# VinAIResearch/COMBAT

Measured on AMD Instinct MI355X. Metric: images/sec per alternated generator+surrogate step, CIFAR-10 bs=128, 1/2/4/8 GPU, higher is better.
Workload: dtype bf16; 1 GPU; train_generator.py --dataset cifar10 --pc 0.5 --noise_rate 0.08: alternated PreActResNet18 surrogate + UNet generator step (Phase C + Phase G, both Nesterov-SGD updates), bs=128 per GPU, on-device augmentation on; per_gpu_batch=128, global_batch=128, parallelism=dp1 (RCCL all-reduce of netC grads in Phase C, netG grads in Phase G), losses_finite=True, deterministic=True

## Files before the change

combat_amd/_lib.py:

```python
from __future__ import annotations

import ctypes as C
import os

HERE = os.path.dirname(os.path.abspath(__file__))
LIB_PATH = os.environ.get("COMBAT_HIP_LIB") or os.path.join(HERE, "libcombat_hip.so")

c_i32, c_i64, c_f32, c_vp = C.c_int32, C.c_int64, C.c_float, C.c_void_p


class ConvArgs(C.Structure):

    _fields_ = [
        ("N", c_i32), ("H", c_i32), ("W", c_i32), ("C", c_i32),
        ("P", c_i32), ("Q", c_i32), ("K", c_i32),
        ("R", c_i32), ("S", c_i32), ("stride", c_i32), ("pad", c_i32),
        ("mode", c_i32),
        ("src", c_vp), ("wpack", c_vp), ("kpad", c_i32), ("rows_pad", c_i32), ("dst", c_vp),
        ("pro_scale", c_vp), ("pro_shift", c_vp), ("pro_group_stride", c_i32), ("pro_act", c_i32),
        ("pro_slope", c_f32),
        ("bias", c_vp), ("add_pre", c_vp), ("mask_x", c_vp), ("mask_scale", c_vp), ("mask_shift", c_vp),
        ("mask_activated", c_i32), ("mask_group_stride", c_i32), ("mask_slope", c_f32), ("mask_mul_scale", c_i32),
        ("add_post", c_vp), ("tanh_out", c_i32),
        ("stats_kind", c_i32), ("stats", c_vp), ("xh_mean", c_vp), ("xh_rstd", c_vp),
        ("act_dst", c_vp), ("act_scale", c_vp), ("act_shift", c_vp), ("act_slope", c_f32),
        ("workspace", c_vp), ("workspace_bytes", c_i64),
        ("tile", c_i32),
        ("src2", c_vp), ("wpack2", c_vp), ("kpad2", c_i32), ("rows_pad2", c_i32),
        ("pro_act_dst", c_vp),
    ]


class WgradArgs(C.Structure):

    _fields_ = [
        ("N", c_i32), ("H", c_i32), ("W", c_i32), ("C", c_i32),
        ("P", c_i32), ("Q", c_i32), ("K", c_i32),
        ("R", c_i32), ("S", c_i32), ("stride", c_i32), ("pad", c_i32),
        ("src", c_vp), ("dy", c_vp), ("dw", c_vp), ("k_real", c_i32), ("c_real", c_i32),
        ("pro_scale", c_vp), ("pro_shift", c_vp), ("pro_group_stride", c_i32), ("pro_act", c_i32),
        ("pro_slope", c_f32), ("split", c_i32),
        ("workspace", c_vp), ("workspace_bytes", c_i64),
        ("defer_reduce", c_i32), ("reserved", c_i32),
        ("reduce_first", c_vp),
    ]


class PackDesc(C.Structure):

    _fields_ = [("w", c_vp), ("wf", c_vp), ("wd", c_vp),
                ("K", c_i32), ("taps", c_i32), ("c_real", c_i32), ("C", c_i32), ("dup_hilo", c_i32),
                ("rows_pad_f", c_i32), ("kpad_f", c_i32), ("rows_pad_d", c_i32), ("kpad_d", c_i32), ("reserved", c_i32),
                ("row_scale", c_vp)]


class BnDesc(C.Structure):

    _fields_ = [("gamma", c_vp), ("beta", c_vp), ("running_mean", c_vp), ("running_var", c_vp),
                ("scale", c_vp), ("shift", c_vp), ("C", c_i32), ("reserved", c_i32)]


SIGNATURES = {
    "combat_version": (C.c_char_p, []),
    "combat_abi_version": (C.c_int, []),
    "combat_set_deterministic": (None, [C.c_int]),
    "combat_get_deterministic": (C.c_int, []),
    "combat_conv_gemm": (C.c_int, [C.POINTER(ConvArgs), c_vp]),
    "combat_conv_gemm_pair": (C.c_int, [C.POINTER(ConvArgs), C.POINTER(ConvArgs), c_vp]),
    "combat_conv_workspace_bytes": (c_i64, [C.POINTER(ConvArgs)]),
    "combat_conv_pick_tile": (C.c_int, [C.POINTER(ConvArgs)]),
    "combat_conv_stats_granule": (C.c_int, [C.c_int]),
    "combat_conv_stats_layout": (C.c_int, [C.POINTER(ConvArgs), C.POINTER(c_i32), C.POINTER(c_i32)]),
    "combat_conv_wgrad": (C.c_int, [C.POINTER(WgradArgs), c_vp]),
    "combat_conv_wgrad_workspace_bytes": (c_i64, [C.POINTER(WgradArgs)]),
    "combat_conv_wgrad_reduce": (C.c_int, [C.POINTER(WgradArgs), c_vp]),
    "combat_pack_weights": (C.c_int, [c_vp, c_i32, c_i32, c_i32, c_i32, c_i32, c_vp, c_i32, c_i32, c_vp, c_i32,
                                      c_i32, c_vp]),
    "combat_norm_finalize": (C.c_int, [c_vp, c_i32, c_i32, c_i32, c_f32, c_f32, c_vp, c_vp, c_vp, c_vp, c_vp, c_vp,
                                       c_vp, c_vp, c_f32, c_vp, c_vp, c_i64, c_vp]),
    "combat_norm_scratch_bytes": (c_i64, [c_i32, c_i32]),
    "combat_bn_eval_fold": (C.c_int, [c_vp, c_vp, c_vp, c_vp, c_f32, c_i32, c_vp, c_vp, c_vp]),
    "combat_pack_weights_batch": (C.c_int, [c_vp, c_i32, c_vp]),
    "combat_bn_eval_fold_batch": (C.c_int, [c_vp, c_i32, c_f32, c_vp]),
    "combat_group_stats": (C.c_int, [c_vp, c_i32, c_i32, c_i32, c_vp, c_vp]),
    "combat_norm_bwd_finalize": (C.c_int, [c_vp, c_i32, c_i32, c_i32, c_f32, c_vp, c_vp, c_vp, c_vp, c_vp, c_vp,
                                           c_vp, c_vp, c_vp, c_i64, c_vp]),
    "combat_norm_bwd_apply": (C.c_int, [c_vp, c_vp, c_vp, c_vp, c_i64, c_i32, c_i32, c_i32, c_vp, c_vp, c_vp, c_vp]),
    "combat_norm_act_fused": (C.c_int, [c_vp, c_vp, c_i32, c_i32, c_i64, c_i32, c_f32, c_f32, c_vp, c_vp, c_vp, c_vp, c_vp,
                                        c_vp, c_vp, c_vp, c_f32, c_vp, c_vp, c_i64, c_vp, c_vp]),
    "combat_norm_add_act_fused": (C.c_int, [c_vp, c_vp, c_i32, c_i32, c_i64, c_i32, c_f32, c_f32, c_vp, c_vp, c_vp, c_vp, c_vp,
                                            c_vp, c_vp, c_vp, c_f32, c_vp, c_vp, c_i64, c_vp, c_vp, c_vp, c_vp, c_vp]),
    "combat_norm_bwd_fused": (C.c_int, [c_vp, c_vp, c_vp, c_vp, c_i32, c_i32, c_i64, c_i32, c_vp, c_vp, c_vp, c_vp, c_vp,
                                        c_vp, c_i64, c_vp, c_vp]),
    "combat_group_stats_bwd": (C.c_int, [c_vp, c_vp, c_i32, c_i32, c_i32, c_i32, c_vp, c_vp, c_vp, c_vp]),
    "combat_unet_up_fused": (C.c_int, [c_vp, c_vp, c_i32, c_vp, c_vp, c_vp, c_i32, c_i32, c_i32, c_i32, c_f32, c_vp, c_vp,
                                       c_vp, c_vp, c_vp, c_vp]),
    "combat_unet_up_bwd_fused": (C.c_int, [c_vp, c_vp, c_vp, c_vp, c_vp, c_i32, c_i32, c_i32, c_i32, c_vp, c_vp, c_vp]),
    "combat_unet_up_fwd": (C.c_int, [c_vp, c_vp, c_vp, c_vp, c_vp, c_vp, c_i32, c_i32, c_i32, c_i32, c_vp, c_vp]),
    "combat_unet_up_bwd": (C.c_int, [c_vp, c_vp, c_i32, c_i32, c_i32, c_i32, c_vp, c_vp]),
    "combat_trigger_fwd": (C.c_int, [c_vp, c_vp, c_vp, c_vp, c_f32, c_i32, c_i32, c_vp, c_vp, c_vp, c_vp, c_vp]),
    "combat_trigger_bwd": (C.c_int, [c_vp, c_vp, c_vp, c_vp, c_f32, c_i32, c_i32, c_vp, c_vp, c_vp, c_f32, c_i32, c_vp, c_vp]),
    "combat_trigger_tv_fwd": (C.c_int, [c_vp, c_vp, c_vp, c_vp, c_f32, c_i32, c_i32, c_vp, c_vp, c_vp, c_vp]),
    "combat_trigger_tv_bwd": (C.c_int, [c_vp, c_vp, c_vp, c_vp, c_f32, c_i32, c_i32, c_vp, c_vp, c_vp, c_f32, c_f32, c_i32, c_vp, c_vp]),
    "combat_trigger_pair_fwd": (C.c_int, [c_vp, c_vp, c_vp, c_vp, c_f32, c_i32, c_i32, c_vp, c_vp, c_vp, c_vp]),
    "combat_trigger_pair_bwd": (C.c_int, [c_vp, c_vp, c_vp, c_vp, c_f32, c_i32, c_i32, c_vp, c_vp, c_vp, c_f32, c_vp, c_i32,
                                          c_vp, c_vp]),
    "combat_trigger_groups_fwd": (C.c_int, [c_vp, c_vp, c_vp, c_vp, c_f32, c_i32, c_i32, c_i32, c_vp, c_vp, c_vp]),
    "combat_trigger_groups_bwd": (C.c_int, [c_vp, c_vp, c_vp, c_vp, c_f32, c_i32, c_i32, c_i32, c_vp, c_vp, c_vp, c_f32, c_i32,
                                            c_vp, c_vp]),
    "combat_cond_fwd": (C.c_int, [c_vp, c_vp, c_i32, c_i32, c_i32, c_i32, c_vp, c_vp]),
    "combat_cond_wgrad": (C.c_int, [c_vp, c_vp, c_i32, c_i32, c_i32, c_i32, c_vp, c_vp, c_vp, c_vp]),
    "combat_augment_fwd": (C.c_int, [c_vp, c_vp, c_vp, c_i32, c_i32, c_vp, c_vp, c_vp]),
    "combat_augment_bwd": (C.c_int, [c_vp, c_i32, c_vp, c_i32, c_i32, c_vp, c_i32, c_vp]),
    "combat_head_fwd": (C.c_int, [c_vp, c_i32, c_i32, c_i32, c_vp, c_vp, c_i32, c_vp, c_f32, c_vp, c_vp, c_vp, c_vp,
                                  c_vp, c_vp, c_vp]),
    "combat_head_bwd": (C.c_int, [c_vp, c_i32, c_i32, c_i32, c_vp, c_i32, c_vp, c_vp, c_f32, c_vp, c_vp, c_vp, c_vp,
                                  c_vp]),
    "combat_head_fwd_bwd": (C.c_int, [c_vp, c_i32, c_i32, c_i32, c_vp, c_vp, c_i32, c_vp, c_f32, c_vp, c_vp, c_vp, c_vp,
                                      c_vp, c_vp, c_vp, c_vp, c_vp]),
    "combat_head_bwd_weights": (C.c_int, [c_vp, c_vp, c_i32, c_i32, c_i32, c_i32, c_vp, c_vp, c_vp]),
    "combat_prune_sweep": (C.c_int, [c_vp, c_i32, c_vp, c_vp, c_vp, c_i32, c_i32, c_i32, c_vp, c_vp, c_vp, c_vp, c_vp]),
    "combat_feature_colsum": (C.c_int, [c_vp, c_i32, c_i32, c_vp, c_vp]),
    "combat_strip_superimpose": (C.c_int, [c_vp, c_i32, c_vp, c_i32, c_vp, c_i32, c_i32, c_i32, c_vp, c_vp]),
    "combat_strip_entropy": (C.c_int, [c_vp, c_i32, c_i32, c_i32, c_vp, c_vp]),
    "combat_nc_blend": (C.c_int, [c_vp, c_i32, c_vp, c_i32, c_vp, c_i32, c_i32, c_i32, c_i32, c_vp, c_vp, c_f32, c_vp, c_vp,
                                  c_vp]),
    "combat_nc_update": (C.c_int, [c_vp, c_vp, c_i32, c_vp, c_i32, c_vp, c_i32, c_i32, c_i32, c_i32, c_vp, c_i32, c_i32,
                                   c_vp, c_vp, c_vp, c_vp, c_f32, c_vp, c_f32, c_f32, c_f32, c_f32, c_vp, c_vp, c_vp, c_i32,
                                   c_vp, c_vp]),
    "combat_gradcam_seed": (C.c_int, [c_vp, c_vp, c_i32, c_i32, c_i32, c_i32, c_vp, c_vp, c_vp, c_vp]),
    "combat_gradcam_map": (C.c_int, [c_vp, c_vp, c_i32, c_i32, c_i32, c_i32, c_vp, c_vp, c_vp, c_vp]),
    "combat_comm_unique_id": (C.c_int, [c_vp]),
    "combat_comm_init_rank": (C.c_int, [C.POINTER(c_vp), c_i32, c_vp, c_i32]),
    "combat_comm_destroy": (C.c_int, [c_vp]),
    "combat_allreduce": (C.c_int, [c_vp, c_i64, c_i32, c_vp, c_vp]),
    "combat_sgd_nesterov": (C.c_int, [c_vp, c_vp, c_i32, c_i64, c_f32, c_f32, c_f32, c_f32, c_i32, c_vp]),
    "combat_image_to_c8": (C.c_int, [c_vp, c_i32, c_i32, c_vp, c_vp]),
    "combat_nhwc_to_nchw_f32": (C.c_int, [c_vp, c_i32, c_i32, c_i32, c_i32, c_i32, c_vp, c_vp]),
    "combat_nchw_to_nhwc_bf16": (C.c_int, [c_vp, c_i32, c_i32, c_i32, c_i32, c_i32, c_vp, c_vp]),
    "combat_memset_zero": (C.c_int, [c_vp, c_i64, c_vp]),
    "combat_copy3": (C.c_int, [c_vp, c_vp, c_i64, c_vp, c_vp, c_i64, c_vp, c_vp, c_i64, c_vp]),
    "combat_relu_mask": (C.c_int, [c_vp, c_vp, c_i64, c_vp, c_vp]),
    "combat_colsum": (C.c_int, [c_vp, c_i64, c_i32, c_i32, c_vp, c_vp]),
    "combat_log_terms": (C.c_int, [c_vp, c_vp, c_vp, c_i32, c_i32, c_vp, c_vp, c_vp, c_vp]),
    "combat_log_terms_tv": (C.c_int, [c_vp, c_vp, c_vp, c_vp, c_i32, c_i32, c_vp, c_vp, c_vp, c_vp]),
    "combat_maxpool2": (C.c_int, [c_vp, c_i32, c_i32, c_i32, c_i32, c_vp, c_vp]),
    "combat_elu_affine": (C.c_int, [c_vp, c_i64, c_i32, c_vp, c_vp, c_vp, c_vp]),
    "combat_affine_act": (C.c_int, [c_vp, c_i64, c_i32, c_vp, c_vp, c_i64, c_f32, c_vp, c_vp]),
    "combat_dct_u8": (C.c_int, [c_vp, c_vp, c_i32, c_i32, c_vp, c_vp]),
    "combat_linear_nhwc": (C.c_int, [c_vp, c_i32, c_i32, c_i32, c_i32, c_vp, c_vp, c_i32, c_vp, c_vp]),
    "combat_grid_head_fwd": (C.c_int, [c_vp, c_vp, c_vp, c_i32, c_i32, c_vp, c_vp]),
    "combat_wanet_grid": (C.c_int, [c_vp, c_vp, c_i32, c_i32, c_f32, c_vp, c_vp, c_vp]),
    "combat_warp_fwd": (C.c_int, [c_vp, c_vp, c_vp, c_i32, c_i32, c_i32, c_vp, c_vp]),
    "combat_warp_bwd": (C.c_int, [c_vp, c_vp, c_vp, c_vp, c_i32, c_i32, c_i32, c_i32, c_vp, c_vp]),
    "combat_warp_bwd_input": (C.c_int, [c_vp, c_vp, c_i32, c_i32, c_i32, c_vp, c_vp]),
    "combat_wanet_field_bwd": (C.c_int, [c_vp, c_i32, c_vp, c_vp, c_i32, c_i32, c_f32, c_f32, c_vp, c_vp, c_vp, c_i32, c_vp,
                                         c_vp, c_vp, c_vp, c_vp]),
    "combat_plan_create": (c_vp, []),
    "combat_plan_destroy": (None, [c_vp]),
    "combat_plan_record": (C.c_int, [c_vp, c_i32]),
    "combat_plan_record_cancel": (C.c_int, []),
    "combat_plan_set_after": (C.c_int, [c_vp, c_i32]),
    "combat_plan_size": (c_i32, [c_vp]),
    "combat_plan_run": (C.c_int, [c_vp, c_i32, c_i32, c_vp, C.POINTER(c_vp), c_i32]),
    "combat_plan_join": (C.c_int, [c_vp, c_vp, C.POINTER(c_vp), c_i32]),
    "combat_plan_failed_call": (c_i32, [c_vp]),
}

TILE_128x128, TILE_128x64, TILE_64x64, TILE_128x16, TILE_64x128 = 1, 2, 3, 4, 5
TILE_H256x64, TILE_H128x128, TILE_H128x64, TILE_H64x64, TILE_D128x64, TILE_D128x32 = 6, 7, 8, 9, 10, 11
TILE_G128x64, TILE_G128x32 = 12, 13
TILE_D256x64, TILE_C8, TILE_D256W64, TILE_S128x64, TILE_K8 = 14, 15, 16, 17, 18
STATS_PER_WORKGROUP = 4


class CombatHipError(RuntimeError):
    pass


def load(path: str = LIB_PATH) -> C.CDLL:
    if not os.path.exists(path):
        raise ImportError(
            "combat_amd: %s not found -- the HIP library is required (no CPU fallback exists); "
            "build it with `python -m combat_amd.build`" % path)
    lib = C.CDLL(path)
    for name, (res, args) in SIGNATURES.items():
        try:
            fn = getattr(lib, name)
        except AttributeError as e:
            raise ImportError("combat_amd: %s does not export %s" % (path, name)) from e
        fn.restype = res
        fn.argtypes = args
    return lib


lib = load()


def check(status: int, what: str, detail: str = "") -> None:
    if status == 0:
        return
    kind = {-1: "invalid shape/argument", -2: "HIP launch failed"}.get(status, "status %d" % status)
    raise CombatHipError("%s: %s %s" % (what, kind, detail))
```

combat_amd/csrc/capi.cpp:

```cpp
#include "combat_hip.h"

#include <hip/hip_runtime.h>

#include <atomic>
#include <cstdlib>
#include <mutex>
#include <unordered_map>

#define COMBAT_ABI_VERSION 20

extern "C" const char *combat_version(void) { return "combat_hip gfx950 abi17"; }
extern "C" int combat_abi_version(void) { return COMBAT_ABI_VERSION; }

static std::atomic<int> g_deterministic{-1};
bool combat_deterministic() {
    int v = g_deterministic.load(std::memory_order_relaxed);
    if (v < 0) {
        const char *e = getenv("COMBAT_DETERMINISTIC");
        v = e && e[0] == '1';
        g_deterministic.store(v, std::memory_order_relaxed);
    }
    return v != 0;
}
extern "C" void combat_set_deterministic(int on) { g_deterministic.store(on ? 1 : 0, std::memory_order_relaxed); }
extern "C" int combat_get_deterministic(void) { return combat_deterministic() ? 1 : 0; }

float *combat_stream_scratch(void *stream, size_t bytes) {
    constexpr size_t kBytes = 2u << 20;
    if (bytes > kBytes) return nullptr;
    static std::mutex mu;
    static std::unordered_map<void *, float *> regions;
    std::lock_guard<std::mutex> lock(mu);
    int dev = 0;
    if (hipGetDevice(&dev) != hipSuccess) return nullptr;
    void *key = reinterpret_cast<void *>(reinterpret_cast<uintptr_t>(stream) ^ (static_cast<uintptr_t>(dev + 1) << 56));
    auto it = regions.find(key);
    if (it != regions.end()) return it->second;
    void *ptr = nullptr;
    if (hipMalloc(&ptr, kBytes) != hipSuccess) return nullptr;
    regions.emplace(key, static_cast<float *>(ptr));
    return static_cast<float *>(ptr);
}
```

combat_amd/csrc/conv_wgrad.hip:

```cpp
#include "conv_common.hpp"
#include "plan.hpp"

namespace {

struct WgradParams {
    combat_wgrad_args a;
    int M, PQ, ntaps, tiles_k, tiles_c, split, pix_per_split;
    float *ws;
};

template <int BMC, int BNC>
struct WCfg {
    static constexpr int WGK = (BNC == 16) ? 4 : (BMC == 16 ? 1 : 2);
    static constexpr int WGC = 4 / WGK;
    static constexpr int WK = BMC / WGK;
    static constexpr int WC = BNC / WGC;
    static constexpr int FK = WK / 16;
    static constexpr int FC = WC / 16;
    static constexpr int SK = (BMC + 16) * 2;
    static constexpr int SC = (BNC + 16) * 2;
    static constexpr int CHK = BMC / 8;
    static constexpr int CHC = BNC / 8;
    static constexpr int ITK = (64 * CHK + 255) / 256;
    static constexpr int ITC = (64 * CHC + 255) / 256;
// ... 276 lines not shown
            {
                const unsigned char *b = kl + prow * SK + (wid * 16 + pp * 4) * 2;
                const s16x4_t lo = lds_tr16(b), hi = lds_tr16(b + 4 * SK);
                const s16x8_t v = {lo[0], lo[1], lo[2], lo[3], hi[0], hi[1], hi[2], hi[3]};
                fk[ks] = __builtin_bit_cast(bf16x8_t, v);
            }
#pragma unroll
            for (int j = 0; j < FC; ++j) {
                const unsigned char *b = cl + prow * SC + (j * 16 + pp * 4) * 2;
                const s16x4_t lo = lds_tr16(b), hi = lds_tr16(b + 4 * SC);
                const s16x8_t v = {lo[0], lo[1], lo[2], lo[3], hi[0], hi[1], hi[2], hi[3]};
                fc[ks][j] = __builtin_bit_cast(bf16x8_t, v);
            }
        }
        __builtin_amdgcn_sched_barrier(0);
#pragma unroll
        for (int ks = 0; ks < 2; ++ks)
#pragma unroll
            for (int j = 0; j < FC; ++j) acc[j] = __builtin_amdgcn_mfma_f32_16x16x32_bf16(fk[ks], fc[ks][j], acc[j], 0, 0, 0);
        __builtin_amdgcn_sched_barrier(0);
    };
    load_tile(0);
    store_tile(0);
    __syncthreads();
    for (int kt = 0; kt < nkt; ++kt) {
        const bool more = kt + 1 < nkt;
        if (more) load_tile(kt + 1);
        compute(kt & 1);
        if (more) store_tile((kt + 1) & 1);
        __syncthreads();
    }
    float *ep = reinterpret_cast<float *>(smem);
    {
        const int fr = lane & 15, fq = lane >> 4;
#pragma unroll
        for (int j = 0; j < FC; ++j) {
            const int col = j * 16 + fr, row = wid * 16 + fq * 4;
#pragma unroll
            for (int e = 0; e < 4; ++e) ep[(row + e) * EPS + col] = acc[j][e];
        }
    }
    __syncthreads();
    const int creal = a.c_real;
    if (p.ws) {
        float *slab = p.ws + (size_t)blockIdx.x * (BMC * 9 * creal);
        for (int idx = tid; idx < BMC * 9 * creal; idx += 256) {
            const int row = idx / (9 * creal), rem = idx - row * 9 * creal;
            const int tap = rem / creal, c = rem - tap * creal;
            float v = ep[row * EPS + tap * 8 + c];
            if (creal < 8 && c + creal < 8) v += ep[row * EPS + tap * 8 + c + creal];
            slab[idx] = v;
        }
        return;
    }
    for (int idx = tid; idx < BMC * 72; idx += 256) {
        const int row = idx / 72, col = idx - row * 72;
        const int n = k0 + row, tap = col >> 3;
        int c = col & 7;
        if (n >= a.k_real) continue;
        if (creal < 8) {
            if (c >= 2 * creal) continue;
            if (c >= creal) c -= creal;
        }
        atomicAdd(a.dw + ((size_t)n * 9 + tap) * creal + c, ep[row * EPS + col]);
    }
}

__global__ __launch_bounds__(256) void conv_wgrad_c8_reduce_kernel(const float *__restrict__ ws, float *__restrict__ dw,
                                                                   int tiles_k, int split, int per_tile, int k_real,
                                                                   int row_elems, float *__restrict__ part) {
    const int e = blockIdx.x * 256 + threadIdx.x, tile_k = blockIdx.y;
    if (e >= per_tile) return;
    const int n = tile_k * 64 + e / row_elems;
    if (n >= k_real) return;
    float s0 = 0.f, s1 = 0.f, s2 = 0.f, s3 = 0.f;
    const int G = gridDim.z;
    int sp = blockIdx.z;
    for (; sp + 3 * G < split; sp += 4 * G) {
        s0 += ws[((size_t)sp * tiles_k + tile_k) * per_tile + e];
        s1 += ws[((size_t)(sp + G) * tiles_k + tile_k) * per_tile + e];
        s2 += ws[((size_t)(sp + 2 * G) * tiles_k + tile_k) * per_tile + e];
        s3 += ws[((size_t)(sp + 3 * G) * tiles_k + tile_k) * per_tile + e];
    }
    for (; sp < split; sp += G) s0 += ws[((size_t)sp * tiles_k + tile_k) * per_tile + e];
    const float s = (s0 + s1) + (s2 + s3);
    if (part) part[((size_t)blockIdx.z * tiles_k + tile_k) * per_tile + e] = s;
    else atomicAdd(dw + (size_t)tile_k * per_tile + e, s);
}

int launch_c8(WgradParams p, hipStream_t st) {
    constexpr int SMEM = 2 * 64 * ((64 + 16) * 2 + (80 + 16) * 2);
    static_assert(SMEM >= 64 * 84 * 4, "epilogue image");
    static bool attr_set = false;
    if (!attr_set) {
        if (hipFuncSetAttribute(reinterpret_cast<const void *>(conv_wgrad_c8_kernel), hipFuncAttributeMaxDynamicSharedMemorySize, SMEM) != hipSuccess)
            return COMBAT_ELAUNCH;
        attr_set = true;
    }
    p.tiles_k = p.a.K / 64;
    p.tiles_c = 1;
    int split = p.a.split;
    const int ktiles = (p.M + 63) / 64;
    if (split <= 0) {
        split = (256 + p.tiles_k - 1) / p.tiles_k;
        const int max_split = (ktiles + 3) / 4;
        if (split > max_split) split = max_split;
        if (split < 1) split = 1;
    }
    if (split > ktiles) split = ktiles;
    p.pix_per_split = ((ktiles + split - 1) / split) * 64;
    p.split = (p.M + p.pix_per_split - 1) / p.pix_per_split;
    const int per_tile = 64 * 9 * p.a.c_real;
    const long need = (long)p.tiles_k * p.split * per_tile * 4;
    p.ws = (p.split > 1 && p.a.workspace && p.a.workspace_bytes >= need) ? reinterpret_cast<float *>(p.a.workspace) : nullptr;
    if (combat_deterministic() && p.split > 1 && !p.ws) return COMBAT_EINVAL;
    COMBAT_LAUNCH(conv_wgrad_c8_kernel, dim3((unsigned)(p.tiles_k * p.split)), dim3(256), SMEM, st, p);
    CB_LAUNCH_CHECK();
    if (p.ws) {
        const int groups = p.split >= 32 ? 16 : 1;
        float *part = nullptr;
        if (combat_deterministic() && groups > 1) {
            const long extra = (long)groups * p.tiles_k * per_tile * 4;
            if (p.a.workspace_bytes >= need + extra) part = p.ws + need / 4;
        }
        const int g1 = combat_deterministic() && !part ? 1 : groups;
        COMBAT_LAUNCH(conv_wgrad_c8_reduce_kernel, dim3((per_tile + 255) / 256, p.tiles_k, g1), dim3(256), 0, st, (const float *)p.ws,
                           p.a.dw, p.tiles_k, p.split, per_tile, p.a.k_real, 9 * p.a.c_real, part);
        CB_LAUNCH_CHECK();
        if (part) {
            COMBAT_LAUNCH(conv_wgrad_c8_reduce_kernel, dim3((per_tile + 255) / 256, p.tiles_k, 1), dim3(256), 0, st, (const float *)part,
                               p.a.dw, p.tiles_k, groups, per_tile, p.a.k_real, 9 * p.a.c_real, (float *)nullptr);
            CB_LAUNCH_CHECK();
        }
    }
    return COMBAT_OK;
}

__global__ __launch_bounds__(256) void wgrad_slab_reduce_kernel(const float *__restrict__ ws, float *__restrict__ dw, int split,
                                                                int ntaps, int tiles_k, int tiles_c, int bmc, int bnc, int k_real,
                                                                int c_real, int C) {
    const long e = (long)blockIdx.x * 256 + threadIdx.x;
    if (e >= (long)k_real * ntaps * c_real) return;
    const int c = (int)(e % c_real), tap = (int)((e / c_real) % ntaps), n = (int)(e / ((long)c_real * ntaps));
    const int tile_k = n / bmc, row = n - tile_k * bmc;
    const size_t tile_elems = (size_t)bmc * bnc, sstride = (size_t)ntaps * tiles_k * tiles_c * tile_elems;
    float total = 0.f;
    for (int half = 0; half < 2; ++half) {
        const int cs = c + half * c_real;
        if (half && (c_real >= C || cs >= C || cs >= 2 * c_real)) break;
        const int tile_c = cs / bnc, col = cs - tile_c * bnc;
        const float *src = ws + (((size_t)tap * tiles_k + tile_k) * tiles_c + tile_c) * tile_elems + (size_t)row * bnc + col;
        float s0 = 0.f, s1 = 0.f, s2 = 0.f, s3 = 0.f;
        int sp = 0;
        for (; sp + 4 <= split; sp += 4) {
            s0 += src[(size_t)sp * sstride];
            s1 += src[(size_t)(sp + 1) * sstride];
            s2 += src[(size_t)(sp + 2) * sstride];
            s3 += src[(size_t)(sp + 3) * sstride];
        }
        for (; sp < split; ++sp) s0 += src[(size_t)sp * sstride];
        total += (s0 + s1) + (s2 + s3);
    }
    dw[e] += total;
}

template <int BMC, int BNC>
int64_t generic_slab_bytes(const combat_wgrad_args &a, int split) {
    const long tiles_k = (a.K + BMC - 1) / BMC, tiles_c = (a.C + BNC - 1) / BNC;
    return (int64_t)split * a.R * a.S * tiles_k * tiles_c * BMC * BNC * 4;
}

template <int BMC, int BNC>
int launch(WgradParams p, hipStream_t st) {
    using T = WCfg<BMC, BNC>;
    static bool attr_set = false;
    auto kern = conv_wgrad_kernel<BMC, BNC>;
    if (!attr_set) {
        if (hipFuncSetAttribute(reinterpret_cast<const void *>(kern), hipFuncAttributeMaxDynamicSharedMemorySize,
                                T::SMEM) != hipSuccess)
            return COMBAT_ELAUNCH;
        attr_set = true;
    }
    p.tiles_k = (p.a.K + BMC - 1) / BMC;
    p.tiles_c = (p.a.C + BNC - 1) / BNC;
    int split = p.a.split;
    const int ktiles = (p.M + 63) / 64;
    if (split <= 0) {
        const int base = p.tiles_k * p.tiles_c * p.ntaps;
        split = ((BMC == 16 ? 2304 : 256) + base - 1) / base;
        const int max_split = (ktiles + 3) / 4;
        if (split > max_split) split = max_split;
        if (split < 1) split = 1;
    }
    if (split > ktiles) split = ktiles;
    p.pix_per_split = ((ktiles + split - 1) / split) * 64;
    p.split = (p.M + p.pix_per_split - 1) / p.pix_per_split;
    const long blocks = (long)p.tiles_k * p.tiles_c * p.ntaps * p.split;
    p.ws = nullptr;
    if (combat_deterministic() && p.split > 1) {
        const int64_t need = generic_slab_bytes<BMC, BNC>(p.a, p.split);
        if (!p.a.workspace || p.a.workspace_bytes < need) return COMBAT_EINVAL;
        p.ws = reinterpret_cast<float *>(p.a.workspace);
    }
    COMBAT_LAUNCH(kern, dim3((unsigned)blocks), dim3(256), T::SMEM, st, p);
    CB_LAUNCH_CHECK();
    if (p.ws) {
        const long elems = (long)p.a.k_real * p.ntaps * p.a.c_real;
        COMBAT_LAUNCH(wgrad_slab_reduce_kernel, dim3((unsigned)((elems + 255) / 256)), dim3(256), 0, st, (const float *)p.ws, p.a.dw,
                      p.split, p.ntaps, p.tiles_k, p.tiles_c, BMC, BNC, p.a.k_real, p.a.c_real, p.a.C);
        CB_LAUNCH_CHECK();
    }
    return COMBAT_OK;
}

template <int BMC, int BNC>
int generic_split(const combat_wgrad_args &a) {
    const long M = (long)a.N * a.P * a.Q;
    const int ktiles = (int)((M + 63) / 64), ntaps = a.R * a.S;
    const int tiles_k = (a.K + BMC - 1) / BMC, tiles_c = (a.C + BNC - 1) / BNC;
    int split = a.split > 0 ? a.split : 0;
    if (split <= 0) {
        const int base = tiles_k * tiles_c * ntaps;
        split = ((BMC == 16 ? 2304 : 256) + base - 1) / base;
        const int max_split = (ktiles + 3) / 4;
        if (split > max_split) split = max_split;
        if (split < 1) split = 1;
    }
    if (split > ktiles) split = ktiles;
    const int pix_per_split = ((ktiles + split - 1) / split) * 64;
    return (int)((M + pix_per_split - 1) / pix_per_split);
}

bool c8_applies(const combat_wgrad_args *a) {
    return a->split >= 0 && a->C == 8 && a->R == 3 && (a->K & 63) == 0 && !a->pro_scale && !a->pro_act;
}

int64_t c8_workspace(const combat_wgrad_args &a) {
    const long M = (long)a.N * a.P * a.Q;
    const int ktiles = (int)((M + 63) / 64), tiles_k = a.K / 64;
    int split = a.split;
    if (split <= 0) {
        split = (256 + tiles_k - 1) / tiles_k;
        const int max_split = (ktiles + 3) / 4;
        if (split > max_split) split = max_split;
        if (split < 1) split = 1;
    }
    if (split > ktiles) split = ktiles;
    const int pix_per_split = ((ktiles + split - 1) / split) * 64;
    const long nsplit = (M + pix_per_split - 1) / pix_per_split;
    if (nsplit <= 1) return 0;
    const int64_t per_tile = 64 * 9 * a.c_real * 4;
    return tiles_k * nsplit * per_tile + (nsplit >= 32 ? 16 * tiles_k * per_tile : 0);
}

int64_t generic_workspace(const combat_wgrad_args &a) {
    if (a.C <= 16) return generic_slab_bytes<64, 16>(a, generic_split<64, 16>(a));
    if (a.K <= 16) return generic_slab_bytes<16, 64>(a, generic_split<16, 64>(a));
    if (a.C % 128 == 0 && a.K % 128 == 0) return generic_slab_bytes<128, 128>(a, generic_split<128, 128>(a));
    return generic_slab_bytes<64, 64>(a, generic_split<64, 64>(a));
}

}

extern "C" int64_t combat_conv_wgrad_workspace_bytes(const combat_wgrad_args *a) {
    if (!a) return 0;
    const int64_t dma = a->split >= 0 ? (int64_t)conv_wgrad3x3_dma_workspace(a) : 0;
    if (dma > 0 || !combat_deterministic()) return dma;
    return c8_applies(a) ? c8_workspace(*a) : generic_workspace(*a);
}

static int validate_wgrad_args(const combat_wgrad_args *a) {
    if (!a || !a->src || !a->dy || !a->dw) return COMBAT_EINVAL;
    if (a->N <= 0 || a->H <= 0 || a->W <= 0 || a->P <= 0 || a->Q <= 0) return COMBAT_EINVAL;
    if (a->C < 8 || (a->C & 7) || a->K < 8 || (a->K & 7)) return COMBAT_EINVAL;
    if (a->R != a->S || (a->R != 1 && a->R != 3)) return COMBAT_EINVAL;
    if (a->stride != 1 && a->stride != 2) return COMBAT_EINVAL;
    if (a->c_real <= 0 || a->c_real > a->C || a->k_real <= 0 || a->k_real > a->K) return COMBAT_EINVAL;
    if ((a->pro_scale == nullptr) != (a->pro_shift == nullptr)) return COMBAT_EINVAL;
    if ((long)a->N * a->P * a->Q > 0x7fffffffL / 8) return COMBAT_EINVAL;
    return COMBAT_OK;
}

extern "C" int combat_conv_wgrad_reduce(const combat_wgrad_args *a, void *stream) {
    COMBAT_PLAN_HOOK(combat_conv_wgrad_reduce, a);
    if (validate_wgrad_args(a) != COMBAT_OK) return COMBAT_EINVAL;
    if (a->split < 0 || !a->defer_reduce) return COMBAT_OK;
    return conv_wgrad3x3_dma_reduce(a, as_stream(stream));
}

extern "C" int combat_conv_wgrad(const combat_wgrad_args *a, void *stream) {
    COMBAT_PLAN_HOOK(combat_conv_wgrad, a);
    if (validate_wgrad_args(a) != COMBAT_OK) return COMBAT_EINVAL;
    WgradParams p;
    p.a = *a;
    p.ws = nullptr;
    p.PQ = a->P * a->Q;
    p.M = (int)((long)a->N * p.PQ);
    p.ntaps = a->R * a->S;
    hipStream_t st = as_stream(stream);
    if (a->split >= 0) {
        int rc = conv_wgrad3x3_dma_try(a, st);
        if (rc <= 0) return rc;
    }
    if (a->reduce_first) {
        const int rc = combat_conv_wgrad_reduce(a->reduce_first, stream);
        if (rc != COMBAT_OK) return rc;
    }
    if (a->split >= 0 && !combat_deterministic()) {
        const int rc = conv_wgrad3x3_try(a, st);
        if (rc <= 0) return rc;
    }
    if (a->split < 0) p.a.split = 0;
    if (c8_applies(a)) return launch_c8(p, st);
    if (a->C <= 16) return launch<64, 16>(p, st);
    if (a->K <= 16) return launch<16, 64>(p, st);
    if (a->C % 128 == 0 && a->K % 128 == 0) return launch<128, 128>(p, st);
    return launch<64, 64>(p, st);
}
```

combat_amd/csrc/conv_wgrad3x3_dma.hip:

```cpp
#include "conv_common.hpp"
#include <stdlib.h>

namespace {

typedef __attribute__((address_space(3))) void lds_void_t;
constexpr unsigned kOob = 0x40000000u;

struct W3dParams {
    combat_wgrad_args a;
    int TW, TH, TI, HWP, HH, HROWS, hpw, tw_shift, th_shift;
    int tiles_x, tiles_y, ntiles, tiles_k, tiles_c, split, per;
    unsigned x_bytes, dy_bytes;
    float *ws;
    const float *red_ws;
    float *red_dw;
    int red_base, red_tiles_c, red_split, red_k_real, red_c_real, red_pad;
    unsigned long long *stamps;
};

#ifdef COMBAT_STAMPS
static unsigned long long *g_stamps_wgrad_host = nullptr;
extern "C" int combat_debug_set_stamps_wgrad(void *p) { g_stamps_wgrad_host = (unsigned long long *)p; return 0; }
#define WCLK() __builtin_readcyclecounter()
#else
#define WCLK() 0ull
#endif

typedef __attribute__((address_space(3))) unsigned char lds_u8;
__device__ __forceinline__ s16x4_t tr16d(const lds_u8 *p) {
    return __builtin_amdgcn_ds_read_tr16_b64_v4i16((__attribute__((address_space(3))) s16x4_t *)(const_cast<lds_u8 *>(p)));
}

__device__ __forceinline__ bf16x8_t join8(const s16x4_t lo, const s16x4_t hi) {
    typedef __attribute__((ext_vector_type(8))) short s16x8_t;
    const s16x8_t v = {lo[0], lo[1], lo[2], lo[3], hi[0], hi[1], hi[2], hi[3]};
    return __builtin_bit_cast(bf16x8_t, v);
}

__device__ __forceinline__ int xkey(int TW, int line, int hx) {
    return ((hx >> 1) & 1) | ((TW == 4 ? (line >> 1) & 1 : ((hx >> 3) + line) & 1) << 1);
}
__device__ __forceinline__ int dkey(int pk) { return ((pk >> 1) & 1) | (((pk >> 3) & 1) << 1); }

template <int N>
__device__ __forceinline__ void wait_vm_lgkm0_barrier() {
    asm volatile("s_waitcnt vmcnt(%0) lgkmcnt(0)" ::"n"(N) : "memory");
    __builtin_amdgcn_s_barrier();
    asm volatile("" ::: "memory");
}

template <int NT>
__device__ __forceinline__ void reduce_slabs(const float *__restrict__ ws, float *__restrict__ dw, int base, int tiles_c, int split,
                                             int k_real, int c_real, unsigned char *scratch, int block, int nblocks) {
    constexpr int U = 4;
    const int tid = threadIdx.x;
    const long e4 = (long)base * 9 * 1024;
    const long per = (e4 + nblocks - 1) / nblocks;
    const long q0 = (long)block * per, q1 = q0 + per < e4 ? q0 + per : e4;
    int SL = 1;
    while (SL * 2 <= split && SL < 32 && (long)(NT / (SL * 2)) * U >= per) SL *= 2;
    const int QP = NT / SL, sl = tid / QP, ql = tid - sl * QP;
    const int nsl = (split - sl + SL - 1) / SL;
    f32x4_t *scr = reinterpret_cast<f32x4_t *>(scratch);
    const size_t sstride = (size_t)base * 9 * 4096;
    for (long qb = q0; qb < q1; qb += (long)QP * U) {
        f32x4_t acc[U];
        long qq[U];
#pragma unroll
        for (int u = 0; u < U; ++u) {
            acc[u] = f32x4_t{0.f, 0.f, 0.f, 0.f};
            qq[u] = qb + (long)u * QP + ql;
        }
        for (int i = 0; i < nsl; i += 4) {
            f32x4_t v[U][4];
#pragma unroll
            for (int u = 0; u < U; ++u)
#pragma unroll
                for (int j = 0; j < 4; ++j) {
                    const bool ok = qq[u] < q1 && i + j < nsl;
                    const float *src = ws + (ok ? qq[u] : q0) * 4 + (size_t)(ok ? sl + (i + j) * SL : 0) * sstride;
                    const f32x4_t x = *reinterpret_cast<const f32x4_t *>(src);
                    v[u][j] = ok ? x : f32x4_t{0.f, 0.f, 0.f, 0.f};
                }
#pragma unroll
            for (int u = 0; u < U; ++u) acc[u] += (v[u][0] + v[u][1]) + (v[u][2] + v[u][3]);
        }
        if (SL > 1) {
#pragma unroll
            for (int u = 0; u < U; ++u) scr[tid * U + u] = acc[u];
            __syncthreads();
            if (sl == 0)
                for (int l = 1; l < SL; ++l)
#pragma unroll
                    for (int u = 0; u < U; ++u) acc[u] += scr[(l * QP + ql) * U + u];
        }
        if (sl == 0) {
#pragma unroll
            for (int u = 0; u < U; ++u) {
                const long q = qq[u];
                if (q >= q1) continue;
                const int f4 = (int)(q & 1023), tap = (int)((q >> 10) % 9), tile = (int)(q / (9 * 1024));
                const int i = f4 >> 9, wave = (f4 >> 6) & 7, lane = f4 & 63;
                const int row = (i * 2 + (wave & 1)) * 16 + (lane >> 4) * 4, col = (wave >> 1) * 16 + (lane & 15);
                const int tile_c = tile % tiles_c, tile_k = tile / tiles_c;
                const int n = tile_k * 64 + row, c = tile_c * 64 + col;
                if (c < c_real) {
#pragma unroll
                    for (int e = 0; e < 4; ++e)
                        if (n + e < k_real) dw[((size_t)(n + e) * 9 + tap) * c_real + c] += acc[u][e];
                }
            }
        }
        if (SL > 1) __syncthreads();
    }
}

template <int HPW, int NS, bool RED>
__device__ __forceinline__ void wgrad3x3_dma_body(const W3dParams &p) {
    extern __shared__ __attribute__((aligned(16))) unsigned char smem[];
    const combat_wgrad_args &a = p.a;
    const int tid = threadIdx.x, lane = tid & 63;
    const int wid = __builtin_amdgcn_readfirstlane(tid >> 6);
    const int wave_k = wid & 1, wave_c = wid >> 1;
    if (RED && p.red_ws) {
        reduce_slabs<512>(p.red_ws, p.red_dw, p.red_base, p.red_tiles_c, p.red_split, p.red_k_real, p.red_c_real, smem, blockIdx.x, gridDim.x);
        __syncthreads();
    }
    int bid = blockIdx.x;
    const int tile_c = bid % p.tiles_c; bid /= p.tiles_c;
    const int tile_k = bid % p.tiles_k;
    const int sp = bid / p.tiles_k;
    const int k0 = tile_k * 64, c0 = tile_c * 64;
    const int t_begin = sp * p.per;
    int t_end = t_begin + p.per;
    if (t_end > p.ntiles) t_end = p.ntiles;
    if (t_begin >= t_end) return;

    const int C = a.C, K = a.K, H = a.H, W = a.W;
    constexpr int XBYTES = HPW * 8192, DYBYTES = 64 * 128, DYBASE = NS * XBYTES;
    constexpr int NDMA = 1 + HPW;
    auto rsrc_words = [&](const void *ptr, unsigned bytes) __attribute__((always_inline)) {
        const unsigned long base = (unsigned long)ptr;
        u32x4_t w;
        w[0] = __builtin_amdgcn_readfirstlane((unsigned)base);
        w[1] = __builtin_amdgcn_readfirstlane((unsigned)(base >> 32) & 0xffffu);
        w[2] = __builtin_amdgcn_readfirstlane(bytes);
        w[3] = 0x00020000u;
        return w;
    };
    const u32x4_t xrs = rsrc_words(a.src, p.x_bytes), dyrs = rsrc_words(a.dy, p.dy_bytes);
    const unsigned lds0 = __builtin_amdgcn_readfirstlane((unsigned)(unsigned long)(lds_void_t *)smem) + wid * 1024;
#ifdef COMBAT_WGRAD_BUILTIN_DMA
    const __amdgpu_buffer_rsrc_t xrsrc = __builtin_amdgcn_make_buffer_rsrc(const_cast<void *>(a.src), 0, p.x_bytes, 0x00020000);
    const __amdgpu_buffer_rsrc_t dyrsrc = __builtin_amdgcn_make_buffer_rsrc(const_cast<void *>(a.dy), 0, p.dy_bytes, 0x00020000);
#define COMBAT_W3_DMA(rs_builtin, rs_words, lds_off, voff) \
    __builtin_amdgcn_raw_ptr_buffer_load_lds(rs_builtin, (lds_void_t *)(smem + (lds_off) + wid * 1024), 16, voff, 0, 0, 0)
#else
#define COMBAT_W3_DMA(rs_builtin, rs_words, lds_off, voff) \
    asm volatile("s_mov_b32 m0, %0\n\ts_nop 0\n\tbuffer_load_dwordx4 %1, %2, 0 offen lds" ::"s"(lds0_l + (unsigned)(lds_off)), "v"(voff), "s"(rs_words##_l) : "memory", "m0")
#endif

    int hdec[HPW], hrel[HPW];
#pragma unroll
    for (int j = 0; j < HPW; ++j) {
        const int row = (wid + 8 * j) * 8 + (lane >> 3), slot = lane & 7;
        const int hx = row % p.HWP, line = row / p.HWP;
        const int hy = line % p.HH, ti = line / p.HH;
        const int chunk = (((slot >> 1) ^ xkey(p.TW, line, hx)) << 1) | (slot & 1);
        hdec[j] = row < p.HROWS ? (hx | (hy << 8) | (ti << 16)) : -1;
        hrel[j] = (((ti * H + hy - 1) * W + hx - 1) * C + c0 + chunk * 8) * 2;
        asm volatile("" : "+v"(hdec[j]), "+v"(hrel[j]));
    }
    int dti[1], drel[1];
#pragma unroll
    for (int j = 0; j < 1; ++j) {
        const int pk = wid * 8 + (lane >> 3), slot = lane & 7;
        const int tx = pk & (p.TW - 1), ty = (pk >> p.tw_shift) & (p.TH - 1), ti = pk >> (p.tw_shift + p.th_shift);
        const int chunk = (((slot >> 1) ^ dkey(pk)) << 1) | (slot & 1);
        dti[j] = ti;
        drel[j] = (((ti * H + ty) * W + tx) * K + k0 + chunk * 8) * 2;
        asm volatile("" : "+v"(dti[j]), "+v"(drel[j]));
    }
    int nt_x, nt_y, nt_g;
    {
        const int t = t_begin;
        nt_x = t % p.tiles_x;
        nt_y = (t / p.tiles_x) % p.tiles_y;
        nt_g = t / (p.tiles_x * p.tiles_y);
    }
    int is_img0 = 0, is_oy0 = 0, is_ox0 = 0, is_xorg = 0, is_dorg = 0;
    auto issue_prep = [&]() __attribute__((always_inline)) {
        is_img0 = nt_g * p.TI;
        is_oy0 = nt_y * p.TH;
        is_ox0 = nt_x * p.TW;
        const int origin = (is_img0 * H + is_oy0) * W + is_ox0;
        is_xorg = origin * C * 2;
        is_dorg = origin * K * 2;
        if (++nt_x == p.tiles_x) {
            nt_x = 0;
            if (++nt_y == p.tiles_y) {
                nt_y = 0;
                ++nt_g;
            }
        }
    };
    auto issue_piece = [&](auto j_tag, auto slot_tag) __attribute__((always_inline)) {
        constexpr int j = decltype(j_tag)::value;
        constexpr int slot_i = decltype(slot_tag)::value;
        const u32x4_t xrs_l = xrs, dyrs_l = dyrs;
        const unsigned lds0_l = lds0;
        (void)xrs_l; (void)dyrs_l; (void)lds0_l;
        if constexpr (j == 0) {
            const unsigned off = is_img0 + dti[0] < a.N ? (unsigned)(is_dorg + drel[0]) : kOob;
            COMBAT_W3_DMA(dyrsrc, dyrs, DYBASE + slot_i * DYBYTES, off);
        } else if constexpr (j <= HPW) {
            const int d = hdec[j - 1];
            const bool ok = d >= 0 && is_img0 + (d >> 16) < a.N && (unsigned)(is_oy0 + ((d >> 8) & 255) - 1) < (unsigned)H &&
                            (unsigned)(is_ox0 + (d & 255) - 1) < (unsigned)W;
            const unsigned off = ok ? (unsigned)(is_xorg + hrel[j - 1]) : kOob;
            COMBAT_W3_DMA(xrsrc, xrs, slot_i * XBYTES + 8 * (j - 1) * 1024, off);
        }
    };
    auto issue = [&](auto slot_tag) __attribute__((always_inline)) {
        using std::integral_constant;
        issue_prep();
        issue_piece(integral_constant<int, 0>{}, slot_tag);
        issue_piece(integral_constant<int, 1>{}, slot_tag);
        issue_piece(integral_constant<int, 2>{}, slot_tag);
        issue_piece(integral_constant<int, 3>{}, slot_tag);
        issue_piece(integral_constant<int, 4>{}, slot_tag);
    };

    const int q = (lane & 15) >> 2, pp = lane & 3, fq = lane >> 4;
    constexpr int SPS = 65536 / XBYTES, NSETS = (NS + SPS - 1) / SPS;
    const lds_u8 *const smem_l = (const lds_u8 *)smem;
    const lds_u8 *dyp[2][2][2], *xp[NSETS][2][2][9];
    int dya[2][2], xa[2][2][9];
#pragma unroll
    for (int ks = 0; ks < 2; ++ks)
#pragma unroll
        for (int hi = 0; hi < 2; ++hi) {
            const int pk = ks * 32 + fq * 8 + q + 4 * hi;
            dya[ks][hi] = pk * 128 + ((wave_k ^ dkey(pk)) & 3) * 32 + pp * 8;
            const int tx = pk & (p.TW - 1), ty = (pk >> p.tw_shift) & (p.TH - 1), ti = pk >> (p.tw_shift + p.th_shift);
#pragma unroll
            for (int tap = 0; tap < 9; ++tap) {
                const int r = (tap * 11) >> 5, s = tap - 3 * r;
                const int line = ti * p.HH + ty + r, hx = tx + s;
                xa[ks][hi][tap] = (line * p.HWP + hx) * 128 + ((wave_c ^ xkey(p.TW, line, hx)) & 3) * 32 + pp * 8;
#pragma unroll
                for (int set = 0; set < NSETS; ++set) {
                    xp[set][ks][hi][tap] = smem_l + set * SPS * XBYTES + xa[ks][hi][tap];
                    asm volatile("" : "+v"(xp[set][ks][hi][tap]));
                }
            }
#pragma unroll
            for (int i = 0; i < 2; ++i) {
                dyp[ks][hi][i] = smem_l + DYBASE + (dya[ks][hi] ^ (i * 64));
                asm volatile("" : "+v"(dyp[ks][hi][i]));
            }
        }

    f32x4_t acc[9][2];
#pragma unroll
    for (int t = 0; t < 9; ++t)
#pragma unroll
        for (int i = 0; i < 2; ++i) acc[t][i] = f32x4_t{0.f, 0.f, 0.f, 0.f};

    auto x_frags = [&](bf16x8_t (&fx)[2], auto slot_tag, auto tap_tag) __attribute__((always_inline)) {
        constexpr int tap = decltype(tap_tag)::value, slot = decltype(slot_tag)::value;
        constexpr int set = slot / SPS, imm = (slot % SPS) * XBYTES;
#pragma unroll
        for (int ks = 0; ks < 2; ++ks) fx[ks] = join8(tr16d(xp[set][ks][0][tap] + imm), tr16d(xp[set][ks][1][tap] + imm));
#ifdef COMBAT_NO_INTERLEAVE
        __builtin_amdgcn_sched_barrier(0);
#endif
    };
    auto mfma_tap = [&](auto tap_tag, const bf16x8_t (&fk)[2][2], const bf16x8_t (&fx)[2]) __attribute__((always_inline)) {
        constexpr int tap = decltype(tap_tag)::value;
#pragma unroll
        for (int ks = 0; ks < 2; ++ks)
#pragma unroll
            for (int i = 0; i < 2; ++i)
                acc[tap][i] = __builtin_amdgcn_mfma_f32_16x16x32_bf16(fk[ks][i], fx[ks], acc[tap][i], 0, 0, 0);
#ifndef COMBAT_NO_INTERLEAVE
        if (tap < 8) {
#pragma unroll
            for (int r = 0; r < 4; ++r) {
                __builtin_amdgcn_sched_group_barrier(0x008, 1, 0);
                __builtin_amdgcn_sched_group_barrier(0x100, 1, 0);
            }
        }
#endif
        __builtin_amdgcn_sched_barrier(0);
    };
    auto compute = [&](auto slot_tag, auto nslot_tag, bool ahead) __attribute__((always_inline)) {
        constexpr int slot = decltype(slot_tag)::value, imm = slot * DYBYTES;
        bf16x8_t fk[2][2];
#pragma unroll
        for (int ks = 0; ks < 2; ++ks)
#pragma unroll
            for (int i = 0; i < 2; ++i)
                fk[ks][i] = join8(tr16d(dyp[ks][0][i] + imm), tr16d(dyp[ks][1][i] + imm));
        using std::integral_constant;
        (void)nslot_tag;
        (void)ahead;
        bf16x8_t fx0[2], fx1[2];
        x_frags(fx0, slot_tag, integral_constant<int, 0>{});
        __builtin_amdgcn_sched_barrier(0);
#define COMBAT_W3_TAP(t, cur, nxt)                                                   \
        if (t < 8) x_frags(nxt, slot_tag, integral_constant<int, (t < 8 ? t + 1 : 8)>{});  \
        mfma_tap(integral_constant<int, t>{}, fk, cur);
        COMBAT_W3_TAP(0, fx0, fx1) COMBAT_W3_TAP(1, fx1, fx0) COMBAT_W3_TAP(2, fx0, fx1) COMBAT_W3_TAP(3, fx1, fx0)
        COMBAT_W3_TAP(4, fx0, fx1) COMBAT_W3_TAP(5, fx1, fx0) COMBAT_W3_TAP(6, fx0, fx1) COMBAT_W3_TAP(7, fx1, fx0)
        COMBAT_W3_TAP(8, fx0, fx1)
#undef COMBAT_W3_TAP
    };
    static_assert(HPW <= 4, "issue() spells out 1 + HPW <= 5 pieces");

    const int npatch = t_end - t_begin;
    using std::integral_constant;
    unsigned long long ph[4] = {0, 0, 0, 0};
    unsigned long long c_loop0 = 0;
    {
    issue(integral_constant<int, 0>{});
    if (NS > 2 && npatch > 1) issue(integral_constant<int, 1 % NS>{});
    if (NS > 2 && npatch > 1) wait_vm_lgkm0_barrier<NDMA>(); else wait_vm_lgkm0_barrier<0>();
    c_loop0 = WCLK();
    auto body = [&](auto slot_tag, int i) __attribute__((always_inline)) {
        constexpr int slot = decltype(slot_tag)::value, nslot = (slot + NS - 1) % NS;
        const bool ahead = i + NS - 1 < npatch;
        const unsigned long long c0 = WCLK();
        if (ahead) issue(integral_constant<int, nslot>{});
        __builtin_amdgcn_sched_barrier(0);
        const unsigned long long c1 = WCLK();
        compute(integral_constant<int, slot>{}, integral_constant<int, nslot>{}, ahead);
        const unsigned long long c2 = WCLK();
        if (ahead) wait_vm_lgkm0_barrier<(NS - 2) * NDMA>(); else wait_vm_lgkm0_barrier<0>();
#ifdef COMBAT_STAMPS
        const unsigned long long c3 = WCLK();
        ph[0] += c1 - c0; ph[1] += c2 - c1; ph[2] += c3 - c2; ph[3] += 1;
#else
        (void)c0; (void)c1; (void)c2;
#endif
    };
    for (int i = 0; i < npatch; i += NS) {
        body(integral_constant<int, 0>{}, i);
        if (NS > 1 && i + 1 < npatch) body(integral_constant<int, 1 % NS>{}, i + 1);
        if (NS > 2 && i + 2 < npatch) body(integral_constant<int, 2 % NS>{}, i + 2);
    }
    }
    static_assert(NS == 2 || NS == 3, "the patch loop is unrolled for rings of two or three stages");
#ifdef COMBAT_STAMPS
    const unsigned long long c_loop1 = WCLK();
#endif

    if (p.ws) {
        float *slab = p.ws + (size_t)blockIdx.x * 9 * 4096;
#pragma unroll
        for (int tap = 0; tap < 9; ++tap)
#pragma unroll
            for (int i = 0; i < 2; ++i)
                *reinterpret_cast<f32x4_t *>(slab + tap * 4096 + ((i * 8 + wid) * 64 + lane) * 4) = acc[tap][i];
    } else {
        float *ep = reinterpret_cast<float *>(smem);
        constexpr int EPS = 68;
        const int fr = lane & 15;
#pragma unroll 1
        for (int tap = 0; tap < 9; ++tap) {
#pragma unroll
            for (int i = 0; i < 2; ++i) {
                const int col = wave_c * 16 + fr;
                const int row = (i * 2 + wave_k) * 16 + fq * 4;
                f32x4_t v;
                switch (tap) {
                    case 0: v = acc[0][i]; break;
                    case 1: v = acc[1][i]; break;
                    case 2: v = acc[2][i]; break;
                    case 3: v = acc[3][i]; break;
                    case 4: v = acc[4][i]; break;
                    case 5: v = acc[5][i]; break;
                    case 6: v = acc[6][i]; break;
                    case 7: v = acc[7][i]; break;
                    default: v = acc[8][i]; break;
                }
#pragma unroll
                for (int e = 0; e < 4; ++e) ep[(row + e) * EPS + col] = v[e];
            }
            __syncthreads();
            for (int idx = tid; idx < 64 * 64; idx += 512) {
                const int row = idx >> 6, col = idx & 63;
                const int n = k0 + row, c = c0 + col;
                if (n < a.k_real && c < a.c_real) atomicAdd(a.dw + ((size_t)n * 9 + tap) * a.c_real + c, ep[row * EPS + col]);
            }
            __syncthreads();
        }
    }
#ifdef COMBAT_STAMPS
    if (lane == 0 && p.stamps) {
        unsigned long long *o = p.stamps + (blockIdx.x * 8 + wid) * 8;
        o[0] = ph[0]; o[1] = ph[1]; o[2] = ph[2]; o[3] = ph[3];
        o[4] = c_loop1 - c_loop0; o[5] = WCLK() - c_loop1; o[6] = c_loop0;
    }
#endif
}

__global__ __launch_bounds__(256) void wgrad3x3_reduce_kernel(const float *__restrict__ ws, float *__restrict__ dw,
                                                              int base, int tiles_c, int split, int k_real, int c_real) {
    const long e4 = (long)blockIdx.x * 256 + threadIdx.x;
    if (e4 >= (long)base * 9 * 1024) return;
    const int f4 = (int)(e4 & 1023), tap = (int)((e4 >> 10) % 9), tile = (int)(e4 / (9 * 1024));
    const int per = (split + gridDim.y - 1) / gridDim.y;
    const int s0 = blockIdx.y * per, s1 = s0 + per < split ? s0 + per : split;
    f32x4_t acc = {0.f, 0.f, 0.f, 0.f};
    const float *src = ws + ((size_t)tile * 9 + tap) * 4096 + f4 * 4;
    const size_t sstride = (size_t)base * 9 * 4096;
    int s = s0;
    for (; s + 4 <= s1; s += 4) {
        const f32x4_t v0 = *reinterpret_cast<const f32x4_t *>(src + (size_t)s * sstride);
        const f32x4_t v1 = *reinterpret_cast<const f32x4_t *>(src + (size_t)(s + 1) * sstride);
        const f32x4_t v2 = *reinterpret_cast<const f32x4_t *>(src + (size_t)(s + 2) * sstride);
        const f32x4_t v3 = *reinterpret_cast<const f32x4_t *>(src + (size_t)(s + 3) * sstride);
        acc += (v0 + v1) + (v2 + v3);
    }
    for (; s < s1; ++s) acc += *reinterpret_cast<const f32x4_t *>(src + (size_t)s * sstride);
    const int i = f4 >> 9, wave = (f4 >> 6) & 7, lane = f4 & 63;
    const int row = (i * 2 + (wave & 1)) * 16 + (lane >> 4) * 4, col = (wave >> 1) * 16 + (lane & 15);
    const int tile_c = tile % tiles_c, tile_k = tile / tiles_c;
    const int n = tile_k * 64 + row, c = tile_c * 64 + col;
    if (c < c_real && s0 < s1) {
#pragma unroll
        for (int e = 0; e < 4; ++e) {
            if (n + e >= k_real) break;
            float *o = dw + ((size_t)(n + e) * 9 + tap) * c_real + c;
            if (gridDim.y == 1) *o += acc[e];
            else atomicAdd(o, acc[e]);
        }
    }
}

__global__ __launch_bounds__(256) void wgrad3x3_reduce_det_kernel(const float *__restrict__ ws, float *__restrict__ dw, int base,
                                                                  int tiles_c, int split, int k_real, int c_real) {
    __shared__ __attribute__((aligned(16))) unsigned char scratch[256 * 64];
    reduce_slabs<256>(ws, dw, base, tiles_c, split, k_real, c_real, scratch, blockIdx.x, gridDim.x);
}

template <int HPW, int NS, bool RED>
__global__ __launch_bounds__(512, 1) void conv_wgrad3x3_dma_kernel(const W3dParams p) { wgrad3x3_dma_body<HPW, NS, RED>(p); }

template <int HPW, int NS, bool RED>
int launch_w3d_red(const W3dParams &p, int blocks, hipStream_t st) {
    constexpr int stage = 8192 + HPW * 8192;
    constexpr int ep = 64 * 68 * 4;
    constexpr int smem = NS * stage > ep ? NS * stage : ep;
    auto kern = conv_wgrad3x3_dma_kernel<HPW, NS, RED>;
    static bool attr = false;
    if (!attr) {
        if (hipFuncSetAttribute(reinterpret_cast<const void *>(kern), hipFuncAttributeMaxDynamicSharedMemorySize, smem) != hipSuccess)
            return COMBAT_ELAUNCH;
        attr = true;
    }
    COMBAT_LAUNCH(kern, dim3(blocks), dim3(512), smem, st, p);
    CB_LAUNCH_CHECK();
    return COMBAT_OK;
}

template <int HPW, int NS>
int launch_w3d(const W3dParams &p, int blocks, hipStream_t st) {
    return p.red_ws ? launch_w3d_red<HPW, NS, true>(p, blocks, st) : launch_w3d_red<HPW, NS, false>(p, blocks, st);
}

bool w3d_geometry(const combat_wgrad_args *a, W3dParams &p, int &smem) {
    if (!(a->R == 3 && a->S == 3 && a->stride == 1 && a->pad == 1 && a->P == a->H && a->Q == a->W)) return false;
    if (a->pro_scale || a->pro_act) return false;
    if (a->C < 64 || (a->C & 63) || a->K < 64 || (a->K & 63) || a->c_real != a->C) return false;
    const int W = a->W, H = a->H;
    const int TW = W < 16 ? W : 16;
    const int TH = H < 64 / TW ? H : 64 / TW;
    const int TI = 64 / (TW * TH);
    if (TW < 2 || TI < 1 || TW * TH * TI != 64) return false;
    p.a = *a;
    p.TW = TW; p.TH = TH; p.TI = TI;
    p.HWP = TW + 2; p.HH = TH + 2; p.HROWS = TI * p.HH * p.HWP;
    p.hpw = (p.HROWS + 63) / 64;
    p.tw_shift = ilog2_exact(TW); p.th_shift = ilog2_exact(TH);
    if (p.tw_shift < 0 || p.th_shift < 0 || W % TW || H % TH) return false;
    const long xb = (long)a->N * H * W * a->C * 2, db = (long)a->N * H * W * a->K * 2;
    if (xb >= (long)kOob || db >= (long)kOob) return false;
    p.x_bytes = (unsigned)xb; p.dy_bytes = (unsigned)db;
    p.tiles_x = W / TW; p.tiles_y = H / TH;
    p.ntiles = p.tiles_x * p.tiles_y * ((a->N + TI - 1) / TI);
    p.tiles_k = a->K / 64; p.tiles_c = a->C / 64;
    smem = 0;
    return p.hpw >= 2 && p.hpw <= 4;
}

int pick_split(const combat_wgrad_args *a, const W3dParams &p, bool with_ws) {
    const int base = p.tiles_k * p.tiles_c;
    int split = a->split;
    if (split <= 0) {
        static const int ws_wgs = getenv("COMBAT_WGRAD_WGS") ? atoi(getenv("COMBAT_WGRAD_WGS")) : 128;
        const int by_cus = ((with_ws ? ws_wgs : 256) + base - 1) / base;
        const int by_atomics = 164 / base > 0 ? 164 / base : 1;
        split = with_ws || by_cus < by_atomics ? by_cus : by_atomics;
        const int by_work = (p.ntiles + 3) / 4;
        if (split > by_work) split = by_work;
        if (split < 1) split = 1;
    }
    if (split > p.ntiles) split = p.ntiles;
    const int per = (p.ntiles + split - 1) / split;
    return (p.ntiles + per - 1) / per;
}

}

long conv_wgrad3x3_dma_workspace(const combat_wgrad_args *a) {
    W3dParams p;
    int smem;
    if (!w3d_geometry(a, p, smem)) return 0;
    const int split = pick_split(a, p, true);
    return split > 1 ? (long)split * p.tiles_k * p.tiles_c * 9 * 4096 * 4 : 0;
}

namespace {
bool w3d_plan(const combat_wgrad_args *a, W3dParams &p) {
    int smem;
    if (!w3d_geometry(a, p, smem)) return false;
    const int base = p.tiles_k * p.tiles_c;
    int split = pick_split(a, p, true);
    const bool use_ws = split > 1 && a->workspace && a->workspace_bytes >= (long)split * base * 9 * 4096 * 4;
    if (!use_ws) split = pick_split(a, p, false);
    p.ws = use_ws ? reinterpret_cast<float *>(a->workspace) : nullptr;
    p.per = (p.ntiles + split - 1) / split;
    p.split = (p.ntiles + p.per - 1) / p.per;
    return true;
}

int launch_reduce(const combat_wgrad_args *a, const W3dParams &p, hipStream_t st) {
    const int base = p.tiles_k * p.tiles_c;
    static const bool env_det = getenv("COMBAT_WGRAD_DET_REDUCE") != nullptr;
    const bool det = combat_deterministic();
    const bool atomics = !env_det && (!det || base >= 4);
    if (atomics) {
        const long e4 = (long)base * 9 * 1024;
        int groups = (int)(512 / ((e4 + 255) / 256));
        if (groups < 1 || det) groups = 1;
        if (groups > p.split) groups = p.split;
        COMBAT_LAUNCH(wgrad3x3_reduce_kernel, dim3((unsigned)((e4 + 255) / 256), groups), dim3(256), 0, st, p.ws, a->dw, base,
                           p.tiles_c, p.split, a->k_real, a->c_real);
    } else {
        COMBAT_LAUNCH(wgrad3x3_reduce_det_kernel, dim3(256), dim3(256), 0, st, (const float *)p.ws, a->dw, base, p.tiles_c, p.split,
                           a->k_real, a->c_real);
    }
    CB_LAUNCH_CHECK();
    return COMBAT_OK;
}

bool fill_reduce_first(const combat_wgrad_args *prev, W3dParams &p) {
    p.red_ws = nullptr;
    p.red_dw = nullptr;
    p.red_base = p.red_tiles_c = p.red_split = p.red_k_real = p.red_c_real = p.red_pad = 0;
    if (!prev) return true;
    W3dParams q;
    if (!w3d_plan(prev, q)) return true;
    if (!q.ws) return true;
    p.red_ws = q.ws;
    p.red_dw = prev->dw;
    p.red_base = q.tiles_k * q.tiles_c;
    p.red_tiles_c = q.tiles_c;
    p.red_split = q.split;
    p.red_k_real = prev->k_real;
    p.red_c_real = prev->c_real;
    return true;
}
}

int conv_wgrad3x3_dma_try(const combat_wgrad_args *a, hipStream_t st) {
    W3dParams p;
    if (!w3d_plan(a, p)) return 1;
    if (combat_deterministic() && !p.ws && p.split > 1) return COMBAT_EINVAL;
    if (!fill_reduce_first(a->reduce_first, p)) return COMBAT_EINVAL;
#ifdef COMBAT_STAMPS
    p.stamps = g_stamps_wgrad_host;
#else
    p.stamps = nullptr;
#endif
    const int blocks = p.tiles_k * p.tiles_c * p.split;
    int rc;
    if (p.hpw == 2) rc = launch_w3d<2, 3>(p, blocks, st);
    else if (p.hpw == 3) rc = launch_w3d<3, 2>(p, blocks, st);
    else rc = launch_w3d<4, 2>(p, blocks, st);
    if (rc != COMBAT_OK || !p.ws || a->defer_reduce) return rc;
    return launch_reduce(a, p, st);
}

int conv_wgrad3x3_dma_reduce(const combat_wgrad_args *a, hipStream_t st) {
    W3dParams p;
    if (!w3d_plan(a, p) || !p.ws) return COMBAT_OK;
    return launch_reduce(a, p, st);
}
```

combat_amd/engine.py:

```python
from __future__ import annotations

import ctypes
import os
from typing import Dict, List, Optional, Tuple

import torch

from . import ops
from ._lib import STATS_PER_WORKGROUP, TILE_D128x32, TILE_D128x64, TILE_S128x64, CombatHipError, ConvArgs, lib
from .nets import UNET_LAYERS
from .ops import Affine, PackedConv, bf16

BATCH_STATS_ROWS = 0 if os.environ.get("COMBAT_STATS_PER_WAVE") == "1" else STATS_PER_WORKGROUP

f32 = torch.float32


def _p(t):
    return None if t is None else t.data_ptr()


class Plan:

    serial = False
# ... 113 lines not shown
            return self._run_py(prof, on_mark)
        prog = self._program()
        if on_mark is None:
            prog = self._prog_nomark
        stream = torch.cuda.current_stream()
        st = stream.cuda_stream
        n_aux = self.aux_queues if (self.aux and not Plan.serial) else 0
        auxp = _aux_pointers(stream, n_aux) if n_aux else None
        cp = self._cplan
        for it in prog:
            kind = it[0]
            if kind == "c":
                rc = lib.combat_plan_run(cp, it[1], it[2], st, auxp, n_aux)
                if rc:
                    what = self._cnames[lib.combat_plan_failed_call(cp)]
                    kindname = {-1: "invalid shape/argument", -2: "HIP launch failed"}.get(rc, "status %d" % rc)
                    raise CombatHipError("%s/%s: %s" % (self.name, what, kindname))
            elif kind == "py":
                rc = it[1](*it[2], st)
                if rc:
                    raise CombatHipError("%s/%s: status %d" % (self.name, it[3], rc))
            else:
                if n_aux:
                    ops.check(lib.combat_plan_join(cp, st, auxp, n_aux), "combat_plan_join")
                on_mark(it[1])
        if n_aux:
            ops.check(lib.combat_plan_join(cp, st, auxp, n_aux), "combat_plan_join")

    def __del__(self):
        try:
            if self._cplan:
                lib.combat_plan_destroy(self._cplan)
        except Exception:
            pass

    def _run_py(self, prof: Optional[list] = None, on_mark=None) -> None:
        stream = torch.cuda.current_stream()
        st = stream.cuda_stream
        auxs = []
        if self.aux and not Plan.serial:
            auxs = [_aux_stream(stream, k) for k in range(self.aux_queues)]
        used = set()
        awaited = set(self.after.values()) if auxs else set()
        done: Dict[int, torch.cuda.Event] = {}
        for ci, (cfunc, args, what) in enumerate(self.calls):
            if auxs and ci in self.after and self.after[ci] in done:
                (auxs[self.aux[ci]] if ci in self.aux else stream).wait_event(done[self.after[ci]])
            if prof is not None and cfunc is lib.combat_conv_gemm_pair:
                rc = 0
                for sub, arg in zip(what.split("+"), args):
                    e0, e1 = torch.cuda.Event(enable_timing=True), torch.cuda.Event(enable_timing=True)
                    e0.record(stream)
                    rc = rc or lib.combat_conv_gemm(arg, st)
                    e1.record(stream)
                    prof.append((self.name + "/" + sub, arg._obj, e0, e1))
            elif prof is not None and (cfunc is lib.combat_conv_gemm or cfunc is lib.combat_conv_wgrad or
                                       cfunc is lib.combat_conv_wgrad_reduce):
                e0, e1 = torch.cuda.Event(enable_timing=True), torch.cuda.Event(enable_timing=True)
                e0.record(stream)
                rc = cfunc(*args, st)
                e1.record(stream)
                prof.append((self.name + "/" + what, args[0]._obj, e0, e1))
            elif auxs and ci in self.aux:
                q = self.aux[ci]
                ev = torch.cuda.Event()
                ev.record(stream)
                auxs[q].wait_event(ev)
                rc = cfunc(*args, auxs[q].cuda_stream)
                used.add(q)
            else:
                rc = cfunc(*args, st)
            if rc:
                kind = {-1: "invalid shape/argument", -2: "HIP launch failed"}.get(rc, "status %d" % rc)
                raise CombatHipError("%s/%s: %s" % (self.name, what, kind))
            if ci in awaited:
                done[ci] = torch.cuda.Event()
                done[ci].record(auxs[self.aux[ci]] if ci in self.aux else stream)
            if on_mark is not None and ci in self.marks:
                for q in used:
                    ev = torch.cuda.Event()
                    ev.record(auxs[q])
                    stream.wait_event(ev)
                on_mark(self.marks[ci])
        for q in used:
            ev = torch.cuda.Event()
            ev.record(auxs[q])
            stream.wait_event(ev)

    def __len__(self):
        return len(self.calls)


_AUX_STREAMS: Dict = {}
_AUX_POINTERS: Dict = {}


class PlanSeq:

    def __init__(self, name: str, plans):
        self.name, self.plans = name, list(plans)

    @property
    def calls(self):
        return [c for p in self.plans for c in p.calls]

    def run(self, prof: Optional[list] = None, on_mark=None) -> None:
        for p in self.plans:
            p.run(prof, on_mark=on_mark)

    def __len__(self):
        return sum(len(p) for p in self.plans)


def _aux_pointers(parent: torch.cuda.Stream, n: int):
    key = (parent.device, parent.cuda_stream, n)
    arr = _AUX_POINTERS.get(key)
    if arr is None:
        arr = (ctypes.c_void_p * n)(*[_aux_stream(parent, k).cuda_stream for k in range(n)])
        _AUX_POINTERS[key] = arr
    return arr


_HIP = None


def low_priority_stream(dev) -> torch.cuda.Stream:
    global _HIP
    if _HIP is None:
        _HIP = ctypes.CDLL("libamdhip64.so")
    least, greatest = ctypes.c_int(), ctypes.c_int()
    assert _HIP.hipDeviceGetStreamPriorityRange(ctypes.byref(least), ctypes.byref(greatest)) == 0
    h = ctypes.c_void_p()
    with torch.cuda.device(dev):
        assert _HIP.hipStreamCreateWithPriority(ctypes.byref(h), 1, least.value) == 0
    print("low-priority stream: range least %d greatest %d" % (least.value, greatest.value), flush=True)
    return torch.cuda.ExternalStream(h.value, device=dev)


def _aux_stream(parent: torch.cuda.Stream, k: int = 0) -> torch.cuda.Stream:
    key = (parent.device, parent.cuda_stream, k)
    s = _AUX_STREAMS.get(key)
    if s is None:
        if os.environ.get("COMBAT_LOW_PRIO_SIDE", "0") == "1":
            s = low_priority_stream(parent.device)
        else:
            s = torch.cuda.Stream(device=parent.device)
        _AUX_STREAMS[key] = s
    return s


class Slot:

    def __init__(self, device, n: int, hw: int):
        self.device, self.N, self.hw = device, n, hw
        self.bufs: Dict[str, torch.Tensor] = {}
        self.norm: Dict[str, "NormState"] = {}
        self.plans: Dict[str, Plan] = {}

    def half_view(self, lo: int, n: int, share: Tuple[str, ...]) -> "Slot":
        s = Slot(self.device, n, self.hw)
        for k in share:
            if k in self.bufs:
                s.bufs[k] = self.bufs[k][lo:lo + n]
        s.feat_hw = getattr(self, "feat_hw", None)
        return s

    def buf(self, name: str, shape, dtype=bf16, zero: bool = False) -> torch.Tensor:
        t = self.bufs.get(name)
        if t is None:
            t = (torch.zeros if zero else torch.empty)(tuple(shape), dtype=dtype, device=self.device)
            self.bufs[name] = t
        assert tuple(t.shape) == tuple(shape) and t.dtype == dtype, (name, t.shape, shape)
        return t


class NormState:

    def __init__(self, slot: Slot, key: str, groups: int, c: int):
        mk = lambda s: slot.buf("%s.%s" % (key, s), (groups, c), f32)
        self.groups, self.C = groups, c
        self.mean, self.rstd, self.scale, self.shift = mk("mean"), mk("rstd"), mk("scale"), mk("shift")
        self.pending = self.bpending = None
        self._slot, self._key = slot, key


class FlatParams:

    ALIGN = 64

    def __init__(self, module: torch.nn.Module):
        params = list(module.named_parameters())
        dev = params[0][1].device
        self.offsets: Dict[str, Tuple[int, int, tuple]] = {}
        off = 0
        for name, p in params:
            self.offsets[name] = (off, p.numel(), tuple(p.shape))
            off += (p.numel() + self.ALIGN - 1) // self.ALIGN * self.ALIGN
        self.total = off
        self.flat = torch.zeros(off, dtype=f32, device=dev)
        self.grad = torch.zeros(off, dtype=f32, device=dev)
        self.mom = torch.zeros(off, dtype=f32, device=dev)
        with torch.no_grad():
            for name, p in params:
                o, n, shape = self.offsets[name]
                dst = self.flat[o:o + n]
                if p.dim() == 4:
                    k, c, r, s = shape
                    dst.copy_(p.detach().permute(0, 2, 3, 1).reshape(-1))
                    p.data = dst.view(k, r, s, c).permute(0, 3, 1, 2)
                else:
                    dst.copy_(p.detach().reshape(-1))
                    p.data = dst.view(shape)
        self.sgd_ptrs = torch.tensor([[self.flat.data_ptr(), self.grad.data_ptr(), self.mom.data_ptr()]],
                                     dtype=torch.int64, device=dev)
        self.sgd_sizes = torch.tensor([self.total], dtype=torch.int64, device=dev)

    def _slice(self, base: torch.Tensor, name: str) -> torch.Tensor:
        o, n, _ = self.offsets[name]
        return base[o:o + n]

    def grad_phys(self, name: str) -> torch.Tensor:
        o, n, shape = self.offsets[name]
        g = self.grad[o:o + n]
        if len(shape) == 4:
            k, c, r, s = shape
            return g.view(k, r * s, c)
        return g.view(shape)

    def logical(self, base: torch.Tensor, name: str) -> torch.Tensor:
        o, n, shape = self.offsets[name]
        g = base[o:o + n]
        if len(shape) == 4:
            k, c, r, s = shape
            return g.view(k, r, s, c).permute(0, 3, 1, 2)
        return g.view(shape)

    zero_ev = None

    def zero_grad_behind(self) -> None:
        if Plan.serial:
            return
        main = torch.cuda.current_stream()
        aux = _aux_stream(main)
        ev = torch.cuda.Event()
        ev.record(main)
        aux.wait_event(ev)
        ops.check(lib.combat_memset_zero(self.grad.data_ptr(), self.total * 4, aux.cuda_stream), "zero_grad")
        self.zero_ev = torch.cuda.Event()
        self.zero_ev.record(aux)

    def sgd_step(self, lr: float, momentum: float = 0.9, weight_decay: float = 5e-4, grad_scale: float = 1.0):
        ops.sgd_nesterov(self.sgd_ptrs, self.sgd_sizes, 1, self.total, lr, momentum, weight_decay, grad_scale, False)




def _zero_grad_call(fp, st):
    ev = fp.zero_ev
    if ev is not None:
        fp.zero_ev = None
        torch.cuda.current_stream().wait_event(ev)
        return 0
    return lib.combat_memset_zero(fp.grad.data_ptr(), fp.total * 4, st)


_SHORT_WORKGROUPS = False


class short_workgroups:

    def __enter__(self):
        global _SHORT_WORKGROUPS
        self.prev, _SHORT_WORKGROUPS = _SHORT_WORKGROUPS, True

    def __exit__(self, *exc):
        global _SHORT_WORKGROUPS
        _SHORT_WORKGROUPS = self.prev


def _tile_preference(a) -> None:
    if _SHORT_WORKGROUPS and a.tile == 0 and lib.combat_conv_pick_tile(ctypes.byref(a)) == TILE_S128x64:
        a.tile = TILE_D128x64


FUSE_SHORTCUT = os.environ.get("COMBAT_NO_FUSED_SHORTCUT", "0") != "1"
REDUCE_BEHIND = os.environ.get("COMBAT_REDUCE_BEHIND", "0") == "1"
FUSED_PROLOGUE = os.environ.get("COMBAT_FUSED_PROLOGUE", "0") == "1"


def fuse_shortcut(dy, dx, pc: PackedConv, dy_sc, pc_sc: PackedConv):
    if FUSE_SHORTCUT and not Plan.serial_shortcuts and ops.shortcut_fusable(dy, dx, pc, pc_sc) and tuple(dy_sc.shape) == tuple(dy.shape):
        return (dy_sc, pc_sc)
    return None


def rec_conv(plan: Plan, what: str, src, dst, pc: PackedConv, mode: int, **kw):
    a = ops.conv_args(src, dst, pc, mode, workspace=plan.workspace(src.device), **kw)
    _tile_preference(a)
    plan.hold(a)
    plan.add(what, lib.combat_conv_gemm, ctypes.byref(a))
    return a


def rec_wgrad(plan: Plan, what: str, src, dy, pc: PackedConv, dw, pro: Optional[Affine] = None, aux: bool = True):
    a = ops.WgradArgs()
    a.N, a.H, a.W, a.C = src.shape
    _, a.P, a.Q, a.K = dy.shape
    a.R = a.S = pc.R
    a.stride, a.pad = pc.stride, pc.pad
    a.src, a.dy, a.dw, a.k_real, a.c_real = src.data_ptr(), dy.data_ptr(), dw.data_ptr(), pc.K, pc.c_real
    if pro is not None:
        a.pro_scale, a.pro_shift = _p(pro.scale), _p(pro.shift)
        a.pro_group_stride, a.pro_act, a.pro_slope = pro.group_stride, int(pro.act), pro.slope
    a.split = 0
    queue = plan.next_aux_queue() if aux else -1
    ws = _wgrad_workspace(src.device, queue)
    a.workspace, a.workspace_bytes = ws.data_ptr(), ws.numel()
    need = int(lib.combat_conv_wgrad_workspace_bytes(ctypes.byref(a)))
    prev = plan.chain.get(queue) if aux else None
    if aux and REDUCE_BEHIND and not Plan.defer_reduces and need > 0:
        if prev is not None:
            a.reduce_first = ctypes.addressof(prev[1])
            plan.pending_reduces = [q for q in plan.pending_reduces if q[1] is not prev[1]]
            plan.hold(prev[1])
            plan.chain.pop(queue)
        k = plan.chain_count.get(queue, 0)
        plan.chain_count[queue] = k + 1
        ws = _wgrad_slab_region(src.device, queue, k % 2, need)
        a.workspace, a.workspace_bytes, a.defer_reduce = ws.data_ptr(), ws.numel(), 1
        plan.chain[queue] = (what, a)
    elif aux and need > 0 and Plan.defer_reduces:
        ws = torch.empty(need, dtype=torch.uint8, device=src.device)
        a.workspace, a.workspace_bytes, a.defer_reduce = ws.data_ptr(), need, 1
    plan.hold(a, src, dy, dw, pro, ws)
    plan.add(what, lib.combat_conv_wgrad, ctypes.byref(a), aux=aux)
    plan.wgrads.append((len(plan.calls) - 1, a))
    if a.defer_reduce:
        plan.pending_reduces.append((what + ".reduce", a, len(plan.calls) - 1))


def set_deterministic(on: bool) -> None:
    lib.combat_set_deterministic(1 if on else 0)


def deterministic() -> bool:
    return bool(lib.combat_get_deterministic())


_WGRAD_SLABS: Dict = {}


def _wgrad_slab_region(device, queue: int, which: int, need: int) -> torch.Tensor:
    key = (device, int(queue), int(which))
    t = _WGRAD_SLABS.get(key)
    if t is None or t.numel() < need:
        t = torch.empty(max(need, 24 << 20), dtype=torch.uint8, device=device)
        _WGRAD_SLABS[key] = t
    return t


def balance_wgrads(plan: Plan, device) -> None:
    tail = int(os.environ.get("COMBAT_WGRAD_MAIN_TAIL", WGRAD_MAIN_TAIL))
    if tail <= 0 or Plan.serial:
        return
    aux_calls = [(ci, a) for ci, a in plan.wgrads if ci in plan.aux]
    ws = _wgrad_workspace(device, -1)
    plan._prog = None
    for ci, a in aux_calls[-tail:]:
        plan.aux.pop(ci, None)
        a.workspace, a.workspace_bytes = ws.data_ptr(), ws.numel()
        plan.hold(ws)


WGRAD_MAIN_TAIL = 0


_WGRAD_WS: Dict = {}


def _wgrad_workspace(device, queue: int = 0) -> torch.Tensor:
    key = (device, int(queue))
    ws = _WGRAD_WS.get(key)
    if ws is None:
        ws = torch.empty(48 << 20, dtype=torch.uint8, device=device)
        _WGRAD_WS[key] = ws
    return ws


def rec_act(plan: Plan, what: str, src, dst, aff: Affine):
    c = src.shape[-1]
    rows = src.numel() // c
    group_rows = (src.shape[1] * src.shape[2]) if aff.group_stride else 0
    assert aff.act and aff.group_stride in (0, c)
    plan.hold(src, dst, aff)
    plan.add(what, lib.combat_affine_act, src.data_ptr(), rows, c, _p(aff.scale), _p(aff.shift), group_rows,
             float(aff.slope), dst.data_ptr())


def _pow2_part(pq: int, cap: int = 32) -> int:
    g = 1
    while g * 2 <= cap and pq % (g * 2) == 0:
        g *= 2
    return g


class NetEngine:

    _flush_at_marks = False

    @property
    def flush_at_marks(self) -> bool:
        return self._flush_at_marks

    @flush_at_marks.setter
    def flush_at_marks(self, value: bool) -> None:
        value = bool(value)
        if value != self._flush_at_marks:
            for slot in getattr(self, "slots", {}).values():
                for k in [k for k in slot.plans if k.startswith("bwd")]:
                    del slot.plans[k]
        self._flush_at_marks = value

    def __init__(self, module: torch.nn.Module):
        self.module = module
        self.device = next(module.parameters()).device
        if self.device.type != "cuda":
            raise CombatHipError("combat_amd engines run on the GPU only (module is on %s); there is no CPU path"
                                 % self.device)
        self.fp = FlatParams(module)
        self.convs: List[PackedConv] = []
        self.slots: Dict[Tuple, Slot] = {}
        self._scratch = torch.empty(ops.norm_scratch_bytes(1, 512) // 4, dtype=f32, device=self.device)
        self.weights_dirty = True

    def mark_weights_dirty(self) -> None:
        self.weights_dirty = True

    def slot(self, name: str, n: int, hw: int) -> Slot:
        key = (name, n, hw)
        s = self.slots.get(key)
        if s is None:
            s = Slot(self.device, n, hw)
            self.slots[key] = s
        return s

    def _pc(self, weight, stride, pad, cin_pad, dup=False, need_dgrad=True, row_scale=None) -> PackedConv:
        pc = PackedConv(weight, stride, pad, cin_pad, dup_hilo=dup, need_dgrad=need_dgrad, row_scale=row_scale)
        self.convs.append(pc)
        return pc

    def refresh(self) -> None:
        if not self.weights_dirty:
            return
        self._pack_all()
        self._refresh_extra()
        self.weights_dirty = False

    def _pack_all(self) -> None:
        ptrs = tuple(pc.weight.data_ptr() for pc in self.convs)
        if getattr(self, "_pack_ptrs", None) != ptrs:
            masters = [pc.master() for pc in self.convs]
            if any(m.data_ptr() != q for m, q in zip(masters, ptrs)):
                self._pack_ptrs = None
                for pc in self.convs:
                    pc.pack()
                return
            from ._lib import PackDesc
            tab = (PackDesc * len(self.convs))()
            for d, pc, m in zip(tab, self.convs, masters):
                pc.fill_desc(d, m)
            self._pack_tab = torch.frombuffer(bytearray(bytes(tab)), dtype=torch.uint8).to(self.device)
            self._pack_ptrs = ptrs
        ops.check(lib.combat_pack_weights_batch(self._pack_tab.data_ptr(), len(self.convs),
                                                torch.cuda.current_stream().cuda_stream), "combat_pack_weights_batch")

    def _refresh_extra(self) -> None:
        pass

    FUSED_DIRECT_PX = 1024

    def _conv_norm(self, plan: Plan, slot: Slot, key: str, src, dst, pc: PackedConv, *, groups: int,
                   gamma=None, beta=None, running=None, act_dst=None, slope: float = 0.0, defer: bool = False,
                   **conv_kw) -> NormState:
        n, p, q, c = dst.shape
        pq, m = p * q, n * p * q
        a = ops.conv_args(src, dst, pc, 0, workspace=plan.workspace(src.device), **conv_kw)
        a.stats_kind = 1 | (BATCH_STATS_ROWS if groups == 1 else 0)
        _tile_preference(a)
        rows, rpi = ops.conv_stats_layout(a)
        fused = (groups == 1) or (rpi > 0)
        st = slot.norm.get(key)
        if st is None:
            st = NormState(slot, key, groups, c)
            slot.norm[key] = st
        part = None
        if fused:
            part = slot.buf(key + ".part", (rows, 2, c), f32)
            a.stats = part.data_ptr()
            rpg = rows if groups == 1 else rpi
        else:
            a.stats_kind = 0
        plan.hold(a, part)
        plan.add(key + ".conv", lib.combat_conv_gemm, ctypes.byref(a))
        one_launch = act_dst is not None or defer
        if not fused and not (one_launch and pq <= self.FUSED_DIRECT_PX):
            g = _pow2_part(pq)
            parts = m // g
            part = slot.buf(key + ".part", (parts, 2, c), f32)
            plan.add(key + ".stats", lib.combat_group_stats, dst.data_ptr(), parts, g, c, part.data_ptr())
            rpg = pq // g
        rm = rv = nbt = None
        if running is not None:
            rm, rv, nbt = running
        plan.hold(gamma, beta, rm, rv, nbt)
        if one_launch:
            st.pending = dict(x=dst, part=part, rpg=rpg if part is not None else 0, pxg=m // groups, key=key,
                              gamma=gamma, beta=beta, rm=rm, rv=rv, nbt=nbt)
            if act_dst is not None:
                self._norm_act(plan, st, act_dst, slope)
            return st
        plan.add(key + ".finalize", lib.combat_norm_finalize, part.data_ptr(), groups, rpg, c, float(m // groups),
                 1e-5, _p(gamma), _p(beta), st.mean.data_ptr(), st.rstd.data_ptr(), st.scale.data_ptr(),
                 st.shift.data_ptr(), _p(rm), _p(rv), 0.1, _p(nbt), self._scratch.data_ptr(),
                 self._scratch.numel() * 4)
        return st

    def _lds_prologue_ok(self, src, pc: PackedConv) -> bool:
        if not FUSED_PROLOGUE or pc.R != 3 or pc.stride != 1:
            return False
        n, h, w, _ = src.shape
        probe = getattr(self, "_pro_probe", None)
        if probe is None:
            t = torch.zeros(512, dtype=f32, device=self.device)
            probe = self._pro_probe = Affine(t, t, 0, True, 0.0)
        a = ConvArgs()
        a.N, a.H, a.W, a.C = src.shape
        a.P, a.Q, a.K = h, w, pc.Kc
        a.R = a.S = 3
        a.stride, a.pad, a.mode = 1, pc.pad, 0
        a.src, a.dst, a.pro_act_dst = src.data_ptr(), src.data_ptr(), src.data_ptr()
        a.wpack, a.kpad, a.rows_pad = pc.wf.data_ptr(), pc.kpad_f, pc.rows_f
        a.pro_scale, a.pro_shift, a.pro_act = probe.scale.data_ptr(), probe.shift.data_ptr(), 1
        return lib.combat_conv_pick_tile(ctypes.byref(a)) in (TILE_D128x64, TILE_D128x32)

    def _norm_act(self, plan: Plan, st: NormState, act_dst, slope: float):
        q = st.pending
        st.pending = None
        x = q["x"]
        plan.hold(x, act_dst, q["part"])
        plan.add(q["key"] + ".finact", lib.combat_norm_act_fused, x.data_ptr(), _p(q["part"]), st.groups, q["rpg"],
                 q["pxg"], st.C, 1e-5, float(slope), _p(q["gamma"]), _p(q["beta"]), st.mean.data_ptr(),
                 st.rstd.data_ptr(), st.scale.data_ptr(), st.shift.data_ptr(), _p(q["rm"]), _p(q["rv"]), 0.1,
                 _p(q["nbt"]), self._scratch.data_ptr(), self._scratch.numel() * 4, act_dst.data_ptr())

    def _dgrad_norm(self, plan: Plan, slot: Slot, key: str, dy, dz, pc: PackedConv, x_pre, st: NormState, *,
                    group_stride: int, slope: float, gamma=None, dgamma=None, dbeta=None, add_pre=None, shortcut=None):
        n, p, q, c = dz.shape
        pq, m = p * q, n * p * q
        groups = st.groups
        mask = Affine(st.scale, st.shift, group_stride, True, slope)
        a = ops.conv_args(dy, dz, pc, 1, add_pre=add_pre, mask_x=x_pre, mask=mask, workspace=plan.workspace(dy.device),
                          shortcut=shortcut)
        a.stats_kind = 2 | (BATCH_STATS_ROWS if groups == 1 else 0)
        a.xh_mean, a.xh_rstd = st.mean.data_ptr(), st.rstd.data_ptr()
        _tile_preference(a)
        rows, rpi = ops.conv_stats_layout(a)
        fused = (groups == 1) or (rpi > 0)
        part, rpg = None, 0
        if fused:
            part = slot.buf(key + ".bpart", (rows, 2, c), f32)
            a.stats = part.data_ptr()
            rpg = rows if groups == 1 else rpi
        else:
            a.stats_kind, a.xh_mean, a.xh_rstd = 0, None, None
        plan.hold(a, part)
        plan.add(key + ".dgrad", lib.combat_conv_gemm, ctypes.byref(a))
        if not fused and pq > self.FUSED_DIRECT_PX:
            part, rpg = self._stats_bwd(plan, slot, key, dz, x_pre, st)
        st.bpending = dict(part=part, rpg=rpg, gamma=gamma, dgamma=dgamma, dbeta=dbeta)

    def _stats_bwd(self, plan: Plan, slot: Slot, key: str, dz, x_pre, st: NormState):
        n, p, q, c = dz.shape
        pq, m = p * q, n * p * q
        g = _pow2_part(pq if st.groups > 1 else m)
        parts = m // g
        part = slot.buf(key + ".bpart", (parts, 2, c), f32)
        ppi = (pq // g) if st.groups > 1 else 0
        plan.add(key + ".bstats", lib.combat_group_stats_bwd, dz.data_ptr(), x_pre.data_ptr(), parts, g, c, ppi,
                 st.mean.data_ptr(), st.rstd.data_ptr(), part.data_ptr())
        return part, (pq // g if st.groups > 1 else parts)

    def _bwd_apply(self, plan: Plan, slot: Slot, key: str, dz, x_pre, dx, st: NormState, add=None):
        n, p, q, c = dz.shape
        pq, m = p * q, n * p * q
        pend = getattr(st, "bpending", None) or dict(part=None, rpg=0, gamma=None, dgamma=None, dbeta=None)
        st.bpending = None
        part, rpg = pend["part"], pend["rpg"]
        pxg = m // st.groups
        if part is None and (st.groups == 1 or pq > self.FUSED_DIRECT_PX):
            part, rpg = self._stats_bwd(plan, slot, key, dz, x_pre, st)
        plan.hold(dz, x_pre, dx, add, part, pend["gamma"], pend["dgamma"], pend["dbeta"])
        plan.add(key + ".bfused", lib.combat_norm_bwd_fused, dz.data_ptr(), x_pre.data_ptr(), _p(add), _p(part),
                 st.groups, rpg, pxg, c, _p(pend["gamma"]), st.mean.data_ptr(), st.rstd.data_ptr(),
                 _p(pend["dgamma"]), _p(pend["dbeta"]), self._scratch.data_ptr(), self._scratch.numel() * 4,
                 dx.data_ptr())




class _BN:
    def __init__(self, eng: "NetEngine", mod: torch.nn.BatchNorm2d, prefix: str):
        self.prefix, self.C = prefix, mod.num_features
        self.gamma, self.beta = mod.weight.data, mod.bias.data
        self.rm, self.rv, self.nbt = mod.running_mean, mod.running_var, mod.num_batches_tracked
        self.escale = torch.empty(self.C, dtype=f32, device=eng.device)
        self.eshift = torch.empty(self.C, dtype=f32, device=eng.device)

    def fold(self):
        ops.bn_eval_fold(self.gamma, self.beta, self.rm, self.rv, self.escale, self.eshift)

    def eval_affine(self) -> Affine:
        return Affine(self.escale, self.eshift, 0, True, 0.0)


class _Blk:
    pass


class PreActEngine(NetEngine):

    def __init__(self, module):
        super().__init__(module)
        m = module
        self.classes = m.linear.out_features
        self.stem = self._pc(m.conv1.weight.data, 1, 1, 8, dup=True)
        self.blocks: List[_Blk] = []
        self.bns: List[_BN] = []
        for li in range(1, 5):
            for bi, blk in enumerate(getattr(m, "layer%d" % li)):
                e = _Blk()
                e.prefix = "layer%d.%d." % (li, bi)
                e.stride, e.cin, e.planes = blk.stride, blk.conv1.in_channels, blk.conv1.out_channels
                e.bn1, e.bn2 = _BN(self, blk.bn1, e.prefix + "bn1"), _BN(self, blk.bn2, e.prefix + "bn2")
                e.conv1 = self._pc(blk.conv1.weight.data, blk.stride, 1, e.cin)
                e.conv2 = self._pc(blk.conv2.weight.data, 1, 1, e.planes)
                e.sc = self._pc(blk.shortcut[0].weight.data, blk.stride, 0, e.cin) if hasattr(blk, "shortcut") else None
                self.blocks.append(e)
                self.bns += [e.bn1, e.bn2]
        self.lin_w, self.lin_b = m.linear.weight.data, m.linear.bias.data

    def _refresh_extra(self):
        self.fold_bn()

    def fold_bn(self):
        ptrs = tuple(t.data_ptr() for bn in self.bns for t in (bn.gamma, bn.beta, bn.rm, bn.rv))
        if getattr(self, "_bn_ptrs", None) != ptrs:
            from ._lib import BnDesc
            tab = (BnDesc * len(self.bns))()
            for d, bn in zip(tab, self.bns):
                d.gamma, d.beta, d.running_mean, d.running_var = (t.data_ptr() for t in (bn.gamma, bn.beta, bn.rm, bn.rv))
                d.scale, d.shift, d.C = bn.escale.data_ptr(), bn.eshift.data_ptr(), bn.C
            self._bn_tab = torch.frombuffer(bytearray(bytes(tab)), dtype=torch.uint8).to(self.device)
            self._bn_ptrs = ptrs
        ops.check(lib.combat_bn_eval_fold_batch(self._bn_tab.data_ptr(), len(self.bns), 1e-5,
                                                torch.cuda.current_stream().cuda_stream), "combat_bn_eval_fold_batch")

    def head_bufs(self, slot: Slot):
        n = slot.N
        return dict(
            logits=slot.buf("logits", (n, self.classes), f32), dlogits=slot.buf("dlogits", (n, self.classes), f32),
            pooled=slot.buf("pooled", (n, self.lin_w.shape[1]), f32), loss=slot.buf("loss", (1,), f32, zero=True),
            correct=slot.buf("correct", (2,), torch.int32, zero=True),
            targets=slot.buf("targets", (n,), torch.int64, zero=True),
            targets2=slot.buf("targets2", (n,), torch.int64, zero=True))

    def input(self, slot: Slot) -> torch.Tensor:
        return slot.buf("x", (slot.N, slot.hw, slot.hw, 8))

    FWD_SHARED = ("stem", "logits", "dlogits", "pooled", "targets", "targets2") + tuple(
        "b%d.%s" % (b, s) for b in range(8) for s in ("y1", "out", "sc", "a1", "act")) + ("stem.act",)

    def forward_plan(self, slot: Slot, train: bool, loss_weight: float = 1.0, with_targets2: bool = False,
                     split_head: bool = False, head_bwd: bool = False, two_loss: bool = False, keep_raw_blocks=()) -> Plan:
        keep_raw_blocks = tuple(sorted(set(int(b) for b in keep_raw_blocks)))
        if keep_raw_blocks:
            if type(self) is not PreActEngine or train or two_loss:
                raise ValueError("keep_raw_blocks: only an eval pass of the pre-activation classifier keeps extra raw outputs")
            if keep_raw_blocks[0] < 0 or keep_raw_blocks[-1] >= len(self.blocks):
                raise ValueError("keep_raw_blocks: blocks %s outside 0..%d" % (keep_raw_blocks, len(self.blocks) - 1))
        if two_loss:
            assert not train and not split_head and not with_targets2 and not head_bwd
            key = "fwd.eval.%g.tl" % loss_weight
            if key not in slot.plans:
                halves = self.two_loss_halves(slot)
                slot.plans[key] = PlanSeq("%s.%s" % (type(self).__name__, key),
                                          [self.forward_plan(s, False, loss_weight) for s in halves])
                slot.feat_hw = halves[0].feat_hw
            return slot.plans[key]
        key = "fwd.%s.%g.%d.%d%s" % ("train" if train else "eval", loss_weight, with_targets2, split_head, ".hb" if head_bwd else "")
        if keep_raw_blocks:
            key += ".kr" + ",".join(str(b) for b in keep_raw_blocks)
        if key in slot.plans:
            return slot.plans[key]
        P = Plan("preact." + key)
        n, hw = slot.N, slot.hw
        x = self.input(slot)
        if keep_raw_blocks:
            cur, chw = self._forward_eval_body(P, slot, x, keep_raw_blocks)
        elif not train:
            cur, chw = self._forward_eval_body(P, slot, x)
        else:
            cur, chw = self._forward_train_body(P, slot, x)
        h = self.head_bufs(slot)
        P.hold(h)
        if head_bwd:
            assert not split_head and type(self) is PreActEngine
            d_feat = slot.buf("g.feat", cur.shape)
            P.hold(d_feat)
            P.add("head+bwd", lib.combat_head_fwd_bwd, cur.data_ptr(), n, chw, cur.shape[-1], self.lin_w.data_ptr(),
                  self.lin_b.data_ptr(), self.classes, h["targets"].data_ptr(), loss_weight, h["pooled"].data_ptr(),
                  h["logits"].data_ptr(), h["loss"].data_ptr(), h["correct"].data_ptr(),
                  h["targets2"].data_ptr() if with_targets2 else None,
                  h["correct"][1:].data_ptr() if with_targets2 else None, h["dlogits"].data_ptr(), d_feat.data_ptr())
        elif not split_head:
            P.add("head", lib.combat_head_fwd, cur.data_ptr(), n, chw, cur.shape[-1], self.lin_w.data_ptr(),
                  self.lin_b.data_ptr(), self.classes, h["targets"].data_ptr(), loss_weight, h["pooled"].data_ptr(),
                  h["logits"].data_ptr(), h["loss"].data_ptr(), h["correct"].data_ptr(),
                  h["targets2"].data_ptr() if with_targets2 else None,
                  h["correct"][1:].data_ptr() if with_targets2 else None)
        else:
            assert not train and n % 2 == 0
            m = n // 2
            loss0 = slot.buf("loss0", (1,), f32, zero=True)
            correct0 = slot.buf("correct0", (2,), torch.int32, zero=True)
            views = [cur[:m], cur[m:], h["targets"][:m], h["targets"][m:], h["pooled"][:m], h["pooled"][m:],
                     h["logits"][:m], h["logits"][m:], h["targets2"][m:]]
            P.hold(views, loss0, correct0)
            P.add("head.metric", lib.combat_head_fwd, views[0].data_ptr(), m, chw, cur.shape[-1], self.lin_w.data_ptr(),
                  self.lin_b.data_ptr(), self.classes, views[2].data_ptr(), 1.0, views[4].data_ptr(),
                  views[6].data_ptr(), loss0.data_ptr(), correct0.data_ptr(), None, None)
            P.add("head.loss", lib.combat_head_fwd, views[1].data_ptr(), m, chw, cur.shape[-1], self.lin_w.data_ptr(),
                  self.lin_b.data_ptr(), self.classes, views[3].data_ptr(), loss_weight, views[5].data_ptr(),
                  views[7].data_ptr(), h["loss"].data_ptr(), h["correct"].data_ptr(),
                  views[8].data_ptr() if with_targets2 else None,
                  h["correct"][1:].data_ptr() if with_targets2 else None)
        slot.plans[key] = P
        slot.feat_hw = chw
        return P

    def _forward_train_body(self, P: Plan, slot: Slot, x):
        n, hw = slot.N, slot.hw
        cur = slot.buf("stem", (n, hw, hw, 64))

        def fuse(blk, src):
            return blk.sc is None and blk.stride == 1 and self._lds_prologue_ok(src, blk.conv1)

        first = self.blocks[0].bn1
        a0 = slot.buf("b0.a0", cur.shape)
        st = self._conv_norm(P, slot, first.prefix, x, cur, self.stem, groups=1, gamma=first.gamma, beta=first.beta,
                             running=(first.rm, first.rv, first.nbt), act_dst=None if fuse(self.blocks[0], cur) else a0)
        chw = hw
        for b, blk in enumerate(self.blocks):
            ohw = chw // blk.stride
            i_sc = len(P.calls)
            if blk.sc is not None:
                resid = slot.buf("b%d.sc" % b, (n, ohw, ohw, blk.planes))
                rec_conv(P, "b%d.sc" % b, a0, resid, blk.sc, 0)
            else:
                resid = cur
            y1 = slot.buf("b%d.y1" % b, (n, ohw, ohw, blk.planes))
            out = slot.buf("b%d.out" % b, (n, ohw, ohw, blk.planes))
            nxt = self.blocks[b + 1].bn1 if b + 1 < len(self.blocks) else None
            a1 = slot.buf("b%d.a1t" % b, y1.shape)
            fuse2 = self._lds_prologue_ok(y1, blk.conv2)
            bn2 = dict(groups=1, gamma=blk.bn2.gamma, beta=blk.bn2.beta, running=(blk.bn2.rm, blk.bn2.rv, blk.bn2.nbt),
                       act_dst=None if fuse2 else a1)
            if fuse(blk, cur):
                st2 = self._conv_norm(P, slot, blk.bn2.prefix, cur, y1, blk.conv1, **bn2,
                                      pro=Affine(st.scale, st.shift, 0, True, 0.0), pro_act_dst=a0)
            else:
                st2 = self._conv_norm(P, slot, blk.bn2.prefix, a0, y1, blk.conv1, **bn2)
            if blk.sc is not None:
                P.merge_convs(i_sc)
            c2 = dict(add_post=resid)
            src2 = a1
            if fuse2:
                c2.update(pro=Affine(st2.scale, st2.shift, 0, True, 0.0), pro_act_dst=a1)
                src2 = y1
            if nxt is not None:
                a0 = slot.buf("b%d.a0" % (b + 1), out.shape)
                st = self._conv_norm(P, slot, nxt.prefix, src2, out, blk.conv2, groups=1, gamma=nxt.gamma, beta=nxt.beta,
                                     running=(nxt.rm, nxt.rv, nxt.nbt),
                                     act_dst=None if fuse(self.blocks[b + 1], out) else a0, **c2)
            else:
                rec_conv(P, "b%d.c2" % b, src2, out, blk.conv2, 0, **c2)
            cur, chw = out, ohw
        return cur, chw

    def _forward_eval_body(self, P: Plan, slot: Slot, x, keep_raw_blocks=()):
        n, hw = slot.N, slot.hw
        blocks = self.blocks
        raw = slot.buf("stem", (n, hw, hw, 64)) if blocks[0].sc is None else None
        act = slot.buf("stem.act", (n, hw, hw, 64))
        rec_conv(P, "stem", x, raw, self.stem, 0, act_dst=act, act=blocks[0].bn1.eval_affine())
        chw = hw
        for b, blk in enumerate(blocks):
            ohw = chw // blk.stride
            shape = (n, ohw, ohw, blk.planes)
            if blk.sc is not None:
                resid = slot.buf("b%d.sc" % b, shape)
                rec_conv(P, "b%d.sc" % b, act, resid, blk.sc, 0)
            else:
                resid = raw
            a1 = slot.buf("b%d.a1" % b, shape)
            rec_conv(P, "b%d.c1" % b, act, None, blk.conv1, 0, act_dst=a1, act=blk.bn2.eval_affine())
            if blk.sc is not None:
                P.merge_convs(len(P.calls) - 2)
            nxt = blocks[b + 1] if b + 1 < len(blocks) else None
            keep_raw = nxt is None or nxt.sc is None or b in keep_raw_blocks
            out = slot.buf("b%d.out" % b, shape) if keep_raw else None
            if nxt is not None:
                nact = slot.buf("b%d.act" % b, shape)
                rec_conv(P, "b%d.c2" % b, a1, out, blk.conv2, 0, add_post=resid, act_dst=nact, act=nxt.bn1.eval_affine())
            else:
                nact = None
                rec_conv(P, "b%d.c2" % b, a1, out, blk.conv2, 0, add_post=resid)
            raw, act, chw = out, nact, ohw
        return raw, chw

    def _block_io(self, slot: Slot, b: int):
        xin = slot.bufs["stem"] if b == 0 else slot.bufs["b%d.out" % (b - 1)]
        return xin, slot.bufs["b%d.y1" % b], slot.bufs["b%d.out" % b]

    def backward_train_plan(self, slot: Slot, loss_weight: float = 1.0, head_done: bool = False) -> Plan:
        key = "bwd.train.%g%s" % (loss_weight, ".hd" if head_done else "")
        if key in slot.plans:
            return slot.plans[key]
        P = Plan("preact." + key)
        P.flush_at_marks = self.flush_at_marks
        fp, n = self.fp, slot.N
        h = self.head_bufs(slot)
        P.add("zero_grad", _zero_grad_call, fp)
        feat = slot.bufs["b%d.out" % (len(self.blocks) - 1)]
        d_out = slot.buf("g.feat", feat.shape)
        if not head_done:
            P.add("head_bwd", lib.combat_head_bwd, h["pooled"].data_ptr(), n, slot.feat_hw, feat.shape[-1],
                  self.lin_w.data_ptr(), self.classes, h["logits"].data_ptr(), h["targets"].data_ptr(), loss_weight,
                  h["dlogits"].data_ptr(), d_out.data_ptr(), fp.grad_phys("linear.weight").data_ptr(),
                  fp.grad_phys("linear.bias").data_ptr())
        head_w_pending = head_done
        for b in reversed(range(len(self.blocks))):
            blk = self.blocks[b]
            xin, y1, _ = self._block_io(slot, b)
            st1, st2 = slot.norm[blk.bn1.prefix], slot.norm[blk.bn2.prefix]
            a0, a1 = slot.bufs["b%d.a0" % b], slot.bufs["b%d.a1t" % b]
            pre = blk.prefix
            if not head_w_pending:
                rec_wgrad(P, "b%d.c2.wgrad" % b, a1, d_out, blk.conv2, fp.grad_phys(pre + "conv2.weight"))
            dz2 = slot.buf("g.b%d.dz2" % b, y1.shape)
            self._dgrad_norm(P, slot, "g." + blk.bn2.prefix, d_out, dz2, blk.conv2, y1, st2, group_stride=0,
                             slope=0.0, gamma=blk.bn2.gamma, dgamma=fp.grad_phys(pre + "bn2.weight"),
                             dbeta=fp.grad_phys(pre + "bn2.bias"))
            if head_w_pending:
                head_w_pending = False
                P.hold(h)
                P.add("head_bwd.w", lib.combat_head_bwd_weights, h["dlogits"].data_ptr(), h["pooled"].data_ptr(), n, slot.feat_hw,
                      feat.shape[-1], self.classes, fp.grad_phys("linear.weight").data_ptr(), fp.grad_phys("linear.bias").data_ptr(),
                      aux=True)
                rec_wgrad(P, "b%d.c2.wgrad" % b, a1, d_out, blk.conv2, fp.grad_phys(pre + "conv2.weight"))
            dy1 = slot.buf("g.b%d.dy1" % b, y1.shape)
            self._bwd_apply(P, slot, "g." + blk.bn2.prefix, dz2, y1, dy1, st2)
            tsc, fused = None, None
            dz1 = slot.buf("g.b%d.dz1" % b, xin.shape)
            if blk.sc is not None:
                rec_wgrad(P, "b%d.sc.wgrad" % b, a0, d_out, blk.sc, fp.grad_phys(pre + "shortcut.0.weight"))
                fused = fuse_shortcut(dy1, dz1, blk.conv1, d_out, blk.sc)
                if fused is None:
                    tsc = slot.buf("g.b%d.tsc" % b, xin.shape)
                    rec_conv(P, "b%d.sc.dgrad" % b, d_out, tsc, blk.sc, 1)
            rec_wgrad(P, "b%d.c1.wgrad" % b, a0, dy1, blk.conv1, fp.grad_phys(pre + "conv1.weight"))
            self._dgrad_norm(P, slot, "g." + blk.bn1.prefix, dy1, dz1, blk.conv1, xin, st1, group_stride=0,
                             slope=0.0, gamma=blk.bn1.gamma, dgamma=fp.grad_phys(pre + "bn1.weight"),
                             dbeta=fp.grad_phys(pre + "bn1.bias"), add_pre=tsc, shortcut=fused)
            dxin = slot.buf("g.b%d.dx" % b, xin.shape)
            self._bwd_apply(P, slot, "g." + blk.bn1.prefix, dz1, xin, dxin, st1,
                            add=None if blk.sc is not None else d_out)
            d_out = dxin
            if b in (6, 4, 2):
                P.mark(fp.offsets[pre + "bn1.weight"][0])
        rec_wgrad(P, "stem.wgrad", self.input(slot), d_out, self.stem, fp.grad_phys("conv1.weight"), aux=False)
        P.mark(0)
        balance_wgrads(P, self.device)
        slot.plans[key] = P
        return P

    def two_loss_halves(self, slot: Slot):
        halves = getattr(slot, "two_loss_halves", None)
        if halves is None:
            assert slot.N % 2 == 0
            m = slot.N // 2
            h, x = self.head_bufs(slot), self.input(slot)
            gimg = slot.buf("g.img", (slot.N, slot.hw, slot.hw, 8))
            cells = ((h["loss"], h["correct"]),
                     (slot.buf("loss1", (1,), f32, zero=True), slot.buf("correct1", (2,), torch.int32, zero=True)))
            halves = []
            for k in range(2):
                s = Slot(slot.device, m, slot.hw)
                for name in ("logits", "dlogits", "pooled", "targets", "targets2"):
                    s.bufs[name] = h[name][k * m:(k + 1) * m]
                s.bufs["x"], s.bufs["g.img"] = x[k * m:(k + 1) * m], gimg[k * m:(k + 1) * m]
                s.bufs["loss"], s.bufs["correct"] = cells[k]
                halves.append(s)
            slot.two_loss_halves = halves
        return halves

    def _two_loss_backward(self, slot: Slot, half_weights) -> PlanSeq:
        key = "bwd.eval.tl%g,%g" % tuple(half_weights)
        if key not in slot.plans:
            slot.plans[key] = PlanSeq("%s.%s" % (type(self).__name__, key),
                                      [self.backward_eval_plan(s, float(w)) for s, w in zip(self.two_loss_halves(slot),
                                                                                            half_weights)])
        return slot.plans[key]

    def backward_eval_plan(self, slot: Slot, loss_weight: float, head_done: bool = False, half_weights=None,
                           stop_before: Optional[int] = None) -> Plan:
        if half_weights is not None:
            assert not head_done and stop_before is None
            return self._two_loss_backward(slot, half_weights)
        key = "bwd.eval.%g%s" % (loss_weight, ".hd" if head_done else "")
        if stop_before is not None:
            if not 0 <= int(stop_before) < len(self.blocks):
                raise ValueError("stop_before: block %s outside 0..%d" % (stop_before, len(self.blocks) - 1))
            stop_before = int(stop_before)
            key += ".sb%d" % stop_before
        if key in slot.plans:
            return slot.plans[key]
        P = Plan("preact." + key)
        n = slot.N
        h = self.head_bufs(slot)
        feat = slot.bufs["b%d.out" % (len(self.blocks) - 1)]
        d_out = slot.buf("g.feat", feat.shape)
        if not head_done:
            P.add("head_bwd", lib.combat_head_bwd, None, n, slot.feat_hw, feat.shape[-1], self.lin_w.data_ptr(),
                  self.classes, h["logits"].data_ptr(), h["targets"].data_ptr(), loss_weight, h["dlogits"].data_ptr(),
                  d_out.data_ptr(), None, None)
        for b in reversed(range(len(self.blocks))):
            blk = self.blocks[b]
            xact = slot.bufs["stem.act"] if b == 0 else slot.bufs["b%d.act" % (b - 1)]
            a1 = slot.bufs["b%d.a1" % b]
            dy1 = slot.buf("g.b%d.dy1" % b, a1.shape)
            rec_conv(P, "b%d.c2.dgrad" % b, d_out, dy1, blk.conv2, 1, mask_x=a1, mask=blk.bn2.eval_affine(),
                     mask_mul_scale=True, mask_activated=True)
            tsc, fused = None, None
            dxin = slot.buf("g.b%d.dx" % b, xact.shape)
            if blk.sc is not None:
                fused = fuse_shortcut(dy1, dxin, blk.conv1, d_out, blk.sc)
                if fused is None:
                    tsc = slot.buf("g.b%d.tsc" % b, xact.shape)
                    rec_conv(P, "b%d.sc.dgrad" % b, d_out, tsc, blk.sc, 1)
            rec_conv(P, "b%d.c1.dgrad" % b, dy1, dxin, blk.conv1, 1, shortcut=fused, add_pre=tsc, mask_x=xact,
                     mask=blk.bn1.eval_affine(), mask_mul_scale=True, mask_activated=True,
                     add_post=None if blk.sc is not None else d_out)
            d_out = dxin
            if b == stop_before:
                slot.plans[key] = P
                return P
        gimg = slot.buf("g.img", (n, slot.hw, slot.hw, 8))
        rec_conv(P, "stem.dgrad", d_out, gimg, self.stem, 1)
        slot.plans[key] = P
        return P


class ResNetEngine(PreActEngine):

    def __init__(self, module):
        NetEngine.__init__(self, module)
        m = module
        self.classes = m.linear.out_features
        self.stem = self._pc(m.conv1.weight.data, 1, 1, 8, dup=True)
        self.bn0 = _BN(self, m.bn1, "bn1")
        self.blocks: List[_Blk] = []
        self.bns: List[_BN] = [self.bn0]
        for li in range(1, 5):
            for bi, blk in enumerate(getattr(m, "layer%d" % li)):
                e = _Blk()
                e.prefix = "layer%d.%d." % (li, bi)
                e.stride, e.cin, e.planes = blk.stride, blk.conv1.in_channels, blk.conv1.out_channels
                e.bn1, e.bn2 = _BN(self, blk.bn1, e.prefix + "bn1"), _BN(self, blk.bn2, e.prefix + "bn2")
                e.conv1 = self._pc(blk.conv1.weight.data, blk.stride, 1, e.cin)
                e.conv2 = self._pc(blk.conv2.weight.data, 1, 1, e.planes)
                e.conv2e = self._pc(blk.conv2.weight.data, 1, 1, e.planes, row_scale=e.bn2.escale)
                e.sc = e.sce = e.bns = None
                if len(blk.shortcut):
                    e.bns = _BN(self, blk.shortcut[1], e.prefix + "shortcut.1")
                    e.sc = self._pc(blk.shortcut[0].weight.data, blk.stride, 0, e.cin)
                    e.sce = self._pc(blk.shortcut[0].weight.data, blk.stride, 0, e.cin, row_scale=e.bns.escale)
                    self.bns.append(e.bns)
                self.blocks.append(e)
                self.bns += [e.bn1, e.bn2]
        self.lin_w, self.lin_b = m.linear.weight.data, m.linear.bias.data
        self.ones = torch.ones(512, dtype=f32, device=self.device)
        self.zeros = torch.zeros(512, dtype=f32, device=self.device)

    def refresh(self) -> None:
        if not self.weights_dirty:
            return
        self.fold_bn()
        self._pack_all()
        self.weights_dirty = False

    FWD_SHARED = ("stem.a", "logits", "dlogits", "pooled", "targets", "targets2") + tuple(
        "b%d.%s" % (b, s) for b in range(8) for s in ("a1", "out", "scv"))

    def _block_in(self, slot: Slot, b: int):
        return slot.bufs["stem.a"] if b == 0 else slot.bufs["b%d.out" % (b - 1)]

    def _forward_eval_body(self, P: Plan, slot: Slot, x):
        n, hw = slot.N, slot.hw
        cur = slot.buf("stem.a", (n, hw, hw, 64))
        rec_conv(P, "stem", x, None, self.stem, 0, act_dst=cur, act=self.bn0.eval_affine())
        relu = Affine(self.ones, self.zeros, 0, True, 0.0)
        chw = hw
        for b, blk in enumerate(self.blocks):
            ohw = chw // blk.stride
            shape = (n, ohw, ohw, blk.planes)
            a1 = slot.buf("b%d.a1" % b, shape)
            rec_conv(P, "b%d.c1" % b, cur, None, blk.conv1, 0, act_dst=a1, act=blk.bn1.eval_affine())
            if blk.sc is not None:
                resid = slot.buf("b%d.scv" % b, shape)
                rec_conv(P, "b%d.sc" % b, cur, resid, blk.sce, 0, bias=blk.bns.eshift)
                P.merge_convs(len(P.calls) - 2)
            else:
                resid = cur
            out = slot.buf("b%d.out" % b, shape)
            rec_conv(P, "b%d.c2" % b, a1, None, blk.conv2e, 0, bias=blk.bn2.eshift, add_post=resid, act_dst=out, act=relu)
            cur, chw = out, ohw
        return cur, chw

    def _norm_add_act(self, plan: Plan, st: NormState, act_dst, add, add_scale, add_shift):
        q = st.pending
        st.pending = None
        x = q["x"]
        plan.hold(x, act_dst, q["part"], add, add_scale, add_shift)
        plan.add(q["key"] + ".finaddact", lib.combat_norm_add_act_fused, x.data_ptr(), _p(q["part"]), st.groups, q["rpg"],
                 q["pxg"], st.C, 1e-5, 0.0, _p(q["gamma"]), _p(q["beta"]), st.mean.data_ptr(), st.rstd.data_ptr(),
                 st.scale.data_ptr(), st.shift.data_ptr(), _p(q["rm"]), _p(q["rv"]), 0.1, _p(q["nbt"]),
                 self._scratch.data_ptr(), self._scratch.numel() * 4, add.data_ptr(), _p(add_scale), _p(add_shift),
                 act_dst.data_ptr())

    def _forward_train_body(self, P: Plan, slot: Slot, x):
        n, hw = slot.N, slot.hw
        bnk = lambda bn: dict(gamma=bn.gamma, beta=bn.beta, running=(bn.rm, bn.rv, bn.nbt))
        y0 = slot.buf("stem", (n, hw, hw, 64))
        cur = slot.buf("stem.a", y0.shape)
        self._conv_norm(P, slot, self.bn0.prefix, x, y0, self.stem, groups=1, act_dst=cur, **bnk(self.bn0))
        chw = hw
        for b, blk in enumerate(self.blocks):
            ohw = chw // blk.stride
            shape = (n, ohw, ohw, blk.planes)
            y1, a1 = slot.buf("b%d.y1" % b, shape), slot.buf("b%d.a1" % b, shape)
            self._conv_norm(P, slot, blk.bn1.prefix, cur, y1, blk.conv1, groups=1, act_dst=a1, **bnk(blk.bn1))
            y2 = slot.buf("b%d.y2" % b, shape)
            st2 = self._conv_norm(P, slot, blk.bn2.prefix, a1, y2, blk.conv2, groups=1, defer=True, **bnk(blk.bn2))
            out = slot.buf("b%d.out" % b, shape)
            if blk.sc is not None:
                ys = slot.buf("b%d.ys" % b, shape)
                sts = self._conv_norm(P, slot, blk.bns.prefix, cur, ys, blk.sc, groups=1, **bnk(blk.bns))
                self._norm_add_act(P, st2, out, ys, sts.scale, sts.shift)
            else:
                self._norm_add_act(P, st2, out, cur, None, None)
            cur, chw = out, ohw
        return cur, chw

    def _head_grad(self, P: Plan, slot: Slot, loss_weight: float, train: bool):
        fp, n = self.fp, slot.N
        h = self.head_bufs(slot)
        feat = slot.bufs["b%d.out" % (len(self.blocks) - 1)]
        d_feat = slot.buf("g.feat", feat.shape)
        P.add("head_bwd", lib.combat_head_bwd, h["pooled"].data_ptr() if train else None, n, slot.feat_hw, feat.shape[-1],
              self.lin_w.data_ptr(), self.classes, h["logits"].data_ptr(), h["targets"].data_ptr(), loss_weight,
              h["dlogits"].data_ptr(), d_feat.data_ptr(), fp.grad_phys("linear.weight").data_ptr() if train else None,
              fp.grad_phys("linear.bias").data_ptr() if train else None)
        d_out = slot.buf("g.feat.m", feat.shape)
        P.add("head_bwd.relu", lib.combat_relu_mask, d_feat.data_ptr(), feat.data_ptr(), feat.numel(), d_out.data_ptr())
        return d_out

    def backward_train_plan(self, slot: Slot, loss_weight: float = 1.0) -> Plan:
        key = "bwd.train.%g" % loss_weight
        if key in slot.plans:
            return slot.plans[key]
        P = Plan("resnet." + key)
        P.flush_at_marks = self.flush_at_marks
        fp = self.fp
        G = lambda name, like: slot.buf("g." + name, like.shape)
        P.add("zero_grad", _zero_grad_call, fp)
        d_out = self._head_grad(P, slot, loss_weight, True)

        def bn_bwd(bn, key_, dz, x_pre, name):
            st = slot.norm[bn.prefix]
            st.bpending = dict(part=None, rpg=0, gamma=bn.gamma, dgamma=fp.grad_phys(bn.prefix + ".weight"),
                               dbeta=fp.grad_phys(bn.prefix + ".bias"))
            dx = G(name, x_pre)
            self._bwd_apply(P, slot, key_, dz, x_pre, dx, st)
            return dx

        for b in reversed(range(len(self.blocks))):
            blk, pre = self.blocks[b], self.blocks[b].prefix
            cur_in = self._block_in(slot, b)
            y1, a1, y2 = slot.bufs["b%d.y1" % b], slot.bufs["b%d.a1" % b], slot.bufs["b%d.y2" % b]
            dy2 = bn_bwd(blk.bn2, "g." + blk.bn2.prefix, d_out, y2, "b%d.dy2" % b)
            tsc, dys = None, None
            if blk.sc is not None:
                dys = bn_bwd(blk.bns, "g." + blk.bns.prefix, d_out, slot.bufs["b%d.ys" % b], "b%d.dys" % b)
                rec_wgrad(P, "b%d.sc.wgrad" % b, cur_in, dys, blk.sc, fp.grad_phys(pre + "shortcut.0.weight"))
            rec_wgrad(P, "b%d.c2.wgrad" % b, a1, dy2, blk.conv2, fp.grad_phys(pre + "conv2.weight"))
            st1 = slot.norm[blk.bn1.prefix]
            dz1 = G("b%d.dz1" % b, y1)
            self._dgrad_norm(P, slot, "g." + blk.bn1.prefix, dy2, dz1, blk.conv2, y1, st1, group_stride=0, slope=0.0,
                             gamma=blk.bn1.gamma, dgamma=fp.grad_phys(pre + "bn1.weight"),
                             dbeta=fp.grad_phys(pre + "bn1.bias"))
            dy1 = G("b%d.dy1" % b, y1)
            self._bwd_apply(P, slot, "g." + blk.bn1.prefix, dz1, y1, dy1, st1)
            rec_wgrad(P, "b%d.c1.wgrad" % b, cur_in, dy1, blk.conv1, fp.grad_phys(pre + "conv1.weight"))
            dxin = G("b%d.dx" % b, cur_in) if b > 0 else None
            fused = None
            if blk.sc is not None:
                fused = fuse_shortcut(dy1, dxin, blk.conv1, dys, blk.sc) if b > 0 else None
                if fused is None:
                    tsc = G("b%d.tsc" % b, cur_in)
                    rec_conv(P, "b%d.sc.dgrad" % b, dys, tsc, blk.sc, 1)
            other = (None if fused is not None else tsc) if blk.sc is not None else d_out
            if b > 0:
                rec_conv(P, "b%d.c1.dgrad" % b, dy1, dxin, blk.conv1, 1, shortcut=fused, add_pre=other, mask_x=cur_in,
                         mask_activated=True)
                d_out = dxin
                if b in (6, 4, 2):
                    P.mark(fp.offsets[pre + "conv1.weight"][0])
            else:
                y0, st0 = slot.bufs["stem"], slot.norm[self.bn0.prefix]
                dz0 = G("stem.dz", y0)
                self._dgrad_norm(P, slot, "g." + self.bn0.prefix, dy1, dz0, blk.conv1, y0, st0, group_stride=0, slope=0.0,
                                 gamma=self.bn0.gamma, dgamma=fp.grad_phys("bn1.weight"), dbeta=fp.grad_phys("bn1.bias"),
                                 add_pre=other)
                dy0 = G("stem.dy", y0)
                self._bwd_apply(P, slot, "g." + self.bn0.prefix, dz0, y0, dy0, st0)
                rec_wgrad(P, "stem.wgrad", self.input(slot), dy0, self.stem, fp.grad_phys("conv1.weight"), aux=False)
        P.mark(0)
        slot.plans[key] = P
        return P

    def backward_eval_plan(self, slot: Slot, loss_weight: float, half_weights=None) -> Plan:
        if half_weights is not None:
            return self._two_loss_backward(slot, half_weights)
        key = "bwd.eval.%g" % loss_weight
        if key in slot.plans:
            return slot.plans[key]
        P = Plan("resnet." + key)
        n = slot.N
        d_out = self._head_grad(P, slot, loss_weight, False)
        for b in reversed(range(len(self.blocks))):
            blk = self.blocks[b]
            cur_in, a1 = self._block_in(slot, b), slot.bufs["b%d.a1" % b]
            dy1 = slot.buf("g.b%d.dy1" % b, a1.shape)
            rec_conv(P, "b%d.c2.dgrad" % b, d_out, dy1, blk.conv2e, 1, mask_x=a1, mask=blk.bn1.eval_affine(),
                     mask_mul_scale=True, mask_activated=True)
            other, fused = d_out, None
            dxin = slot.buf("g.b%d.dx" % b, cur_in.shape)
            if blk.sc is not None:
                fused = fuse_shortcut(dy1, dxin, blk.conv1, d_out, blk.sce) if b > 0 else None
                other = None
                if fused is None:
                    other = slot.buf("g.b%d.tsc" % b, cur_in.shape)
                    rec_conv(P, "b%d.sc.dgrad" % b, d_out, other, blk.sce, 1)
            if b > 0:
                rec_conv(P, "b%d.c1.dgrad" % b, dy1, dxin, blk.conv1, 1, shortcut=fused, add_pre=other, mask_x=cur_in,
                         mask_activated=True)
            else:
                rec_conv(P, "b%d.c1.dgrad" % b, dy1, dxin, blk.conv1, 1, add_pre=other, mask_x=cur_in,
                         mask=self.bn0.eval_affine(), mask_mul_scale=True, mask_activated=True)
            d_out = dxin
        gimg = slot.buf("g.img", (n, slot.hw, slot.hw, 8))
        rec_conv(P, "stem.dgrad", d_out, gimg, self.stem, 1)
        slot.plans[key] = P
# ... 502 lines not shown
```

combat_amd/ops.py:

```python
from __future__ import annotations

import ctypes
from dataclasses import dataclass
from typing import Optional

import torch

from . import _lib
from ._lib import ConvArgs, WgradArgs, check, lib

bf16 = torch.bfloat16


def _p(t: Optional[torch.Tensor]):
    return None if t is None else t.data_ptr()


def _stream():
    return torch.cuda.current_stream().cuda_stream


def _round_up(v: int, m: int) -> int:
    return (v + m - 1) // m * m


def rows_pad(n: int) -> int:
    return 16 if n <= 16 else _round_up(n, 128)


@dataclass
class Affine:

    scale: Optional[torch.Tensor] = None
    shift: Optional[torch.Tensor] = None
    group_stride: int = 0
    act: bool = False
    slope: float = 0.0


class PackedConv:

    def __init__(self, weight: torch.Tensor, stride: int, pad: int, c_in_padded: int, dup_hilo: bool = False,
                 need_dgrad: bool = True, row_scale: Optional[torch.Tensor] = None):
        k, c_real, r, s = weight.shape
        self.row_scale = row_scale
        assert r == s
        self.weight = weight
        self.K, self.c_real, self.R, self.stride, self.pad = k, c_real, r, stride, pad
        self.C = c_in_padded
        self.Kc = _round_up(k, 8)
        self.dup_hilo = dup_hilo
        self.taps = r * s
        dev = weight.device
        self.rows_f, self.kpad_f = rows_pad(self.Kc), _round_up(self.taps * self.C, 64)
        self.wf = torch.empty(self.rows_f, self.kpad_f, dtype=bf16, device=dev)
        self.wd = None
        self.rows_d = self.kpad_d = 0
        if need_dgrad:
            self.rows_d, self.kpad_d = rows_pad(self.C), _round_up(self.taps * self.Kc, 64)
            self.wd = torch.empty(self.rows_d, self.kpad_d, dtype=bf16, device=dev)

    def master(self) -> torch.Tensor:
        w = self.weight.detach()
        return w.permute(0, 2, 3, 1).contiguous() if not w.permute(0, 2, 3, 1).is_contiguous() else w.permute(0, 2, 3, 1)

    def fill_desc(self, d, master: torch.Tensor) -> None:
        d.w, d.wf, d.wd = master.data_ptr(), self.wf.data_ptr(), (self.wd.data_ptr() if self.wd is not None else None)
        d.K, d.taps, d.c_real, d.C, d.dup_hilo = self.K, self.taps, self.c_real, self.C, int(self.dup_hilo)
        d.rows_pad_f, d.kpad_f = self.rows_f, self.kpad_f
        d.rows_pad_d, d.kpad_d = (self.rows_d, self.kpad_d) if self.wd is not None else (0, 0)
        d.row_scale = _p(self.row_scale)

    def pack(self) -> None:
        w = self.master()
        if self.row_scale is not None:
            from ._lib import PackDesc
            tab = (PackDesc * 1)()
            self.fill_desc(tab[0], w)
            dtab = torch.frombuffer(bytearray(bytes(tab)), dtype=torch.uint8).to(self.weight.device)
            check(lib.combat_pack_weights_batch(dtab.data_ptr(), 1, _stream()), "combat_pack_weights_batch")
            torch.cuda.current_stream().synchronize()
            return
        check(lib.combat_pack_weights(w.data_ptr(), self.K, self.taps, self.c_real, self.C, int(self.dup_hilo),
                                      self.wf.data_ptr(), self.rows_f, self.kpad_f, _p(self.wd), self.rows_d,
                                      self.kpad_d, _stream()),
              "combat_pack_weights", "K=%d C=%d taps=%d" % (self.K, self.C, self.taps))

    def out_hw(self, h: int, w: int):
        return ((h + 2 * self.pad - self.R) // self.stride + 1, (w + 2 * self.pad - self.R) // self.stride + 1)


def conv_args(src, dst, pc: PackedConv, mode: int, *, pro: Optional[Affine] = None, bias=None, add_pre=None,
              mask_x=None, mask: Optional[Affine] = None, mask_mul_scale=False, add_post=None, tanh_out=False,
              stats_kind=0, stats=None, xh_mean=None, xh_rstd=None, tile=0, act_dst=None,
              act: Optional[Affine] = None, mask_activated=False, workspace=None, shortcut=None,
              pro_act_dst=None) -> ConvArgs:
    a = ConvArgs()
    a.N, a.H, a.W, a.C = src.shape
    _, a.P, a.Q, a.K = (dst if dst is not None else act_dst).shape
    a.R = a.S = pc.R
    a.stride, a.pad, a.mode = pc.stride, pc.pad, mode
    a.src, a.dst = src.data_ptr(), _p(dst)
    if act_dst is not None:
        assert act is not None and act.group_stride == 0
        a.act_dst, a.act_scale, a.act_shift, a.act_slope = act_dst.data_ptr(), _p(act.scale), _p(act.shift), act.slope
    a.mask_activated = int(mask_activated)
    if mode == 0:
        a.wpack, a.kpad, a.rows_pad = pc.wf.data_ptr(), pc.kpad_f, pc.rows_f
    else:
        a.wpack, a.kpad, a.rows_pad = pc.wd.data_ptr(), pc.kpad_d, pc.rows_d
    if pro is not None:
        a.pro_scale, a.pro_shift = _p(pro.scale), _p(pro.shift)
        a.pro_group_stride, a.pro_act, a.pro_slope = pro.group_stride, int(pro.act), pro.slope
    if pro_act_dst is not None:
        assert pro is not None and tuple(pro_act_dst.shape) == tuple(src.shape)
        a.pro_act_dst = pro_act_dst.data_ptr()
    a.bias, a.add_pre, a.mask_x, a.add_post = _p(bias), _p(add_pre), _p(mask_x), _p(add_post)
    if mask is not None:
        a.mask_scale, a.mask_shift = _p(mask.scale), _p(mask.shift)
        a.mask_group_stride, a.mask_slope = mask.group_stride, mask.slope
    a.mask_mul_scale = int(mask_mul_scale)
    a.tanh_out = int(tanh_out)
    a.stats_kind, a.stats = stats_kind, _p(stats)
    a.xh_mean, a.xh_rstd = _p(xh_mean), _p(xh_rstd)
    a.tile = tile
    if shortcut is not None:
        src2, pc2 = shortcut
        assert mode == 1 and tuple(src2.shape) == tuple(src.shape)
        a.src2, a.wpack2, a.kpad2, a.rows_pad2 = src2.data_ptr(), pc2.wd.data_ptr(), pc2.kpad_d, pc2.rows_d
    if workspace is not None:
        need = int(lib.combat_conv_workspace_bytes(ctypes.byref(a)))
        if 0 < need <= workspace.numel() * workspace.element_size():
            a.workspace, a.workspace_bytes = workspace.data_ptr(), workspace.numel() * workspace.element_size()
    a._keepalive = (src, dst, pc, pro, bias, add_pre, mask_x, mask, add_post, stats, xh_mean, xh_rstd, act_dst, act,
                    workspace, shortcut, pro_act_dst)
    return a


def shortcut_fusable(dy, dx, pc: PackedConv, pc_sc: PackedConv) -> bool:
    if pc_sc.R != 1 or pc_sc.stride != 2 or pc_sc.wd is None:
        return False
    a = conv_args(dy, dx, pc, 1, shortcut=(dy, pc_sc))
    return lib.combat_conv_pick_tile(ctypes.byref(a)) > 0


def conv_tile_granule(a: ConvArgs):
    tile = lib.combat_conv_pick_tile(ctypes.byref(a))
    return tile, lib.combat_conv_stats_granule(tile)


def conv_stats_layout(a: ConvArgs):
    rows, rpi = ctypes.c_int32(0), ctypes.c_int32(0)
    check(lib.combat_conv_stats_layout(ctypes.byref(a), ctypes.byref(rows), ctypes.byref(rpi)),
          "combat_conv_stats_layout")
    return rows.value, rpi.value


def conv_launch(a: ConvArgs) -> None:
    check(lib.combat_conv_gemm(ctypes.byref(a), _stream()), "combat_conv_gemm",
          "mode=%d src=%dx%dx%dx%d dst=%dx%dx%d R=%d stride=%d" % (a.mode, a.N, a.H, a.W, a.C, a.P, a.Q, a.K, a.R,
                                                                   a.stride))


def conv_wgrad(src, dy, pc: PackedConv, dw, *, pro: Optional[Affine] = None, split=0, workspace=None) -> None:
    a = WgradArgs()
    a.N, a.H, a.W, a.C = src.shape
    _, a.P, a.Q, a.K = dy.shape
    a.R = a.S = pc.R
    a.stride, a.pad = pc.stride, pc.pad
    a.src, a.dy, a.dw, a.k_real, a.c_real = src.data_ptr(), dy.data_ptr(), dw.data_ptr(), pc.K, pc.c_real
    if pro is not None:
        a.pro_scale, a.pro_shift = _p(pro.scale), _p(pro.shift)
        a.pro_group_stride, a.pro_act, a.pro_slope = pro.group_stride, int(pro.act), pro.slope
    a.split = split
    if workspace is True:
        nbytes = int(lib.combat_conv_wgrad_workspace_bytes(ctypes.byref(a)))
        workspace = torch.empty(max(nbytes, 4), dtype=torch.uint8, device=src.device) if nbytes else None
    if workspace is not None:
        a.workspace, a.workspace_bytes = workspace.data_ptr(), workspace.numel() * workspace.element_size()
    check(lib.combat_conv_wgrad(ctypes.byref(a), _stream()), "combat_conv_wgrad",
          "src=%s dy=%s" % (tuple(src.shape), tuple(dy.shape)))


def norm_scratch_bytes(groups: int, c: int) -> int:
    return int(lib.combat_norm_scratch_bytes(groups, c))


def norm_finalize(partials, groups, rows_per_group, c, count, *, eps=1e-5, gamma=None, beta=None, mean=None,
                  rstd=None, scale=None, shift=None, running_mean=None, running_var=None, momentum=0.1, nbt=None,
                  scratch=None) -> None:
    check(lib.combat_norm_finalize(partials.data_ptr(), groups, rows_per_group, c, float(count), eps, _p(gamma),
                                   _p(beta), _p(mean), _p(rstd), _p(scale), _p(shift), _p(running_mean),
                                   _p(running_var), momentum, _p(nbt), _p(scratch),
                                   0 if scratch is None else scratch.numel() * scratch.element_size(), _stream()),
          "combat_norm_finalize", "groups=%d rows=%d C=%d" % (groups, rows_per_group, c))


def norm_bwd_finalize(partials, groups, rows_per_group, c, count, *, gamma, mean, rstd, ca, cb, cc, dgamma=None,
                      dbeta=None, scratch=None) -> None:
    check(lib.combat_norm_bwd_finalize(partials.data_ptr(), groups, rows_per_group, c, float(count), _p(gamma),
                                       mean.data_ptr(), rstd.data_ptr(), ca.data_ptr(), cb.data_ptr(), cc.data_ptr(),
                                       _p(dgamma), _p(dbeta), _p(scratch),
                                       0 if scratch is None else scratch.numel() * scratch.element_size(), _stream()),
          "combat_norm_bwd_finalize", "groups=%d rows=%d C=%d" % (groups, rows_per_group, c))


def bn_eval_fold(gamma, beta, rm, rv, scale, shift, eps=1e-5) -> None:
    check(lib.combat_bn_eval_fold(gamma.data_ptr(), beta.data_ptr(), rm.data_ptr(), rv.data_ptr(), eps,
                                  gamma.numel(), scale.data_ptr(), shift.data_ptr(), _stream()), "combat_bn_eval_fold")


def group_stats(x, parts, rows_per_part, partials) -> None:
    check(lib.combat_group_stats(x.data_ptr(), parts, rows_per_part, x.shape[-1], partials.data_ptr(), _stream()),
          "combat_group_stats", "parts=%d rows=%d C=%d" % (parts, rows_per_part, x.shape[-1]))


def group_stats_bwd(dz, x, parts, rows_per_part, parts_per_image, xh_mean, xh_rstd, partials) -> None:
    check(lib.combat_group_stats_bwd(dz.data_ptr(), x.data_ptr(), parts, rows_per_part, x.shape[-1], parts_per_image,
                                     xh_mean.data_ptr(), xh_rstd.data_ptr(), partials.data_ptr(), _stream()),
          "combat_group_stats_bwd", "parts=%d rows=%d C=%d" % (parts, rows_per_part, x.shape[-1]))


def norm_bwd_apply(dz, x, dx, ca, cb, cc, *, rows_per_group=0, add=None) -> None:
    c = x.shape[-1]
    rows = x.numel() // c
    check(lib.combat_norm_bwd_apply(dz.data_ptr(), x.data_ptr(), _p(add), dx.data_ptr(), rows, c, rows_per_group,
                                    int(rows_per_group > 0), ca.data_ptr(), cb.data_ptr(), cc.data_ptr(), _stream()),
          "combat_norm_bwd_apply", "rows=%d C=%d" % (rows, c))


def unet_up_fwd(y, sy, ty, out, skip=None, ss=None, ts=None) -> None:
    n, h, w, c = y.shape
    check(lib.combat_unet_up_fwd(y.data_ptr(), sy.data_ptr(), ty.data_ptr(), _p(skip), _p(ss), _p(ts), n, h, w, c,
                                 out.data_ptr(), _stream()), "combat_unet_up_fwd", str(tuple(y.shape)))


def unet_up_bwd(d_out, out, du) -> None:
    n, h, w, c = du.shape
    check(lib.combat_unet_up_bwd(d_out.data_ptr(), out.data_ptr(), n, h, w, c, du.data_ptr(), _stream()),
          "combat_unet_up_bwd", str(tuple(du.shape)))


def trigger_fwd(x, noise, p_mat, k1, noise_rate, out, out_c8=None, mse_partial=None, src_index=None) -> None:
    hw = x.shape[2]
    n = x.shape[0] if src_index is None else src_index.numel()
    check(lib.combat_trigger_fwd(x.data_ptr(), noise.data_ptr(), p_mat.data_ptr(), k1.data_ptr(), noise_rate, n, hw,
                                 _p(src_index), out.data_ptr(), _p(out_c8), _p(mse_partial), _stream()),
          "combat_trigger_fwd", str(tuple(x.shape)))


def trigger_bwd(x, noise, p_mat, k1, noise_rate, d_out, out, l2_scale, d_noise, pre_tanh=False, d_out2=None) -> None:
    n, _, hw, _ = x.shape
    check(lib.combat_trigger_bwd(x.data_ptr(), noise.data_ptr(), p_mat.data_ptr(), k1.data_ptr(), noise_rate, n, hw,
                                 _p(d_out), _p(d_out2), _p(out), l2_scale, int(pre_tanh), d_noise.data_ptr(), _stream()),
          "combat_trigger_bwd", str(tuple(x.shape)))


def trigger_tv_fwd(x, noise, p_mat, k1, noise_rate, out, tv_partial, mse_partial=None) -> None:
    n, _, hw, _ = x.shape
    check(lib.combat_trigger_tv_fwd(x.data_ptr(), noise.data_ptr(), p_mat.data_ptr(), k1.data_ptr(), noise_rate, n, hw,
                                    out.data_ptr(), _p(mse_partial), tv_partial.data_ptr(), _stream()),
          "combat_trigger_tv_fwd", str(tuple(x.shape)))


def trigger_tv_bwd(x, noise, p_mat, k1, noise_rate, d_out, out, l2_scale, tv_scale, d_noise, pre_tanh=False,
                   d_out2=None) -> None:
    n, _, hw, _ = x.shape
    check(lib.combat_trigger_tv_bwd(x.data_ptr(), noise.data_ptr(), p_mat.data_ptr(), k1.data_ptr(), noise_rate, n, hw,
                                    _p(d_out), _p(d_out2), _p(out), l2_scale, tv_scale, int(pre_tanh), d_noise.data_ptr(),
                                    _stream()),
          "combat_trigger_tv_bwd", str(tuple(x.shape)))


def trigger_pair_fwd(x, noise, p_mat, k1, noise_rate, out_bd, out_cross, mse_partial=None) -> None:
    n, _, hw, _ = x.shape
    check(lib.combat_trigger_pair_fwd(x.data_ptr(), noise.data_ptr(), p_mat.data_ptr(), k1.data_ptr(), noise_rate, n, hw,
                                      out_bd.data_ptr(), out_cross.data_ptr(), _p(mse_partial), _stream()),
          "combat_trigger_pair_fwd", str(tuple(x.shape)))


def trigger_pair_bwd(x, noise, p_mat, k1, noise_rate, d_bd, out_bd, l2_scale, d_cross, d_noise, pre_tanh=False,
                     d_bd2=None) -> None:
    n, _, hw, _ = x.shape
    check(lib.combat_trigger_pair_bwd(x.data_ptr(), noise.data_ptr(), p_mat.data_ptr(), k1.data_ptr(), noise_rate, n, hw,
                                      _p(d_bd), _p(d_bd2), _p(out_bd), l2_scale, _p(d_cross), int(pre_tanh),
                                      d_noise.data_ptr(), _stream()),
          "combat_trigger_pair_bwd", str(tuple(x.shape)))


def trigger_groups_fwd(x, noise, p_mat, k1, ps, noise_rate, out, mse_partial=None) -> None:
    n, _, hw, _ = x.shape
    if ps < 1 or k1.dtype != torch.float32 or k1.numel() < 3 * ((n + ps - 1) // max(ps, 1)) or not k1.is_contiguous():
        raise ValueError("trigger_groups_fwd: k1 must be contiguous fp32 [ceil(%d / ps)][3] with ps >= 1, got ps = %d, %s %s"
                         % (n, ps, k1.dtype, tuple(k1.shape)))
    check(lib.combat_trigger_groups_fwd(x.data_ptr(), noise.data_ptr(), p_mat.data_ptr(), k1.data_ptr(), noise_rate, n, hw,
                                        ps, out.data_ptr(), _p(mse_partial), _stream()),
          "combat_trigger_groups_fwd", "%s ps=%d" % (tuple(x.shape), ps))


def trigger_groups_bwd(x, noise, p_mat, k1, ps, noise_rate, d_out, out, l2_scale, d_noise, pre_tanh=False, d_out2=None) -> None:
    n, _, hw, _ = x.shape
    if ps < 1 or k1.dtype != torch.float32 or k1.numel() < 3 * ((n + ps - 1) // max(ps, 1)) or not k1.is_contiguous():
        raise ValueError("trigger_groups_bwd: k1 must be contiguous fp32 [ceil(%d / ps)][3] with ps >= 1, got ps = %d, %s %s"
                         % (n, ps, k1.dtype, tuple(k1.shape)))
    check(lib.combat_trigger_groups_bwd(x.data_ptr(), noise.data_ptr(), p_mat.data_ptr(), k1.data_ptr(), noise_rate, n, hw,
                                        ps, _p(d_out), _p(d_out2), _p(out), l2_scale, int(pre_tanh), d_noise.data_ptr(),
                                        _stream()),
          "combat_trigger_groups_bwd", "%s ps=%d" % (tuple(x.shape), ps))


def _cond_shapes(what, w, labels, nf, classes, n):
    if w.dtype != torch.float32 or tuple(w.shape) != (nf, 9, nf + classes) or not w.is_contiguous():
        raise ValueError("%s: the weight (or its gradient) must be contiguous fp32 [%d][9][%d], got %s %s"
                         % (what, nf, nf + classes, w.dtype, tuple(w.shape)))
    if labels.dtype != torch.int32 or labels.dim() != 1 or labels.numel() < n or not labels.is_contiguous():
        raise ValueError("%s: labels must be int32 [>= %d], got %s %s" % (what, n, labels.dtype, tuple(labels.shape)))


def cond_fwd(w, labels, classes, cond) -> None:
    n, s, s2, nf = cond.shape
    _cond_shapes("cond_fwd", w, labels, nf, classes, n)
    if cond.dtype != bf16 or s != s2 or not cond.is_contiguous():
        raise ValueError("cond_fwd: cond must be contiguous bf16 [n][s][s][nf], got %s %s" % (cond.dtype, tuple(cond.shape)))
    check(lib.combat_cond_fwd(w.data_ptr() + 4 * nf, labels.data_ptr(), n, s, nf, classes, cond.data_ptr(), _stream()),
          "combat_cond_fwd", "n=%d hw_map=%d nf=%d classes=%d" % (n, s, nf, classes))


def cond_wgrad(d, labels, classes, dw, scratch, dwf=None) -> None:
    n, s, s2, nf = d.shape
    _cond_shapes("cond_wgrad", dw, labels, nf, classes, n)
    if d.dtype != bf16 or s != s2 or not d.is_contiguous():
        raise ValueError("cond_wgrad: d must be contiguous bf16 [n][s][s][nf], got %s %s" % (d.dtype, tuple(d.shape)))
    if scratch.dtype != torch.float32 or scratch.numel() < n * 9 * nf or not scratch.is_contiguous():
        raise ValueError("cond_wgrad: scratch must be contiguous fp32 with at least %d elements" % (n * 9 * nf))
    if dwf is not None and (dwf.dtype != torch.float32 or dwf.numel() != nf * 9 * nf or not dwf.is_contiguous()):
        raise ValueError("cond_wgrad: dwf must be contiguous fp32 [%d][9][%d]" % (nf, nf))
    check(lib.combat_cond_wgrad(d.data_ptr(), labels.data_ptr(), n, s, nf, classes, _p(dwf), dw.data_ptr(), scratch.data_ptr(),
                                _stream()),
          "combat_cond_wgrad", "n=%d hw_map=%d nf=%d classes=%d" % (n, s, nf, classes))


def augment_fwd(x, n, hw, out_c8, params=None, index=None, out_f32=None) -> None:
    check(lib.combat_augment_fwd(x.data_ptr(), _p(index), _p(params), n, hw, out_c8.data_ptr(), _p(out_f32),
                                 _stream()), "combat_augment_fwd", "n=%d hw=%d" % (n, hw))


def augment_bwd(d_c8, n, hw, d_x, params=None, accumulate=False) -> None:
    check(lib.combat_augment_bwd(d_c8.data_ptr(), d_c8.shape[-1], _p(params), n, hw, d_x.data_ptr(),
                                 int(accumulate), _stream()),
          "combat_augment_bwd", "n=%d hw=%d" % (n, hw))


def head_fwd(feat, weight, bias, logits, *, targets=None, loss_weight=1.0, pooled=None, loss_sum=None, correct=None,
             targets2=None, correct2=None) -> None:
    n, hw, _, c = feat.shape
    check(lib.combat_head_fwd(feat.data_ptr(), n, hw, c, weight.data_ptr(), bias.data_ptr(), weight.shape[0],
                              _p(targets), loss_weight, _p(pooled), logits.data_ptr(), _p(loss_sum), _p(correct),
                              _p(targets2), _p(correct2), _stream()), "combat_head_fwd", str(tuple(feat.shape)))


def head_bwd(pooled, n, hw, c, weight, logits, targets, loss_weight, dlogits, d_feat=None, dw=None, db=None) -> None:
    check(lib.combat_head_bwd(_p(pooled), n, hw, c, weight.data_ptr(), weight.shape[0], logits.data_ptr(),
                              targets.data_ptr(), loss_weight, dlogits.data_ptr(), _p(d_feat), _p(dw), _p(db),
                              _stream()), "combat_head_bwd", "n=%d hw=%d C=%d" % (n, hw, c))


def prune_sweep(pooled, weight, bias, order, per, targets, correct, targets2=None, correct2=None) -> None:
    n, c = pooled.shape[0], order.numel()
    check(lib.combat_prune_sweep(pooled.data_ptr(), n, weight.data_ptr(), bias.data_ptr(), order.data_ptr(), c, per,
                                 weight.shape[0], _p(targets), _p(targets2), _p(correct), _p(correct2), _stream()),
          "combat_prune_sweep", "n=%d C=%d per=%d classes=%d" % (n, c, per, weight.shape[0]))


def feature_colsum(pooled, acc) -> None:
    n, fin = pooled.shape
    check(lib.combat_feature_colsum(pooled.data_ptr(), n, fin, acc.data_ptr(), _stream()), "combat_feature_colsum",
          "n=%d in=%d" % (n, fin))


def strip_superimpose(backgrounds, dataset, index, norm_cols, out_c8) -> None:
    b, hw = backgrounds.shape[0], backgrounds.shape[1]
    s = index.shape[1]
    if out_c8.shape[0] < b * s or tuple(out_c8.shape[1:]) != (hw, hw, 8) or tuple(dataset.shape[1:]) != (hw, hw, 3):
        raise ValueError("strip_superimpose: out_c8 %s / dataset %s do not hold %d x %d blends of %d x %d pixels"
                         % (tuple(out_c8.shape), tuple(dataset.shape), b, s, hw, hw))
    check(lib.combat_strip_superimpose(backgrounds.data_ptr(), b, dataset.data_ptr(), dataset.shape[0], index.data_ptr(),
                                       s, hw, norm_cols, out_c8.data_ptr(), _stream()),
          "combat_strip_superimpose", "B=%d S=%d hw=%d norm_cols=%d" % (b, s, hw, norm_cols))


def strip_entropy(logits, b, s, out) -> None:
    check(lib.combat_strip_entropy(logits.data_ptr(), b, s, logits.shape[1], out.data_ptr(), _stream()),
          "combat_strip_entropy", "B=%d S=%d classes=%d" % (b, s, logits.shape[1]))


def _nc_shapes(what, dataset, index, hw, mask_tanh, pattern_tanh, image_buf, n):
    if tuple(dataset.shape[1:]) != (hw, hw, 3) or dataset.dtype != torch.uint8 or index.dtype != torch.int32:
        raise ValueError("%s: dataset must be uint8 [n][%d][%d][3] and index int32, got %s %s / %s"
                         % (what, hw, hw, dataset.dtype, tuple(dataset.shape), index.dtype))
    if mask_tanh.numel() != hw * hw or pattern_tanh.numel() != 3 * hw * hw or mask_tanh.dtype != torch.float32 \
            or pattern_tanh.dtype != torch.float32:
        raise ValueError("%s: mask_tanh / pattern_tanh must be fp32 [%d][%d] / [3][%d][%d]" % (what, hw, hw, hw, hw))
    if image_buf.dim() != 4 or tuple(image_buf.shape[1:]) != (hw, hw, 8) or image_buf.dtype != bf16 or n > image_buf.shape[0]:
        raise ValueError("%s: the c8 buffer %s does not hold %d images of %d x %d pixels" % (what, tuple(image_buf.shape), n, hw, hw))


def nc_blend_args(dataset, index, cursor, bs, n, mask_tanh, pattern_tanh, epsilon, norm, out_c8):
    hw = out_c8.shape[1]
    _nc_shapes("nc_blend", dataset, index, hw, mask_tanh, pattern_tanh, out_c8, n)
    if norm.numel() != 6 or norm.dtype != torch.float32 or cursor.dtype != torch.int32:
        raise ValueError("nc_blend: norm must be fp32 [6] (mean, std) and cursor int32 [1]")
    return (dataset.data_ptr(), dataset.shape[0], index.data_ptr(), index.numel(), cursor.data_ptr(), bs, n, out_c8.shape[0], hw,
            mask_tanh.data_ptr(), pattern_tanh.data_ptr(), epsilon, norm.data_ptr(), out_c8.data_ptr())


def nc_blend(dataset, index, cursor, bs, n, mask_tanh, pattern_tanh, epsilon, norm, out_c8) -> None:
    args = nc_blend_args(dataset, index, cursor, bs, n, mask_tanh, pattern_tanh, epsilon, norm, out_c8)
    check(lib.combat_nc_blend(*args, _stream()), "combat_nc_blend", "n=%d N=%d hw=%d bs=%d" % (n, out_c8.shape[0], out_c8.shape[1], bs))


def nc_update_args(g_img, dataset, index, cursor, bs, n, logits, target_label, mask_tanh, pattern_tanh, exp_avg, exp_avg_sq,
                   epsilon, norm, lr, beta1, beta2, adam_eps, t, cost, stats, grad_out=None):
    hw = g_img.shape[1]
    _nc_shapes("nc_update", dataset, index, hw, mask_tanh, pattern_tanh, g_img, n)
    for name, v in (("exp_avg", exp_avg), ("exp_avg_sq", exp_avg_sq), ("grad_out", grad_out)):
        if v is not None and (v.numel() != 4 * hw * hw or v.dtype != torch.float32):
            raise ValueError("nc_update: %s must be fp32 [4][%d][%d]" % (name, hw, hw))
    if logits.dim() != 2 or logits.shape[0] < n or logits.dtype != torch.float32 or stats.dim() != 2 or stats.shape[1] != 4 \
            or stats.dtype != torch.float32:
        raise ValueError("nc_update: logits must be fp32 [>= n][classes] and stats fp32 [steps][4]")
    if norm.numel() != 6 or norm.dtype != torch.float32 or cursor.dtype != torch.int32 or t.dtype != torch.int32 \
            or cost.dtype != torch.float32:
        raise ValueError("nc_update: norm must be fp32 [6], cursor and t int32 [1], cost fp32 [1]")
    return (g_img.data_ptr(), dataset.data_ptr(), dataset.shape[0], index.data_ptr(), index.numel(), cursor.data_ptr(), bs, n,
            g_img.shape[0], hw, logits.data_ptr(), logits.shape[1], target_label, mask_tanh.data_ptr(), pattern_tanh.data_ptr(),
            exp_avg.data_ptr(), exp_avg_sq.data_ptr(), epsilon, norm.data_ptr(), lr, beta1, beta2, adam_eps, t.data_ptr(),
            cost.data_ptr(), stats.data_ptr(), stats.shape[0], _p(grad_out))


def nc_update(g_img, dataset, index, cursor, bs, n, logits, target_label, mask_tanh, pattern_tanh, exp_avg, exp_avg_sq,
              epsilon, norm, lr, beta1, beta2, adam_eps, t, cost, stats, grad_out=None) -> None:
    args = nc_update_args(g_img, dataset, index, cursor, bs, n, logits, target_label, mask_tanh, pattern_tanh, exp_avg,
                          exp_avg_sq, epsilon, norm, lr, beta1, beta2, adam_eps, t, cost, stats, grad_out)
    check(lib.combat_nc_update(*args, _stream()), "combat_nc_update",
          "n=%d N=%d hw=%d classes=%d target=%d" % (n, g_img.shape[0], g_img.shape[1], logits.shape[1], target_label))


def gradcam_seed(logits, index, n, weight, chosen, d_feat) -> None:
    N, classes = logits.shape
    c = weight.shape[1]
    if logits.dtype != torch.float32 or weight.dtype != torch.float32 or weight.shape[0] != classes or not weight.is_contiguous():
        raise ValueError("gradcam_seed: logits must be fp32 [N][classes] and weight fp32 [classes][C], got %s %s / %s %s"
                         % (logits.dtype, tuple(logits.shape), weight.dtype, tuple(weight.shape)))
    if chosen.dtype != torch.int32 or chosen.numel() < N or d_feat.dtype != bf16 or tuple(d_feat.shape) != (N, 4, 4, c):
        raise ValueError("gradcam_seed: chosen must be int32 [N = %d] and d_feat bf16 [%d][4][4][%d], got %s %s / %s %s"
                         % (N, N, c, chosen.dtype, tuple(chosen.shape), d_feat.dtype, tuple(d_feat.shape)))
    if index is not None and (index.dtype != torch.int32 or index.numel() < n):
        raise ValueError("gradcam_seed: index must be int32 [>= n = %d], got %s %s" % (n, index.dtype, tuple(index.shape)))
    check(lib.combat_gradcam_seed(logits.data_ptr(), _p(index), n, N, classes, c, weight.data_ptr(), chosen.data_ptr(),
                                  d_feat.data_ptr(), _stream()),
          "combat_gradcam_seed", "n=%d N=%d classes=%d C=%d" % (n, N, classes, c))


def gradcam_map(act, grad, n, cam, raw=None, weights=None) -> None:
    if act.dim() != 4 or act.shape != grad.shape or act.dtype != bf16 or grad.dtype != bf16 or act.shape[1] != act.shape[2] \
            or act.shape[0] < n or not act.is_contiguous() or not grad.is_contiguous():
        raise ValueError("gradcam_map: act and grad must be contiguous bf16 [>= n = %d][f][f][C] of one shape, got %s %s / %s %s"
                         % (n, act.dtype, tuple(act.shape), grad.dtype, tuple(grad.shape)))
    f, c = act.shape[1], act.shape[3]
    for name, v, size in (("cam", cam, n * 32 * 32), ("raw", raw, n * f * f), ("weights", weights, n * c)):
        if v is not None and (v.dtype != torch.float32 or v.numel() < size or not v.is_contiguous()):
            raise ValueError("gradcam_map: %s must be contiguous fp32 with at least %d elements, got %s %s"
                             % (name, size, v.dtype, tuple(v.shape)))
    check(lib.combat_gradcam_map(act.data_ptr(), grad.data_ptr(), n, f, c, 32, cam.data_ptr(), _p(raw), _p(weights), _stream()),
          "combat_gradcam_map", "n=%d f=%d C=%d" % (n, f, c))


def sgd_nesterov(ptrs, sizes, count, max_size, lr, momentum, weight_decay, grad_scale, first_step) -> None:
    check(lib.combat_sgd_nesterov(ptrs.data_ptr(), sizes.data_ptr(), count, max_size, lr, momentum, weight_decay,
                                  grad_scale, int(first_step), _stream()), "combat_sgd_nesterov", "count=%d" % count)


def image_to_c8(x, out_c8) -> None:
    n, _, hw, _ = x.shape
    check(lib.combat_image_to_c8(x.data_ptr(), n, hw, out_c8.data_ptr(), _stream()), "combat_image_to_c8")

# ... 39 lines not shown
```

include/combat_hip.h:

```cpp
#ifndef COMBAT_HIP_H
#define COMBAT_HIP_H

#include <stdint.h>

#ifdef __cplusplus
extern "C" {
#endif

#define COMBAT_OK 0
#define COMBAT_EINVAL (-1)
#define COMBAT_ELAUNCH (-2)

const char *combat_version(void);
int combat_abi_version(void);

void combat_set_deterministic(int on);
int combat_get_deterministic(void);

typedef struct combat_conv_args {
    int32_t N, H, W, C;
    int32_t P, Q, K;
    int32_t R, S, stride, pad;
    int32_t mode;
    const void *src;
    const void *wpack;
    int32_t kpad;
    int32_t rows_pad;
    void *dst;
    const float *pro_scale, *pro_shift;
    int32_t pro_group_stride;
    int32_t pro_act;
    float pro_slope;
    const float *bias;
    const void *add_pre;
    const void *mask_x;
    const float *mask_scale, *mask_shift;
    int32_t mask_activated;
    int32_t mask_group_stride;
    float mask_slope;
    int32_t mask_mul_scale;
    const void *add_post;
    int32_t tanh_out;
    int32_t stats_kind;
    float *stats;
    const float *xh_mean, *xh_rstd;
    void *act_dst;
    const float *act_scale, *act_shift;
    float act_slope;
    void *workspace;
    int64_t workspace_bytes;
    int32_t tile;
    const void *src2, *wpack2;
    int32_t kpad2, rows_pad2;
    void *pro_act_dst;
} combat_conv_args;

#define COMBAT_STATS_PER_WORKGROUP 4
#define COMBAT_TILE_128x128 1
#define COMBAT_TILE_128x64 2
#define COMBAT_TILE_64x64 3
#define COMBAT_TILE_128x16 4
#define COMBAT_TILE_64x128 5
#define COMBAT_TILE_H256x64 6
#define COMBAT_TILE_H128x128 7
#define COMBAT_TILE_H128x64 8
#define COMBAT_TILE_H64x64 9
#define COMBAT_TILE_D128x64 10
#define COMBAT_TILE_D128x32 11
#define COMBAT_TILE_G128x64 12
#define COMBAT_TILE_G128x32 13
#define COMBAT_TILE_D256x64 14
#define COMBAT_TILE_C8 15
#define COMBAT_TILE_S128x64 17
#define COMBAT_TILE_K8 18
#define COMBAT_TILE_D256W64 16

int combat_conv_gemm(const combat_conv_args *a, void *stream);
int combat_conv_gemm_pair(const combat_conv_args *a, const combat_conv_args *b, void *stream);
int64_t combat_conv_workspace_bytes(const combat_conv_args *a);
int combat_conv_pick_tile(const combat_conv_args *a);
int combat_conv_stats_granule(int tile);
int combat_conv_stats_layout(const combat_conv_args *a, int32_t *rows, int32_t *rows_per_image);

typedef struct combat_wgrad_args {
    int32_t N, H, W, C;
    int32_t P, Q, K;
    int32_t R, S, stride, pad;
    const void *src;
    const void *dy;
    float *dw;
    int32_t k_real;
    int32_t c_real;
    const float *pro_scale, *pro_shift;
    int32_t pro_group_stride;
    int32_t pro_act;
    float pro_slope;
    int32_t split;
    void *workspace;
    int64_t workspace_bytes;
    int32_t defer_reduce;
    int32_t reserved;
    const struct combat_wgrad_args *reduce_first;
} combat_wgrad_args;

int combat_conv_wgrad(const combat_wgrad_args *a, void *stream);
int combat_conv_wgrad_reduce(const combat_wgrad_args *a, void *stream);
int64_t combat_conv_wgrad_workspace_bytes(const combat_wgrad_args *a);

int combat_pack_weights(const float *w, int32_t K, int32_t taps, int32_t c_real, int32_t C, int32_t dup_hilo,
                        void *wf, int32_t rows_pad_f, int32_t kpad_f,
                        void *wd, int32_t rows_pad_d, int32_t kpad_d, void *stream);
typedef struct combat_pack_desc {
    const float *w;
    void *wf, *wd;
    int32_t K, taps, c_real, C, dup_hilo, rows_pad_f, kpad_f, rows_pad_d, kpad_d;
    int32_t reserved;
    const float *row_scale;
} combat_pack_desc;
int combat_pack_weights_batch(const combat_pack_desc *descs, int32_t n, void *stream);

int combat_norm_finalize(const float *partials, int32_t groups, int32_t rows_per_group, int32_t C,
                         float count, float eps, const float *gamma, const float *beta,
                         float *mean, float *rstd, float *scale, float *shift,
                         float *running_mean, float *running_var, float momentum,
                         int64_t *num_batches_tracked, float *scratch, int64_t scratch_bytes, void *stream);
int64_t combat_norm_scratch_bytes(int32_t groups, int32_t C);

int combat_bn_eval_fold(const float *gamma, const float *beta, const float *running_mean,
                        const float *running_var, float eps, int32_t C, float *scale, float *shift,
                        void *stream);
typedef struct combat_bn_desc {
    const float *gamma, *beta, *running_mean, *running_var;
    float *scale, *shift;
    int32_t C, reserved;
} combat_bn_desc;
int combat_bn_eval_fold_batch(const combat_bn_desc *descs, int32_t n, float eps, void *stream);

int combat_group_stats(const void *x, int32_t groups, int32_t rows_per_group, int32_t C,
                       float *partials, void *stream);

int combat_norm_bwd_finalize(const float *partials, int32_t groups, int32_t rows_per_group, int32_t C,
                             float count, const float *gamma, const float *mean, const float *rstd,
                             float *ca, float *cb, float *cc, float *dgamma, float *dbeta,
                             float *scratch, int64_t scratch_bytes, void *stream);

int combat_norm_bwd_apply(const void *dz, const void *x, const void *add, void *dx, int64_t rows,
                          int32_t C, int32_t rows_per_group, int32_t grouped,
                          const float *ca, const float *cb, const float *cc, void *stream);

int combat_norm_act_fused(const void *x, const float *partials, int32_t groups, int32_t rows_per_group,
                          int64_t px_per_group, int32_t C, float eps, float slope, const float *gamma,
                          const float *beta, float *mean, float *rstd, float *scale, float *shift,
                          float *running_mean, float *running_var, float momentum, int64_t *num_batches_tracked,
                          float *scratch, int64_t scratch_bytes, void *act, void *stream);
int combat_norm_add_act_fused(const void *x, const float *partials, int32_t groups, int32_t rows_per_group,
                              int64_t px_per_group, int32_t C, float eps, float slope, const float *gamma,
                              const float *beta, float *mean, float *rstd, float *scale, float *shift,
                              float *running_mean, float *running_var, float momentum,
                              int64_t *num_batches_tracked, float *scratch, int64_t scratch_bytes, const void *add,
                              const float *add_scale, const float *add_shift, void *act, void *stream);
int combat_norm_bwd_fused(const void *dz, const void *x, const void *add, const float *partials, int32_t groups,
                          int32_t rows_per_group, int64_t px_per_group, int32_t C, const float *gamma,
                          const float *mean, const float *rstd, float *dgamma, float *dbeta, float *scratch,
                          int64_t scratch_bytes, void *dx, void *stream);

int combat_group_stats_bwd(const void *dz, const void *x, int32_t groups, int32_t rows_per_group,
                           int32_t C, int32_t parts_per_image, const float *xh_mean, const float *xh_rstd,
                           float *partials, void *stream);

int combat_unet_up_fwd(const void *y, const float *sy, const float *ty, const void *s, const float *ss,
                       const float *ts, int32_t N, int32_t H, int32_t W, int32_t C, void *out, void *stream);
int combat_unet_up_bwd(const void *d_out, const void *out, int32_t N, int32_t H, int32_t W, int32_t C,
                       void *du, void *stream);
int combat_unet_up_bwd_fused(const void *d_out, const void *out, const void *y, const float *mean, const float *rstd,
                             int32_t N, int32_t H, int32_t W, int32_t C, void *du, void *dx, void *stream);
int combat_unet_up_fused(const void *y, const float *partials, int32_t rows_per_group, const void *s,
                         const float *ss, const float *ts, int32_t N, int32_t H, int32_t W, int32_t C, float eps,
                         float *mean, float *rstd, float *scale, float *shift, void *out, void *stream);

int combat_trigger_fwd(const float *x, const void *noise, const float *P, const float *k1, float noise_rate,
                       int32_t n, int32_t hw, const int32_t *src_index ,
                       float *out, void *out_c8, float *mse_partial, void *stream);
int combat_trigger_bwd(const float *x, const void *noise, const float *P, const float *k1, float noise_rate,
                       int32_t n, int32_t hw, const float *d_out, const float *d_out2 ,
                       const float *out, float l2_scale, int32_t pre_tanh, void *d_noise, void *stream);
int combat_trigger_pair_fwd(const float *x, const void *noise, const float *P, const float *k1, float noise_rate,
                            int32_t n, int32_t hw, float *out_bd, float *out_cross, float *mse_partial, void *stream);
int combat_trigger_pair_bwd(const float *x, const void *noise, const float *P, const float *k1, float noise_rate,
                            int32_t n, int32_t hw, const float *d_bd, const float *d_bd2 ,
                            const float *out_bd, float l2_scale, const float *d_cross , int32_t pre_tanh,
                            void *d_noise, void *stream);

int combat_trigger_groups_fwd(const float *x, const void *noise, const float *P, const float *k1, float noise_rate,
                              int32_t n, int32_t hw, int32_t ps, float *out, float *mse_partial, void *stream);
int combat_trigger_groups_bwd(const float *x, const void *noise, const float *P, const float *k1, float noise_rate,
                              int32_t n, int32_t hw, int32_t ps, const float *d_out,
                              const float *d_out2 , const float *out, float l2_scale,
                              int32_t pre_tanh, void *d_noise, void *stream);

int combat_cond_fwd(const float *W_y, const int32_t *labels, int32_t n, int32_t hw_map, int32_t nf, int32_t num_classes,
                    void *cond_out, void *stream);
int combat_cond_wgrad(const void *d, const int32_t *labels, int32_t n, int32_t hw_map, int32_t nf, int32_t num_classes,
                      const float *dwf, float *dw, float *scratch, void *stream);

int combat_trigger_tv_fwd(const float *x, const void *noise, const float *P, const float *k1, float noise_rate,
                          int32_t n, int32_t hw, float *out, float *mse_partial , float *tv_partial,
                          void *stream);
int combat_trigger_tv_bwd(const float *x, const void *noise, const float *P, const float *k1, float noise_rate,
                          int32_t n, int32_t hw, const float *d_out, const float *d_out2 ,
                          const float *out, float l2_scale, float tv_scale, int32_t pre_tanh, void *d_noise,
                          void *stream);

int combat_augment_fwd(const float *x, const int32_t *src_index, const float *params, int32_t n, int32_t hw,
                       void *out_c8, float *out_f32, void *stream);
int combat_augment_bwd(const void *d_c8, int32_t c8_channels, const float *params, int32_t n, int32_t hw,
                       float *d_x, int32_t accumulate, void *stream);

int combat_head_fwd(const void *feat, int32_t n, int32_t hw, int32_t C, const float *W, const float *b,
                    int32_t classes, const int64_t *targets, float loss_weight, float *pooled, float *logits,
                    float *loss_sum, int32_t *correct, const int64_t *targets2, int32_t *correct2,
                    void *stream);
int combat_head_bwd(const float *pooled, int32_t n, int32_t hw, int32_t C, const float *W, int32_t classes,
                    const float *logits, const int64_t *targets, float loss_weight, float *dlogits,
                    void *d_feat, float *dW, float *db, void *stream);
int combat_head_fwd_bwd(const void *feat, int32_t n, int32_t hw, int32_t C, const float *W, const float *b,
                        int32_t classes, const int64_t *targets, float loss_weight, float *pooled, float *logits,
                        float *loss_sum, int32_t *correct, const int64_t *targets2, int32_t *correct2,
                        float *dlogits, void *d_feat, void *stream);
int combat_head_bwd_weights(const float *dlogits, const float *pooled, int32_t n, int32_t hw, int32_t C,
                            int32_t classes, float *dW, float *db, void *stream);

int combat_prune_sweep(const float *pooled, int32_t n, const float *W, const float *b, const int32_t *order, int32_t C,
                       int32_t per, int32_t classes, const int64_t *targets, const int64_t *targets2, int32_t *correct,
                       int32_t *correct2, void *stream);
int combat_feature_colsum(const float *pooled, int32_t n, int32_t in, double *acc, void *stream);

int combat_strip_superimpose(const void *backgrounds, int32_t B, const void *dataset, int32_t n_data, const int32_t *index,
                             int32_t S, int32_t hw, int32_t norm_cols, void *out_c8, void *stream);
int combat_strip_entropy(const float *logits, int32_t B, int32_t S, int32_t classes, float *out, void *stream);

int combat_nc_blend(const void *dataset, int32_t n_data, const int32_t *index, int32_t n_index, const int32_t *cursor,
                    int32_t bs, int32_t n, int32_t N, int32_t hw, const float *mask_tanh, const float *pattern_tanh,
                    float epsilon, const float *norm, void *out_c8, void *stream);
int combat_nc_update(const void *g_img, const void *dataset, int32_t n_data, const int32_t *index, int32_t n_index,
                     int32_t *cursor, int32_t bs, int32_t n, int32_t N, int32_t hw, const float *logits, int32_t classes,
                     int32_t target_label, float *mask_tanh, float *pattern_tanh, float *exp_avg, float *exp_avg_sq,
                     float epsilon, const float *norm, float lr, float beta1, float beta2, float adam_eps, int32_t *t,
                     const float *cost, float *stats, int32_t steps, float *grad_out, void *stream);

int combat_gradcam_seed(const float *logits, const int32_t *index, int32_t n, int32_t N, int32_t classes, int32_t C,
                        const float *W, int32_t *chosen, void *d_feat, void *stream);
int combat_gradcam_map(const void *act, const void *grad, int32_t n, int32_t f, int32_t C, int32_t out_hw, float *cam,
                       float *raw, float *weights, void *stream);

int combat_sgd_nesterov(const void *ptrs, const int64_t *sizes, int32_t count, int64_t max_size, float lr,
                        float momentum, float weight_decay, float grad_scale, int32_t first_step,
                        void *stream);

int combat_image_to_c8(const float *x, int32_t n, int32_t hw, void *out_c8, void *stream);
int combat_nhwc_to_nchw_f32(const void *x, int32_t n, int32_t h, int32_t w, int32_t C, int32_t c, float *out,
                            void *stream);
int combat_nchw_to_nhwc_bf16(const float *x, int32_t n, int32_t c, int32_t h, int32_t w, int32_t C, void *out,
                             void *stream);
int combat_relu_mask(const void *g, const void *act, int64_t elements, void *out, void *stream);
int combat_memset_zero(void *ptr, int64_t bytes, void *stream);
int combat_copy3(void *dst0, const void *src0, int64_t bytes0, void *dst1, const void *src1, int64_t bytes1,
                 void *dst2, const void *src2, int64_t bytes2, void *stream);
int combat_colsum(const void *x, int64_t rows, int32_t C, int32_t c_out, float *out, void *stream);
int combat_log_terms(const float *x, const float *xb, const float *mse_partial, int32_t n, int32_t hw,
                     const float *detector_logits, double *acc2, double *hits, void *stream);
int combat_log_terms_tv(const float *x, const float *xb, const float *mse_partial, const float *tv_partial, int32_t n,
                        int32_t hw, const float *detector_logits, double *acc3, double *hits, void *stream);
int combat_maxpool2(const void *x, int32_t n, int32_t h, int32_t w, int32_t C, void *out, void *stream);
int combat_elu_affine(const void *x, int64_t rows, int32_t C, const float *scale, const float *shift, void *out,
                      void *stream);
int combat_affine_act(const void *x, int64_t rows, int32_t C, const float *scale, const float *shift,
                      int64_t group_rows, float slope, void *out, void *stream);
int combat_dct_u8(const float *x, const float *D, int32_t n, int32_t hw, void *out_c8, void *stream);
int combat_linear_nhwc(const void *x, int32_t n, int32_t h, int32_t w, int32_t C, const float *W, const float *b,
                       int32_t classes, float *logits, void *stream);

int combat_grid_head_fwd(const float *fc1_bias, const float *fc2_weight, const float *fc2_bias, int32_t nf, int32_t nout,
                         float *field, void *stream);
int combat_wanet_grid(const float *field, const float *U, int32_t S, int32_t H, float rescale, float *noise_grid, float *grid,
                      void *stream);
int combat_warp_fwd(const float *x, const int32_t *src_index, const float *grid, int32_t per_image_grid, int32_t n, int32_t H,
                    float *out, void *stream);
int combat_warp_bwd(const float *x, const float *d_out, const float *d_out2, const float *grid, int32_t per_image_grid,
                    int32_t n, int32_t H, int32_t groups, float *partial, void *stream);
int combat_warp_bwd_input(const float *d_out, const float *grid, int32_t per_image_grid, int32_t n, int32_t H, float *d_x,
                          void *stream);
int combat_wanet_field_bwd(const float *partial, int32_t groups, const float *noise_grid, const float *U, int32_t S, int32_t H,
                           float rescale, float l2_scale, const float *field, const float *fc1_bias, const float *fc2_weight,
                           int32_t nf, float *d_fc1_bias, float *d_fc2_weight, float *d_fc2_bias, float *d_field,
                           void *stream);

typedef struct combat_plan combat_plan;
combat_plan *combat_plan_create(void);
void combat_plan_destroy(combat_plan *plan);
int combat_plan_record(combat_plan *plan, int32_t queue);
int combat_plan_set_after(combat_plan *plan, int32_t call_index);
int combat_plan_record_cancel(void);
int32_t combat_plan_size(const combat_plan *plan);
int combat_plan_run(combat_plan *plan, int32_t begin, int32_t end, void *stream, void *const *aux_streams, int32_t n_aux);
int combat_plan_join(combat_plan *plan, void *stream, void *const *aux_streams, int32_t n_aux);
int32_t combat_plan_failed_call(const combat_plan *plan);

#define COMBAT_COMM_UNIQUE_ID_BYTES 128
#define COMBAT_DTYPE_F32 0
#define COMBAT_DTYPE_BF16 1
int combat_comm_unique_id(void *out128);
int combat_comm_init_rank(void **comm, int32_t nranks, const void *unique_id128, int32_t rank);
int combat_comm_destroy(void *comm);
int combat_allreduce(void *buf, int64_t count, int32_t dtype, void *comm, void *stream);

#ifdef __cplusplus
}
#endif
#endif
```

Baseline: 32740 images/sec.

## Add stride-2 DMA 3x3 wgrad path and fuse 1x1 shortcut wgrad into it

Extends the DMA-fed 3x3 weight-gradient kernel to stride-2 convolutions, using a new halo row layout that splits even and odd columns. When a PreAct block's 1x1 stride-2 shortcut shares input geometry with conv1, its weight gradient rides along in the same kernel. A second dy tile is loaded, and only the center tap's input fragments are multiplied against it. This removes a separate shortcut wgrad launch and a second read of the activation. In exchange it adds an extra DMA piece, more LDS and registers, and a separate 1-tap reduce, and it drops the reduce-first fold on the stride-2 path.

```diff
diff --git a/combat_amd/_lib.py b/combat_amd/_lib.py
--- a/combat_amd/_lib.py
+++ b/combat_amd/_lib.py
@@ -43,6 +43,7 @@
         ("workspace", c_vp), ("workspace_bytes", c_i64),
         ("defer_reduce", c_i32), ("reserved", c_i32),
         ("reduce_first", c_vp),
+        ("dy2", c_vp), ("dw2", c_vp), ("k2_real", c_i32), ("reserved2", c_i32),
     ]
 
 
@@ -74,6 +75,7 @@
     "combat_conv_wgrad": (C.c_int, [C.POINTER(WgradArgs), c_vp]),
     "combat_conv_wgrad_workspace_bytes": (c_i64, [C.POINTER(WgradArgs)]),
     "combat_conv_wgrad_reduce": (C.c_int, [C.POINTER(WgradArgs), c_vp]),
+    "combat_conv_wgrad_s2_table": (C.c_int, [C.POINTER(WgradArgs), C.POINTER(c_i32), C.POINTER(c_i32), C.POINTER(c_i32)]),
     "combat_pack_weights": (C.c_int, [c_vp, c_i32, c_i32, c_i32, c_i32, c_i32, c_vp, c_i32, c_i32, c_vp, c_i32,
                                       c_i32, c_vp]),
     "combat_norm_finalize": (C.c_int, [c_vp, c_i32, c_i32, c_i32, c_f32, c_f32, c_vp, c_vp, c_vp, c_vp, c_vp, c_vp,
diff --git a/combat_amd/csrc/capi.cpp b/combat_amd/csrc/capi.cpp
--- a/combat_amd/csrc/capi.cpp
+++ b/combat_amd/csrc/capi.cpp
@@ -7,7 +7,7 @@
 #include <mutex>
 #include <unordered_map>
 
-#define COMBAT_ABI_VERSION 20
+#define COMBAT_ABI_VERSION 21
 
 extern "C" const char *combat_version(void) { return "combat_hip gfx950 abi17"; }
 extern "C" int combat_abi_version(void) { return COMBAT_ABI_VERSION; }
diff --git a/combat_amd/csrc/conv_wgrad.hip b/combat_amd/csrc/conv_wgrad.hip
--- a/combat_amd/csrc/conv_wgrad.hip
+++ b/combat_amd/csrc/conv_wgrad.hip
@@ -602,6 +602,7 @@
         int rc = conv_wgrad3x3_dma_try(a, st);
         if (rc <= 0) return rc;
     }
+    if (a->dy2) return COMBAT_EINVAL;
     if (a->reduce_first) {
         const int rc = combat_conv_wgrad_reduce(a->reduce_first, stream);
         if (rc != COMBAT_OK) return rc;
diff --git a/combat_amd/csrc/conv_wgrad3x3_dma.hip b/combat_amd/csrc/conv_wgrad3x3_dma.hip
--- a/combat_amd/csrc/conv_wgrad3x3_dma.hip
+++ b/combat_amd/csrc/conv_wgrad3x3_dma.hip
@@ -16,6 +16,7 @@
     float *red_dw;
     int red_base, red_tiles_c, red_split, red_k_real, red_c_real, red_pad;
     unsigned long long *stamps;
+    float *ws2;
 };
 
 #ifdef COMBAT_STAMPS
@@ -42,6 +43,28 @@
 }
 __device__ __forceinline__ int dkey(int pk) { return ((pk >> 1) & 1) | (((pk >> 3) & 1) << 1); }
 
+struct S2Geo { int TW, TH, TI, HWP, HH, HROWS; };
+__host__ __device__ inline int s2_col(int HWP, int hx) { return (hx & 1) ? (HWP >> 1) + 1 + (hx >> 1) : hx >> 1; }
+__host__ __device__ inline int s2_hx(int HWP, int u) { const int ne = (HWP >> 1) + 1; return u < ne ? 2 * u : 2 * (u - ne) + 1; }
+__host__ __device__ inline int s2_key(int TW, int line, int ti, int u) {
+    if (TW == 2) return ((line >> 1) & 1) | (((ti >> 1) & 1) << 1);
+    const int b1 = TW >= 16 ? (u >> 3) & 1 : TW == 8 ? (line >> 1) & 1 : (line >> 2) & 1;
+    return ((u >> 1) & 1) | (b1 << 1);
+}
+__host__ __device__ inline bool s2_row_decode(const S2Geo &g, int row, int &ti, int &hy, int &hx, int &key) {
+    const int u = row % g.HWP, line = row / g.HWP;
+    hx = s2_hx(g.HWP, u);
+    hy = line % g.HH;
+    ti = line / g.HH;
+    key = s2_key(g.TW, line, ti, u);
+    return row < g.HROWS;
+}
+__host__ __device__ inline int s2_tap_row(const S2Geo &g, int tx, int ty, int ti, int r, int s, int &key) {
+    const int line = ti * g.HH + 2 * ty + r, u = s2_col(g.HWP, 2 * tx + s);
+    key = s2_key(g.TW, line, ti, u);
+    return line * g.HWP + u;
+}
+
 template <int N>
 __device__ __forceinline__ void wait_vm_lgkm0_barrier() {
     asm volatile("s_waitcnt vmcnt(%0) lgkmcnt(0)" ::"n"(N) : "memory");
@@ -49,12 +72,12 @@
     asm volatile("" ::: "memory");
 }
 
-template <int NT>
+template <int NT, int TAPS = 9>
 __device__ __forceinline__ void reduce_slabs(const float *__restrict__ ws, float *__restrict__ dw, int base, int tiles_c, int split,
                                              int k_real, int c_real, unsigned char *scratch, int block, int nblocks) {
     constexpr int U = 4;
     const int tid = threadIdx.x;
-    const long e4 = (long)base * 9 * 1024;
+    const long e4 = (long)base * TAPS * 1024;
     const long per = (e4 + nblocks - 1) / nblocks;
     const long q0 = (long)block * per, q1 = q0 + per < e4 ? q0 + per : e4;
     int SL = 1;
@@ -62,7 +85,7 @@
     const int QP = NT / SL, sl = tid / QP, ql = tid - sl * QP;
     const int nsl = (split - sl + SL - 1) / SL;
     f32x4_t *scr = reinterpret_cast<f32x4_t *>(scratch);
-    const size_t sstride = (size_t)base * 9 * 4096;
+    const size_t sstride = (size_t)base * TAPS * 4096;
     for (long qb = q0; qb < q1; qb += (long)QP * U) {
         f32x4_t acc[U];
         long qq[U];
@@ -99,7 +122,7 @@
             for (int u = 0; u < U; ++u) {
                 const long q = qq[u];
                 if (q >= q1) continue;
-                const int f4 = (int)(q & 1023), tap = (int)((q >> 10) % 9), tile = (int)(q / (9 * 1024));
+                const int f4 = (int)(q & 1023), tap = (int)((q >> 10) % TAPS), tile = (int)(q / (TAPS * 1024));
                 const int i = f4 >> 9, wave = (f4 >> 6) & 7, lane = f4 & 63;
                 const int row = (i * 2 + (wave & 1)) * 16 + (lane >> 4) * 4, col = (wave >> 1) * 16 + (lane & 15);
                 const int tile_c = tile % tiles_c, tile_k = tile / tiles_c;
@@ -107,7 +130,7 @@
                 if (c < c_real) {
 #pragma unroll
                     for (int e = 0; e < 4; ++e)
-                        if (n + e < k_real) dw[((size_t)(n + e) * 9 + tap) * c_real + c] += acc[u][e];
+                        if (n + e < k_real) dw[((size_t)(n + e) * TAPS + tap) * c_real + c] += acc[u][e];
                 }
             }
         }
@@ -115,7 +138,7 @@
     }
 }
 
-template <int HPW, int NS, bool RED>
+template <int HPW, int NS, bool RED, int SD = 1, bool DY2 = false>
 __device__ __forceinline__ void wgrad3x3_dma_body(const W3dParams &p) {
     extern __shared__ __attribute__((aligned(16))) unsigned char smem[];
     const combat_wgrad_args &a = p.a;
@@ -137,8 +160,9 @@
     if (t_begin >= t_end) return;
 
     const int C = a.C, K = a.K, H = a.H, W = a.W;
-    constexpr int XBYTES = HPW * 8192, DYBYTES = 64 * 128, DYBASE = NS * XBYTES;
-    constexpr int NDMA = 1 + HPW;
+    const int OH = SD == 1 ? H : a.P, OW = SD == 1 ? W : a.Q;
+    constexpr int XBYTES = HPW * 8192, DYBYTES = 64 * 128, DYBASE = NS * XBYTES, DY2BASE = DYBASE + NS * DYBYTES;
+    constexpr int NDMA = 1 + HPW + (DY2 ? 1 : 0);
     auto rsrc_words = [&](const void *ptr, unsigned bytes) __attribute__((always_inline)) {
         const unsigned long base = (unsigned long)ptr;
         u32x4_t w;
@@ -149,10 +173,12 @@
         return w;
     };
     const u32x4_t xrs = rsrc_words(a.src, p.x_bytes), dyrs = rsrc_words(a.dy, p.dy_bytes);
+    const u32x4_t dy2rs = DY2 ? rsrc_words(a.dy2, p.dy_bytes) : dyrs;
     const unsigned lds0 = __builtin_amdgcn_readfirstlane((unsigned)(unsigned long)(lds_void_t *)smem) + wid * 1024;
 #ifdef COMBAT_WGRAD_BUILTIN_DMA
     const __amdgpu_buffer_rsrc_t xrsrc = __builtin_amdgcn_make_buffer_rsrc(const_cast<void *>(a.src), 0, p.x_bytes, 0x00020000);
     const __amdgpu_buffer_rsrc_t dyrsrc = __builtin_amdgcn_make_buffer_rsrc(const_cast<void *>(a.dy), 0, p.dy_bytes, 0x00020000);
+    const __amdgpu_buffer_rsrc_t dy2rsrc = __builtin_amdgcn_make_buffer_rsrc(const_cast<void *>(DY2 ? a.dy2 : a.dy), 0, p.dy_bytes, 0x00020000);
 #define COMBAT_W3_DMA(rs_builtin, rs_words, lds_off, voff) \
     __builtin_amdgcn_raw_ptr_buffer_load_lds(rs_builtin, (lds_void_t *)(smem + (lds_off) + wid * 1024), 16, voff, 0, 0, 0)
 #else
@@ -164,11 +190,19 @@
 #pragma unroll
     for (int j = 0; j < HPW; ++j) {
         const int row = (wid + 8 * j) * 8 + (lane >> 3), slot = lane & 7;
-        const int hx = row % p.HWP, line = row / p.HWP;
-        const int hy = line % p.HH, ti = line / p.HH;
-        const int chunk = (((slot >> 1) ^ xkey(p.TW, line, hx)) << 1) | (slot & 1);
-        hdec[j] = row < p.HROWS ? (hx | (hy << 8) | (ti << 16)) : -1;
-        hrel[j] = (((ti * H + hy - 1) * W + hx - 1) * C + c0 + chunk * 8) * 2;
+        if constexpr (SD == 2) {
+            int hx, hy, ti, key;
+            s2_row_decode(S2Geo{p.TW, p.TH, p.TI, p.HWP, p.HH, p.HROWS}, row, ti, hy, hx, key);
+            const int chunk = (((slot >> 1) ^ key) << 1) | (slot & 1);
+            hdec[j] = row < p.HROWS ? (hx | (hy << 8) | (ti << 16)) : -1;
+            hrel[j] = (((ti * H + hy - 1) * W + hx - 1) * C + c0 + chunk * 8) * 2;
+        } else {
+            const int hx = row % p.HWP, line = row / p.HWP;
+            const int hy = line % p.HH, ti = line / p.HH;
+            const int chunk = (((slot >> 1) ^ xkey(p.TW, line, hx)) << 1) | (slot & 1);
+            hdec[j] = row < p.HROWS ? (hx | (hy << 8) | (ti << 16)) : -1;
+            hrel[j] = (((ti * H + hy - 1) * W + hx - 1) * C + c0 + chunk * 8) * 2;
+        }
         asm volatile("" : "+v"(hdec[j]), "+v"(hrel[j]));
     }
     int dti[1], drel[1];
@@ -178,7 +212,7 @@
         const int tx = pk & (p.TW - 1), ty = (pk >> p.tw_shift) & (p.TH - 1), ti = pk >> (p.tw_shift + p.th_shift);
         const int chunk = (((slot >> 1) ^ dkey(pk)) << 1) | (slot & 1);
         dti[j] = ti;
-        drel[j] = (((ti * H + ty) * W + tx) * K + k0 + chunk * 8) * 2;
+        drel[j] = (((ti * OH + ty) * OW + tx) * K + k0 + chunk * 8) * 2;
         asm volatile("" : "+v"(dti[j]), "+v"(drel[j]));
     }
     int nt_x, nt_y, nt_g;
@@ -191,11 +225,18 @@
     int is_img0 = 0, is_oy0 = 0, is_ox0 = 0, is_xorg = 0, is_dorg = 0;
     auto issue_prep = [&]() __attribute__((always_inline)) {
         is_img0 = nt_g * p.TI;
-        is_oy0 = nt_y * p.TH;
-        is_ox0 = nt_x * p.TW;
-        const int origin = (is_img0 * H + is_oy0) * W + is_ox0;
-        is_xorg = origin * C * 2;
-        is_dorg = origin * K * 2;
+        if constexpr (SD == 1) {
+            is_oy0 = nt_y * p.TH;
+            is_ox0 = nt_x * p.TW;
+            const int origin = (is_img0 * H + is_oy0) * W + is_ox0;
+            is_xorg = origin * C * 2;
+            is_dorg = origin * K * 2;
+        } else {
+            is_oy0 = nt_y * p.TH * SD;
+            is_ox0 = nt_x * p.TW * SD;
+            is_xorg = ((is_img0 * H + is_oy0) * W + is_ox0) * C * 2;
+            is_dorg = ((is_img0 * OH + nt_y * p.TH) * OW + nt_x * p.TW) * K * 2;
+        }
         if (++nt_x == p.tiles_x) {
             nt_x = 0;
             if (++nt_y == p.tiles_y) {
@@ -207,9 +248,9 @@
     auto issue_piece = [&](auto j_tag, auto slot_tag) __attribute__((always_inline)) {
         constexpr int j = decltype(j_tag)::value;
         constexpr int slot_i = decltype(slot_tag)::value;
-        const u32x4_t xrs_l = xrs, dyrs_l = dyrs;
+        const u32x4_t xrs_l = xrs, dyrs_l = dyrs, dy2rs_l = dy2rs;
         const unsigned lds0_l = lds0;
-        (void)xrs_l; (void)dyrs_l; (void)lds0_l;
+        (void)xrs_l; (void)dyrs_l; (void)dy2rs_l; (void)lds0_l;
         if constexpr (j == 0) {
             const unsigned off = is_img0 + dti[0] < a.N ? (unsigned)(is_dorg + drel[0]) : kOob;
             COMBAT_W3_DMA(dyrsrc, dyrs, DYBASE + slot_i * DYBYTES, off);
@@ -219,6 +260,9 @@
                             (unsigned)(is_ox0 + (d & 255) - 1) < (unsigned)W;
             const unsigned off = ok ? (unsigned)(is_xorg + hrel[j - 1]) : kOob;
             COMBAT_W3_DMA(xrsrc, xrs, slot_i * XBYTES + 8 * (j - 1) * 1024, off);
+        } else if constexpr (DY2 && j == HPW + 1) {
+            const unsigned off = is_img0 + dti[0] < a.N ? (unsigned)(is_dorg + drel[0]) : kOob;
+            COMBAT_W3_DMA(dy2rsrc, dy2rs, DY2BASE + slot_i * DYBYTES, off);
         }
     };
     auto issue = [&](auto slot_tag) __attribute__((always_inline)) {
@@ -229,11 +273,16 @@
         issue_piece(integral_constant<int, 2>{}, slot_tag);
         issue_piece(integral_constant<int, 3>{}, slot_tag);
         issue_piece(integral_constant<int, 4>{}, slot_tag);
+        issue_piece(integral_constant<int, 5>{}, slot_tag);
+        issue_piece(integral_constant<int, 6>{}, slot_tag);
+        issue_piece(integral_constant<int, 7>{}, slot_tag);
+        issue_piece(integral_constant<int, 8>{}, slot_tag);
     };
 
     const int q = (lane & 15) >> 2, pp = lane & 3, fq = lane >> 4;
-    constexpr int SPS = 65536 / XBYTES, NSETS = (NS + SPS - 1) / SPS;
+    constexpr int SPS = SD == 2 ? 65535 / XBYTES + 1 : 65536 / XBYTES, NSETS = (NS + SPS - 1) / SPS;
     const lds_u8 *const smem_l = (const lds_u8 *)smem;
+    const lds_u8 *dyp2[2][2][2];
     const lds_u8 *dyp[2][2][2], *xp[NSETS][2][2][9];
     int dya[2][2], xa[2][2][9];
 #pragma unroll
@@ -246,8 +295,14 @@
 #pragma unroll
             for (int tap = 0; tap < 9; ++tap) {
                 const int r = (tap * 11) >> 5, s = tap - 3 * r;
-                const int line = ti * p.HH + ty + r, hx = tx + s;
-                xa[ks][hi][tap] = (line * p.HWP + hx) * 128 + ((wave_c ^ xkey(p.TW, line, hx)) & 3) * 32 + pp * 8;
+                if constexpr (SD == 2) {
+                    int key;
+                    const int row = s2_tap_row(S2Geo{p.TW, p.TH, p.TI, p.HWP, p.HH, p.HROWS}, tx, ty, ti, r, s, key);
+                    xa[ks][hi][tap] = row * 128 + ((wave_c ^ key) & 3) * 32 + pp * 8;
+                } else {
+                    const int line = ti * p.HH + ty + r, hx = tx + s;
+                    xa[ks][hi][tap] = (line * p.HWP + hx) * 128 + ((wave_c ^ xkey(p.TW, line, hx)) & 3) * 32 + pp * 8;
+                }
 #pragma unroll
                 for (int set = 0; set < NSETS; ++set) {
                     xp[set][ks][hi][tap] = smem_l + set * SPS * XBYTES + xa[ks][hi][tap];
@@ -258,6 +313,10 @@
             for (int i = 0; i < 2; ++i) {
                 dyp[ks][hi][i] = smem_l + DYBASE + (dya[ks][hi] ^ (i * 64));
                 asm volatile("" : "+v"(dyp[ks][hi][i]));
+                if constexpr (DY2) {
+                    dyp2[ks][hi][i] = smem_l + DY2BASE + (dya[ks][hi] ^ (i * 64));
+                    asm volatile("" : "+v"(dyp2[ks][hi][i]));
+                }
             }
         }
 
@@ -266,6 +325,7 @@
     for (int t = 0; t < 9; ++t)
 #pragma unroll
         for (int i = 0; i < 2; ++i) acc[t][i] = f32x4_t{0.f, 0.f, 0.f, 0.f};
+    f32x4_t acc2[2] = {f32x4_t{0.f, 0.f, 0.f, 0.f}, f32x4_t{0.f, 0.f, 0.f, 0.f}};
 
     auto x_frags = [&](bf16x8_t (&fx)[2], auto slot_tag, auto tap_tag) __attribute__((always_inline)) {
         constexpr int tap = decltype(tap_tag)::value, slot = decltype(slot_tag)::value;
@@ -276,8 +336,15 @@
         __builtin_amdgcn_sched_barrier(0);
 #endif
     };
-    auto mfma_tap = [&](auto tap_tag, const bf16x8_t (&fk)[2][2], const bf16x8_t (&fx)[2]) __attribute__((always_inline)) {
+    auto mfma_tap = [&](auto tap_tag, const bf16x8_t (&fk)[2][2], const bf16x8_t (&fx)[2], const bf16x8_t (&fk2)[2][2]) __attribute__((always_inline)) {
         constexpr int tap = decltype(tap_tag)::value;
+        if constexpr (DY2 && tap == 4) {
+#pragma unroll
+            for (int ks = 0; ks < 2; ++ks)
+#pragma unroll
+                for (int i = 0; i < 2; ++i)
+                    acc2[i] = __builtin_amdgcn_mfma_f32_16x16x32_bf16(fk2[ks][i], fx[ks], acc2[i], 0, 0, 0);
+        }
 #pragma unroll
         for (int ks = 0; ks < 2; ++ks)
 #pragma unroll
@@ -302,6 +369,14 @@
 #pragma unroll
             for (int i = 0; i < 2; ++i)
                 fk[ks][i] = join8(tr16d(dyp[ks][0][i] + imm), tr16d(dyp[ks][1][i] + imm));
+        bf16x8_t fk2[2][2];
+        if constexpr (DY2) {
+#pragma unroll
+            for (int ks = 0; ks < 2; ++ks)
+#pragma unroll
+                for (int i = 0; i < 2; ++i)
+                    fk2[ks][i] = join8(tr16d(dyp2[ks][0][i] + imm), tr16d(dyp2[ks][1][i] + imm));
+        }
         using std::integral_constant;
         (void)nslot_tag;
         (void)ahead;
@@ -310,13 +385,15 @@
         __builtin_amdgcn_sched_barrier(0);
 #define COMBAT_W3_TAP(t, cur, nxt)                                                   \
         if (t < 8) x_frags(nxt, slot_tag, integral_constant<int, (t < 8 ? t + 1 : 8)>{});  \
-        mfma_tap(integral_constant<int, t>{}, fk, cur);
+        mfma_tap(integral_constant<int, t>{}, fk, cur, DY2 ? fk2 : fk);
         COMBAT_W3_TAP(0, fx0, fx1) COMBAT_W3_TAP(1, fx1, fx0) COMBAT_W3_TAP(2, fx0, fx1) COMBAT_W3_TAP(3, fx1, fx0)
         COMBAT_W3_TAP(4, fx0, fx1) COMBAT_W3_TAP(5, fx1, fx0) COMBAT_W3_TAP(6, fx0, fx1) COMBAT_W3_TAP(7, fx1, fx0)
         COMBAT_W3_TAP(8, fx0, fx1)
 #undef COMBAT_W3_TAP
     };
-    static_assert(HPW <= 4, "issue() spells out 1 + HPW <= 5 pieces");
+    static_assert(HPW <= 7, "issue() spells out 1 + HPW + 1 <= 9 pieces");
+    static_assert(!DY2 || SD == 2, "a second dy rides along in the stride-2 form only");
+    static_assert(SD == 1 || (SD == 2 && NS == 2 && !RED), "the stride-2 form: a two-stage ring (every wait a drain), no reduce-first fold");
 
     const int npatch = t_end - t_begin;
     using std::integral_constant;
@@ -362,6 +439,11 @@
 #pragma unroll
             for (int i = 0; i < 2; ++i)
                 *reinterpret_cast<f32x4_t *>(slab + tap * 4096 + ((i * 8 + wid) * 64 + lane) * 4) = acc[tap][i];
+        if constexpr (DY2) {
+#pragma unroll
+            for (int i = 0; i < 2; ++i)
+                *reinterpret_cast<f32x4_t *>(p.ws2 + (size_t)blockIdx.x * 4096 + ((i * 8 + wid) * 64 + lane) * 4) = acc2[i];
+        }
     } else {
         float *ep = reinterpret_cast<float *>(smem);
         constexpr int EPS = 68;
@@ -395,6 +477,21 @@
             }
             __syncthreads();
         }
+        if constexpr (DY2) {
+#pragma unroll
+            for (int i = 0; i < 2; ++i) {
+                const int col = wave_c * 16 + fr;
+                const int row = (i * 2 + wave_k) * 16 + fq * 4;
+#pragma unroll
+                for (int e = 0; e < 4; ++e) ep[(row + e) * EPS + col] = acc2[i][e];
+            }
+            __syncthreads();
+            for (int idx = tid; idx < 64 * 64; idx += 512) {
+                const int row = idx >> 6, col = idx & 63;
+                const int n = k0 + row, c = c0 + col;
+                if (n < a.k2_real && c < a.c_real) atomicAdd(a.dw2 + (size_t)n * a.c_real + c, ep[row * EPS + col]);
+            }
+        }
     }
 #ifdef COMBAT_STAMPS
     if (lane == 0 && p.stamps) {
@@ -405,16 +502,17 @@
 #endif
 }
 
+template <int TAPS>
 __global__ __launch_bounds__(256) void wgrad3x3_reduce_kernel(const float *__restrict__ ws, float *__restrict__ dw,
                                                               int base, int tiles_c, int split, int k_real, int c_real) {
     const long e4 = (long)blockIdx.x * 256 + threadIdx.x;
-    if (e4 >= (long)base * 9 * 1024) return;
-    const int f4 = (int)(e4 & 1023), tap = (int)((e4 >> 10) % 9), tile = (int)(e4 / (9 * 1024));
+    if (e4 >= (long)base * TAPS * 1024) return;
+    const int f4 = (int)(e4 & 1023), tap = (int)((e4 >> 10) % TAPS), tile = (int)(e4 / (TAPS * 1024));
     const int per = (split + gridDim.y - 1) / gridDim.y;
     const int s0 = blockIdx.y * per, s1 = s0 + per < split ? s0 + per : split;
     f32x4_t acc = {0.f, 0.f, 0.f, 0.f};
-    const float *src = ws + ((size_t)tile * 9 + tap) * 4096 + f4 * 4;
-    const size_t sstride = (size_t)base * 9 * 4096;
+    const float *src = ws + ((size_t)tile * TAPS + tap) * 4096 + f4 * 4;
+    const size_t sstride = (size_t)base * TAPS * 4096;
     int s = s0;
     for (; s + 4 <= s1; s += 4) {
         const f32x4_t v0 = *reinterpret_cast<const f32x4_t *>(src + (size_t)s * sstride);
@@ -432,17 +530,18 @@
 #pragma unroll
         for (int e = 0; e < 4; ++e) {
             if (n + e >= k_real) break;
-            float *o = dw + ((size_t)(n + e) * 9 + tap) * c_real + c;
+            float *o = dw + ((size_t)(n + e) * TAPS + tap) * c_real + c;
             if (gridDim.y == 1) *o += acc[e];
             else atomicAdd(o, acc[e]);
         }
     }
 }
 
+template <int TAPS>
 __global__ __launch_bounds__(256) void wgrad3x3_reduce_det_kernel(const float *__restrict__ ws, float *__restrict__ dw, int base,
                                                                   int tiles_c, int split, int k_real, int c_real) {
     __shared__ __attribute__((aligned(16))) unsigned char scratch[256 * 64];
-    reduce_slabs<256>(ws, dw, base, tiles_c, split, k_real, c_real, scratch, blockIdx.x, gridDim.x);
+    reduce_slabs<256, TAPS>(ws, dw, base, tiles_c, split, k_real, c_real, scratch, blockIdx.x, gridDim.x);
 }
 
 template <int HPW, int NS, bool RED>
@@ -470,29 +569,54 @@
     return p.red_ws ? launch_w3d_red<HPW, NS, true>(p, blocks, st) : launch_w3d_red<HPW, NS, false>(p, blocks, st);
 }
 
-bool w3d_geometry(const combat_wgrad_args *a, W3dParams &p, int &smem) {
-    if (!(a->R == 3 && a->S == 3 && a->stride == 1 && a->pad == 1 && a->P == a->H && a->Q == a->W)) return false;
+template <int HPW, bool DY2>
+__global__ __launch_bounds__(512, 1) void conv_wgrad3x3_dma_s2_kernel(const W3dParams p) { wgrad3x3_dma_body<HPW, 2, false, 2, DY2>(p); }
+
+template <int HPW, bool DY2>
+int launch_w3d_s2(const W3dParams &p, int blocks, hipStream_t st) {
+    constexpr int smem = 2 * (8192 + HPW * 8192 + (DY2 ? 8192 : 0));
+    auto kern = conv_wgrad3x3_dma_s2_kernel<HPW, DY2>;
+    static bool attr = false;
+    if (!attr) {
+        if (hipFuncSetAttribute(reinterpret_cast<const void *>(kern), hipFuncAttributeMaxDynamicSharedMemorySize, smem) != hipSuccess)
+            return COMBAT_ELAUNCH;
+        attr = true;
+    }
+    COMBAT_LAUNCH(kern, dim3(blocks), dim3(512), smem, st, p);
+    CB_LAUNCH_CHECK();
+    return COMBAT_OK;
+}
+
+bool w3d_geometry(const combat_wgrad_args *a, W3dParams &p, int &smem, bool query = false) {
+    const int SD = a->stride;
+    if (!(a->R == 3 && a->S == 3 && a->pad == 1 && (SD == 1 || SD == 2))) return false;
+    if (SD == 1 ? !(a->P == a->H && a->Q == a->W) : !(a->H == 2 * a->P && a->W == 2 * a->Q)) return false;
     if (a->pro_scale || a->pro_act) return false;
     if (a->C < 64 || (a->C & 63) || a->K < 64 || (a->K & 63) || a->c_real != a->C) return false;
-    const int W = a->W, H = a->H;
+    if (a->dy2 && (SD != 2 || !a->dw2 || a->k2_real <= 0 || a->k2_real > a->K)) return false;
+    const int W = a->Q, H = a->P;
     const int TW = W < 16 ? W : 16;
     const int TH = H < 64 / TW ? H : 64 / TW;
     const int TI = 64 / (TW * TH);
     if (TW < 2 || TI < 1 || TW * TH * TI != 64) return false;
     p.a = *a;
     p.TW = TW; p.TH = TH; p.TI = TI;
-    p.HWP = TW + 2; p.HH = TH + 2; p.HROWS = TI * p.HH * p.HWP;
+    p.HWP = SD == 1 ? TW + 2 : 2 * TW + 1; p.HH = SD == 1 ? TH + 2 : 2 * TH + 1; p.HROWS = TI * p.HH * p.HWP;
     p.hpw = (p.HROWS + 63) / 64;
     p.tw_shift = ilog2_exact(TW); p.th_shift = ilog2_exact(TH);
     if (p.tw_shift < 0 || p.th_shift < 0 || W % TW || H % TH) return false;
-    const long xb = (long)a->N * H * W * a->C * 2, db = (long)a->N * H * W * a->K * 2;
+    const long xb = (long)a->N * a->H * a->W * a->C * 2, db = (long)a->N * H * W * a->K * 2;
     if (xb >= (long)kOob || db >= (long)kOob) return false;
     p.x_bytes = (unsigned)xb; p.dy_bytes = (unsigned)db;
     p.tiles_x = W / TW; p.tiles_y = H / TH;
     p.ntiles = p.tiles_x * p.tiles_y * ((a->N + TI - 1) / TI);
     p.tiles_k = a->K / 64; p.tiles_c = a->C / 64;
     smem = 0;
-    return p.hpw >= 2 && p.hpw <= 4;
+    if (SD == 1) return p.hpw >= 2 && p.hpw <= 4;
+    if (p.hpw < 5 || p.hpw > 7) return false;
+    if (a->split > 0 || (a->dy2 && !query)) return true;
+    const int base = p.tiles_k * p.tiles_c;
+    return !combat_deterministic() && p.ntiles >= 8 * ((128 + base - 1) / base);
 }
 
 int pick_split(const combat_wgrad_args *a, const W3dParams &p, bool with_ws) {
@@ -519,7 +643,7 @@
     int smem;
     if (!w3d_geometry(a, p, smem)) return 0;
     const int split = pick_split(a, p, true);
-    return split > 1 ? (long)split * p.tiles_k * p.tiles_c * 9 * 4096 * 4 : 0;
+    return split > 1 ? (long)split * p.tiles_k * p.tiles_c * (9 + (a->dy2 ? 1 : 0)) * 4096 * 4 : 0;
 }
 
 namespace {
@@ -528,39 +652,46 @@
     if (!w3d_geometry(a, p, smem)) return false;
     const int base = p.tiles_k * p.tiles_c;
     int split = pick_split(a, p, true);
-    const bool use_ws = split > 1 && a->workspace && a->workspace_bytes >= (long)split * base * 9 * 4096 * 4;
+    const bool use_ws = split > 1 && a->workspace && a->workspace_bytes >= (long)split * base * (9 + (a->dy2 ? 1 : 0)) * 4096 * 4;
     if (!use_ws) split = pick_split(a, p, false);
     p.ws = use_ws ? reinterpret_cast<float *>(a->workspace) : nullptr;
+    p.ws2 = use_ws && a->dy2 ? p.ws + (size_t)split * base * 9 * 4096 : nullptr;
     p.per = (p.ntiles + split - 1) / split;
     p.split = (p.ntiles + p.per - 1) / p.per;
     return true;
 }
 
-int launch_reduce(const combat_wgrad_args *a, const W3dParams &p, hipStream_t st) {
+template <int TAPS>
+int launch_reduce_taps(const combat_wgrad_args *a, const W3dParams &p, hipStream_t st) {
     const int base = p.tiles_k * p.tiles_c;
+    const float *ws = TAPS == 9 ? p.ws : p.ws2;
+    float *dw = TAPS == 9 ? a->dw : a->dw2;
+    const int k_real = TAPS == 9 ? a->k_real : a->k2_real;
     static const bool env_det = getenv("COMBAT_WGRAD_DET_REDUCE") != nullptr;
     const bool det = combat_deterministic();
     const bool atomics = !env_det && (!det || base >= 4);
     if (atomics) {
-        const long e4 = (long)base * 9 * 1024;
+        const long e4 = (long)base * TAPS * 1024;
         int groups = (int)(512 / ((e4 + 255) / 256));
         if (groups < 1 || det) groups = 1;
         if (groups > p.split) groups = p.split;
-        COMBAT_LAUNCH(wgrad3x3_reduce_kernel, dim3((unsigned)((e4 + 255) / 256), groups), dim3(256), 0, st, p.ws, a->dw, base,
-                           p.tiles_c, p.split, a->k_real, a->c_real);
+        COMBAT_LAUNCH(wgrad3x3_reduce_kernel<TAPS>, dim3((unsigned)((e4 + 255) / 256), groups), dim3(256), 0, st, ws, dw, base,
+                           p.tiles_c, p.split, k_real, a->c_real);
     } else {
-        COMBAT_LAUNCH(wgrad3x3_reduce_det_kernel, dim3(256), dim3(256), 0, st, (const float *)p.ws, a->dw, base, p.tiles_c, p.split,
-                           a->k_real, a->c_real);
+        COMBAT_LAUNCH(wgrad3x3_reduce_det_kernel<TAPS>, dim3(256), dim3(256), 0, st, ws, dw, base, p.tiles_c, p.split,
+                           k_real, a->c_real);
     }
     CB_LAUNCH_CHECK();
     return COMBAT_OK;
 }
+
+int launch_reduce(const combat_wgrad_args *a, const W3dParams &p, hipStream_t st) { return launch_reduce_taps<9>(a, p, st); }
 
 bool fill_reduce_first(const combat_wgrad_args *prev, W3dParams &p) {
     p.red_ws = nullptr;
     p.red_dw = nullptr;
     p.red_base = p.red_tiles_c = p.red_split = p.red_k_real = p.red_c_real = p.red_pad = 0;
-    if (!prev) return true;
+    if (!prev || prev->stride != 1) return true;
     W3dParams q;
     if (!w3d_plan(prev, q)) return true;
     if (!q.ws) return true;
@@ -579,7 +710,6 @@
     W3dParams p;
     if (!w3d_plan(a, p)) return 1;
     if (combat_deterministic() && !p.ws && p.split > 1) return COMBAT_EINVAL;
-    if (!fill_reduce_first(a->reduce_first, p)) return COMBAT_EINVAL;
 #ifdef COMBAT_STAMPS
     p.stamps = g_stamps_wgrad_host;
 #else
@@ -587,6 +717,27 @@
 #endif
     const int blocks = p.tiles_k * p.tiles_c * p.split;
     int rc;
+    if (a->stride == 2) {
+        fill_reduce_first(nullptr, p);
+        if (a->reduce_first && a->reduce_first->split >= 0 && a->reduce_first->defer_reduce) {
+            rc = conv_wgrad3x3_dma_reduce(a->reduce_first, st);
+            if (rc != COMBAT_OK) return rc;
+        }
+        if (a->dy2) {
+            if (p.hpw == 5) rc = launch_w3d_s2<5, true>(p, blocks, st);
+            else if (p.hpw == 6) rc = launch_w3d_s2<6, true>(p, blocks, st);
+            else rc = launch_w3d_s2<7, true>(p, blocks, st);
+        } else {
+            if (p.hpw == 5) rc = launch_w3d_s2<5, false>(p, blocks, st);
+            else if (p.hpw == 6) rc = launch_w3d_s2<6, false>(p, blocks, st);
+            else rc = launch_w3d_s2<7, false>(p, blocks, st);
+        }
+        if (rc != COMBAT_OK || !p.ws) return rc;
+        rc = launch_reduce(a, p, st);
+        if (rc != COMBAT_OK || !a->dy2) return rc;
+        return launch_reduce_taps<1>(a, p, st);
+    }
+    if (!fill_reduce_first(a->reduce_first, p)) return COMBAT_EINVAL;
     if (p.hpw == 2) rc = launch_w3d<2, 3>(p, blocks, st);
     else if (p.hpw == 3) rc = launch_w3d<3, 2>(p, blocks, st);
     else rc = launch_w3d<4, 2>(p, blocks, st);
@@ -596,6 +747,34 @@
 
 int conv_wgrad3x3_dma_reduce(const combat_wgrad_args *a, hipStream_t st) {
     W3dParams p;
-    if (!w3d_plan(a, p) || !p.ws) return COMBAT_OK;
+    if (a->stride != 1 || !w3d_plan(a, p) || !p.ws) return COMBAT_OK;
     return launch_reduce(a, p, st);
 }
+
+extern "C" int combat_conv_wgrad_s2_table(const combat_wgrad_args *a, int32_t *geo, int32_t *row_src, int32_t *tap_row) {
+    W3dParams p;
+    int smem;
+    if (!a || a->stride != 2 || !w3d_geometry(a, p, smem, true)) return 1;
+    const S2Geo g{p.TW, p.TH, p.TI, p.HWP, p.HH, p.HROWS};
+    if (geo) {
+        const int v[8] = {p.TW, p.TH, p.TI, p.HWP, p.HH, p.HROWS, p.hpw, 0};
+        for (int i = 0; i < 8; ++i) geo[i] = v[i];
+    }
+    if (row_src)
+        for (int row = 0; row < p.hpw * 64; ++row) {
+            int ti, hy, hx, key;
+            const bool in = s2_row_decode(g, row, ti, hy, hx, key);
+            row_src[row * 4 + 0] = in ? ti : -1;
+            row_src[row * 4 + 1] = hy;
+            row_src[row * 4 + 2] = hx;
+            row_src[row * 4 + 3] = key;
+        }
+    if (tap_row)
+        for (int pk = 0; pk < 64; ++pk)
+            for (int tap = 0; tap < 9; ++tap) {
+                int key;
+                tap_row[(pk * 9 + tap) * 2] = s2_tap_row(g, pk % g.TW, (pk / g.TW) % g.TH, pk / (g.TW * g.TH), tap / 3, tap % 3, key);
+                tap_row[(pk * 9 + tap) * 2 + 1] = key;
+            }
+    return 0;
+}
diff --git a/combat_amd/engine.py b/combat_amd/engine.py
--- a/combat_amd/engine.py
+++ b/combat_amd/engine.py
@@ -439,7 +439,8 @@
     return a
 
 
-def rec_wgrad(plan: Plan, what: str, src, dy, pc: PackedConv, dw, pro: Optional[Affine] = None, aux: bool = True):
+def rec_wgrad(plan: Plan, what: str, src, dy, pc: PackedConv, dw, pro: Optional[Affine] = None, aux: bool = True,
+              second=None):
     a = ops.WgradArgs()
     a.N, a.H, a.W, a.C = src.shape
     _, a.P, a.Q, a.K = dy.shape
@@ -450,6 +451,9 @@
         a.pro_scale, a.pro_shift = _p(pro.scale), _p(pro.shift)
         a.pro_group_stride, a.pro_act, a.pro_slope = pro.group_stride, int(pro.act), pro.slope
     a.split = 0
+    if second is not None:
+        dy2, pc2, dw2 = second
+        a.dy2, a.dw2, a.k2_real = dy2.data_ptr(), dw2.data_ptr(), pc2.K
     queue = plan.next_aux_queue() if aux else -1
     ws = _wgrad_workspace(src.device, queue)
     a.workspace, a.workspace_bytes = ws.data_ptr(), ws.numel()
@@ -469,7 +473,7 @@
     elif aux and need > 0 and Plan.defer_reduces:
         ws = torch.empty(need, dtype=torch.uint8, device=src.device)
         a.workspace, a.workspace_bytes, a.defer_reduce = ws.data_ptr(), need, 1
-    plan.hold(a, src, dy, dw, pro, ws)
+    plan.hold(a, src, dy, dw, pro, ws, second)
     plan.add(what, lib.combat_conv_wgrad, ctypes.byref(a), aux=aux)
     plan.wgrads.append((len(plan.calls) - 1, a))
     if a.defer_reduce:
@@ -1009,13 +1013,17 @@
             self._bwd_apply(P, slot, "g." + blk.bn2.prefix, dz2, y1, dy1, st2)
             tsc, fused = None, None
             dz1 = slot.buf("g.b%d.dz1" % b, xin.shape)
+            rides = None
             if blk.sc is not None:
-                rec_wgrad(P, "b%d.sc.wgrad" % b, a0, d_out, blk.sc, fp.grad_phys(pre + "shortcut.0.weight"))
+                if ops.wgrad_shortcut_rides(a0, dy1, blk.conv1, d_out, blk.sc):
+                    rides = (d_out, blk.sc, fp.grad_phys(pre + "shortcut.0.weight"))
+                else:
+                    rec_wgrad(P, "b%d.sc.wgrad" % b, a0, d_out, blk.sc, fp.grad_phys(pre + "shortcut.0.weight"))
                 fused = fuse_shortcut(dy1, dz1, blk.conv1, d_out, blk.sc)
                 if fused is None:
                     tsc = slot.buf("g.b%d.tsc" % b, xin.shape)
                     rec_conv(P, "b%d.sc.dgrad" % b, d_out, tsc, blk.sc, 1)
-            rec_wgrad(P, "b%d.c1.wgrad" % b, a0, dy1, blk.conv1, fp.grad_phys(pre + "conv1.weight"))
+            rec_wgrad(P, "b%d.c1.wgrad" % b, a0, dy1, blk.conv1, fp.grad_phys(pre + "conv1.weight"), second=rides)
             self._dgrad_norm(P, slot, "g." + blk.bn1.prefix, dy1, dz1, blk.conv1, xin, st1, group_stride=0,
                              slope=0.0, gamma=blk.bn1.gamma, dgamma=fp.grad_phys(pre + "bn1.weight"),
                              dbeta=fp.grad_phys(pre + "bn1.bias"), add_pre=tsc, shortcut=fused)
diff --git a/combat_amd/ops.py b/combat_amd/ops.py
--- a/combat_amd/ops.py
+++ b/combat_amd/ops.py
@@ -182,6 +182,20 @@
           "src=%s dy=%s" % (tuple(src.shape), tuple(dy.shape)))
 
 
+def wgrad_shortcut_rides(src, dy, pc: PackedConv, dy_sc, pc_sc: PackedConv) -> bool:
+    if pc_sc.R != 1 or pc_sc.stride != 2 or pc_sc.pad != 0 or pc.R != 3 or pc.stride != 2 or tuple(dy_sc.shape) != tuple(dy.shape):
+        return False
+    if pc_sc.c_real != pc.c_real or pc_sc.K > dy.shape[-1]:
+        return False
+    a = WgradArgs()
+    a.N, a.H, a.W, a.C = src.shape
+    _, a.P, a.Q, a.K = dy.shape
+    a.R = a.S = pc.R
+    a.stride, a.pad, a.k_real, a.c_real = pc.stride, pc.pad, pc.K, pc.c_real
+    a.dy2, a.dw2, a.k2_real = dy_sc.data_ptr(), dy_sc.data_ptr(), pc_sc.K
+    return lib.combat_conv_wgrad_s2_table(ctypes.byref(a), None, None, None) == 0
+
+
 def norm_scratch_bytes(groups: int, c: int) -> int:
     return int(lib.combat_norm_scratch_bytes(groups, c))
 
diff --git a/include/combat_hip.h b/include/combat_hip.h
--- a/include/combat_hip.h
+++ b/include/combat_hip.h
@@ -101,11 +101,16 @@
     int32_t defer_reduce;
     int32_t reserved;
     const struct combat_wgrad_args *reduce_first;
+    const void *dy2;
+    float *dw2;
+    int32_t k2_real;
+    int32_t reserved2;
 } combat_wgrad_args;
 
 int combat_conv_wgrad(const combat_wgrad_args *a, void *stream);
 int combat_conv_wgrad_reduce(const combat_wgrad_args *a, void *stream);
 int64_t combat_conv_wgrad_workspace_bytes(const combat_wgrad_args *a);
+int combat_conv_wgrad_s2_table(const combat_wgrad_args *a, int32_t *geo, int32_t *row_src, int32_t *tap_row);
 
 int combat_pack_weights(const float *w, int32_t K, int32_t taps, int32_t c_real, int32_t C, int32_t dup_hilo,
                         void *wf, int32_t rows_pad_f, int32_t kpad_f,
```

Result: no change. 32850 images/sec (median of 3 runs) (+0.3%).
